# yixuan/ADMM

Hardware: AMD Instinct MI355X
Metric: ADMM iterations/sec, Lasso tall n=100000 p=10000 (100-lambda warm-started path) (higher is better)
Workload: dtype f32; 1 GPU; admm_lasso tall path (BASELINE configs[1]); n=100000, p=10000, nlambda=100, standardize=True, intercept=True, parallelism=single GPU, step=one cold-started warm-chained lambda path

## Files before the change

### admm_amd/_lib.py

```python
import ctypes
import os

import numpy as np

_HERE = os.path.dirname(os.path.abspath(__file__))
LIB_PATH = os.environ.get("ADMM_HIP_LIB") or os.path.join(_HERE, "lib", "libadmm_hip.so")

ADMM_MEM_HOST = 0
ADMM_MEM_DEVICE = 1


class AdmmOpts(ctypes.Structure):
    _fields_ = [("maxit", ctypes.c_int), ("eps_abs", ctypes.c_double),
                ("eps_rel", ctypes.c_double), ("rho", ctypes.c_double)]


class AdmmHipOptions(ctypes.Structure):
    _fields_ = [(k, ctypes.c_int) for k in (
        "struct_size", "gram_backend", "gram_split", "factor_backend", "inverse_precision", "tall_xupdate", "tall_refine",
        "consensus_two_pass", "consensus_unfused", "bp_two_pass", "lad_no_hat", "wide_no_persist", "wide_unfused", "wide_gram_sprad",
        "sharing_bp_direct", "cv_downdate", "peer_exchange", "batch_iters", "profile_stride", "pool_mb", "screen", "lad_two_pass",
        "par_devices")] + [("reserved", ctypes.c_int * 9)]


class AdmmStats(ctypes.Structure):
    _fields_ = [("t_h2d", ctypes.c_double), ("t_standardize", ctypes.c_double), ("t_gram", ctypes.c_double),
                ("t_eigs", ctypes.c_double), ("t_factor", ctypes.c_double), ("t_loop", ctypes.c_double),
                ("t_total", ctypes.c_double), ("loop_ms_events", ctypes.c_double),
                ("xupdate_ms_avg", ctypes.c_double), ("xupdate_samples", ctypes.c_longlong),
                ("total_iter", ctypes.c_longlong), ("xupdate_launches", ctypes.c_longlong),
                ("rho", ctypes.c_double), ("eig_est", ctypes.c_double),
                ("branch", ctypes.c_int), ("xupdate_variant", ctypes.c_int),
                ("exchange_variant", ctypes.c_int), ("refine", ctypes.c_int), ("persist_iter", ctypes.c_longlong),
                ("factor_flops", ctypes.c_double)]

    def as_dict(self):
        return {k: getattr(self, k) for k, _ in self._fields_}


class AdmmHipError(RuntimeError):
    def __init__(self, code, msg):
        super().__init__(f"libadmm_hip error {code}: {msg}")
        self.code = code


_lib = None

_DP = ctypes.c_void_p
_c_double_p = ctypes.POINTER(ctypes.c_double)
_c_float_p = ctypes.POINTER(ctypes.c_float)
_c_int_p = ctypes.POINTER(ctypes.c_int)

EXPORTS = ["admm_hip_lasso", "admm_hip_enet", "admm_hip_parlasso", "admm_hip_lad", "admm_hip_bp",
           "admm_hip_last_error", "admm_hip_version", "admm_hip_device_count", "admm_hip_set_device",
           "admm_hip_device_synchronize", "admm_hip_lasso_plan_create", "admm_hip_lasso_plan_run",
           "admm_hip_lasso_plan_destroy", "admm_hip_comm_unique_id", "admm_hip_comm_init", "admm_hip_comm_finalize", "admm_hip_comm_info",
           "admm_hip_parlasso_dist", "admm_hip_lasso_plan_create_dist",
           "admm_hip_lasso_plan_trace_enable", "admm_hip_lasso_plan_trace_read",
           "admm_hip_lasso_plan_state_enable", "admm_hip_lasso_plan_state_read", "admm_hip_lasso_plan_system_read",
           "admm_hip_host_lanczos", "admm_hip_test_symv",
           "admm_hip_comm_peer_prepare", "admm_hip_comm_init_peer", "admm_hip_comm_init_shm", "admm_hip_comm_test_allreduce", "admm_hip_comm_test_reduce_scatter",
           "admm_hip_lasso_dist", "admm_hip_test_gram", "admm_hip_test_spd_inverse", "admm_hip_test_cv_fold_system",
           "admm_hip_lasso_dist_cols", "admm_hip_test_gemv_t", "admm_hip_lad_traced", "admm_hip_bp_traced",
           "admm_hip_lasso_plan_create_dist_cols", "admm_hip_lasso_cv", "admm_hip_lasso_multi",
           "admm_hip_parbp", "admm_hip_parbp_traced", "admm_hip_parbp_dist", "admm_hip_dantzig", "admm_hip_dantzig_traced",
           "admm_hip_lad_state", "admm_hip_bp_state", "admm_hip_lasso_plan_data_read", "admm_hip_trim_memory", "admm_hip_test_gather",
           "admm_hip_options_default", "admm_hip_options_set", "admm_hip_option_set", "admm_hip_options_reset", "admm_hip_option_get",
           "admm_hip_last_parallel_layout", "admm_hip_parallel_assign", "admm_hip_grplasso", "admm_hip_grplasso_plan_create",
           "admm_hip_quantreg", "admm_hip_quantreg_state", "admm_hip_huber", "admm_hip_huber_state",
           "admm_hip_mtlasso", "admm_hip_mtlasso_plan_create", "admm_hip_test_symv_multi", "admm_hip_test_tall_early_exits",
           "admm_hip_sgl", "admm_hip_sgl_plan_create", "admm_hip_host_sgl_lambda0",
           "admm_hip_boxenet", "admm_hip_boxenet_plan_create", "admm_hip_host_box_lambda0",
           "admm_hip_test_gemm_nt", "admm_hip_test_cholesky_linvt", "admm_hip_test_spd_inverse_shift",
           "admm_hip_test_symv_plan", "admm_hip_test_symv_ex", "admm_hip_test_symv_multi_ex", "admm_hip_test_symv_f64acc"]

GROUP_MAX = 1024
MT_MAX = 16
MT_RHS_BUILT = (2, 4, 8, 12)

_GROUP_ARGS = [_c_int_p, _c_double_p, ctypes.c_int]
TALL_ONLY = [("admm_hip_grplasso", _GROUP_ARGS, 5), ("admm_hip_sgl", _GROUP_ARGS + [_c_double_p, ctypes.c_double], 5),
             ("admm_hip_boxenet", [_c_double_p] * 3 + [ctypes.c_double], 5), ("admm_hip_mtlasso", [ctypes.c_int, ctypes.c_int, _c_double_p], 4)]

TRACE_FIELDS = 12
TRACE_COLD, TRACE_CONVERGED, TRACE_ACCELERATE, TRACE_RESTART = -1, 0, 1, 2
TRACE_CONTINUE = 1


def load():
    global _lib
    if _lib is not None:
        return _lib
    path = os.environ.get("ADMM_HIP_LIB") or LIB_PATH
    if not os.path.exists(path):
        raise FileNotFoundError(
            f"{path} not found: build it with `python -m admm_amd.build` (hipcc --offload-arch=gfx950). "
            "admm_amd has no CPU fallback.")
    if not os.environ.get("ADMM_HIP_LIB"):
        from . import build as _build
        if os.path.isdir(_build.CSRC) and not _build._lib_is_current(path):
            raise RuntimeError(f"{path} was not built from the sources in {_build.CSRC} (source hash differs or is missing): "
                               "run `python -m admm_amd.build`")
    lib = ctypes.CDLL(path, mode=ctypes.RTLD_GLOBAL)
    lasso_args = [_DP, _DP, ctypes.c_int, ctypes.c_int, ctypes.c_int,
                  _DP, ctypes.c_int, ctypes.c_int, ctypes.c_double, ctypes.c_int, ctypes.c_int]
    tail = [ctypes.POINTER(AdmmOpts), _c_double_p, _c_float_p, _c_int_p, ctypes.POINTER(AdmmStats)]
    lib.admm_hip_lasso.argtypes = lasso_args + tail
    lib.admm_hip_enet.argtypes = lasso_args + [ctypes.c_double] + tail
    lib.admm_hip_parlasso.argtypes = lasso_args + [ctypes.c_int] + tail
    lib.admm_hip_lasso_cv.argtypes = ([_DP, _DP, ctypes.c_int, ctypes.c_int, ctypes.c_int, _c_int_p, ctypes.c_int,
                                       _DP, ctypes.c_int, ctypes.c_int, ctypes.c_double, ctypes.c_int, ctypes.c_int, ctypes.c_double,
                                       ctypes.POINTER(AdmmOpts), _c_double_p, _c_float_p, _c_int_p,
                                       _c_double_p, _c_double_p, _c_double_p, _c_int_p, _c_float_p, _c_int_p, _c_int_p,
                                       ctypes.POINTER(AdmmStats)])
    lib.admm_hip_lasso_cv.restype = ctypes.c_int
    lib.admm_hip_lasso_multi.argtypes = ([_DP, _DP, ctypes.c_int, ctypes.c_int, ctypes.c_int, ctypes.c_int,
                                          _DP, ctypes.c_int, ctypes.c_int, ctypes.c_double, ctypes.c_int, ctypes.c_int, ctypes.c_double,
                                          ctypes.POINTER(AdmmOpts), _c_double_p, _c_float_p, _c_int_p, ctypes.POINTER(AdmmStats)])
    lib.admm_hip_lasso_multi.restype = ctypes.c_int
    lib.admm_hip_lad.argtypes = [_DP, _DP, ctypes.c_int, ctypes.c_int, ctypes.c_int, ctypes.c_int,
                                 ctypes.POINTER(AdmmOpts), _c_double_p, _c_int_p, ctypes.POINTER(AdmmStats)]
    lib.admm_hip_bp.argtypes = [_DP, _DP, ctypes.c_int, ctypes.c_int, ctypes.c_int,
                                ctypes.POINTER(AdmmOpts), _c_double_p, _c_int_p, ctypes.POINTER(AdmmStats)]
    lib.admm_hip_lad_traced.argtypes = lib.admm_hip_lad.argtypes + [_c_double_p, ctypes.c_longlong, ctypes.POINTER(ctypes.c_longlong)]
    lib.admm_hip_lad_traced.restype = ctypes.c_int
    lib.admm_hip_bp_traced.argtypes = lib.admm_hip_bp.argtypes + [_c_double_p, ctypes.c_longlong, ctypes.POINTER(ctypes.c_longlong)]
    lib.admm_hip_bp_traced.restype = ctypes.c_int
    lib.admm_hip_lad_state.argtypes = lib.admm_hip_lad_traced.argtypes + [_c_double_p, ctypes.c_longlong, ctypes.POINTER(ctypes.c_longlong)]
    lib.admm_hip_lad_state.restype = ctypes.c_int
    lib.admm_hip_quantreg.argtypes = [_DP, _DP, ctypes.c_int, ctypes.c_int, ctypes.c_int, ctypes.c_int, _c_double_p, ctypes.c_int,
                                      ctypes.POINTER(AdmmOpts), _c_double_p, _c_int_p, ctypes.POINTER(AdmmStats)]
    lib.admm_hip_quantreg.restype = ctypes.c_int
    lib.admm_hip_quantreg_state.argtypes = ([_DP, _DP, ctypes.c_int, ctypes.c_int, ctypes.c_int, ctypes.c_int, ctypes.c_double,
                                             ctypes.POINTER(AdmmOpts), _c_double_p, _c_int_p, ctypes.POINTER(AdmmStats)]
                                            + [_c_double_p, ctypes.c_longlong, ctypes.POINTER(ctypes.c_longlong)] * 2)
    lib.admm_hip_quantreg_state.restype = ctypes.c_int
    lib.admm_hip_huber.argtypes = [_DP, _DP, ctypes.c_int, ctypes.c_int, ctypes.c_int, ctypes.c_int, _c_double_p, _c_double_p, ctypes.c_int,
                                   ctypes.POINTER(AdmmOpts), _c_double_p, _c_int_p, ctypes.POINTER(AdmmStats)]
    lib.admm_hip_huber.restype = ctypes.c_int
    lib.admm_hip_huber_state.argtypes = ([_DP, _DP, ctypes.c_int, ctypes.c_int, ctypes.c_int, ctypes.c_int, ctypes.c_double, ctypes.c_double,
                                          ctypes.POINTER(AdmmOpts), _c_double_p, _c_int_p, ctypes.POINTER(AdmmStats)]
                                         + [_c_double_p, ctypes.c_longlong, ctypes.POINTER(ctypes.c_longlong)] * 2)
    lib.admm_hip_huber_state.restype = ctypes.c_int
    lib.admm_hip_bp_state.argtypes = lib.admm_hip_bp_traced.argtypes + [_c_double_p, ctypes.c_longlong, ctypes.POINTER(ctypes.c_longlong)]
    lib.admm_hip_bp_state.restype = ctypes.c_int
    lib.admm_hip_dantzig.argtypes = [_DP, _DP, ctypes.c_int, ctypes.c_int, ctypes.c_int, _DP, ctypes.c_int, ctypes.c_int, ctypes.c_double,
                                     ctypes.c_int, ctypes.c_int, ctypes.POINTER(AdmmOpts), _c_double_p, _c_double_p, _c_int_p, ctypes.POINTER(AdmmStats)]
    lib.admm_hip_dantzig.restype = ctypes.c_int
    lib.admm_hip_dantzig_traced.argtypes = lib.admm_hip_dantzig.argtypes + [_c_double_p, ctypes.c_longlong, ctypes.POINTER(ctypes.c_longlong)]
    lib.admm_hip_dantzig_traced.restype = ctypes.c_int
    lib.admm_hip_parbp.argtypes = [_DP, _DP, ctypes.c_int, ctypes.c_int, ctypes.c_int, ctypes.c_int,
                                   ctypes.POINTER(AdmmOpts), _c_double_p, _c_int_p, ctypes.POINTER(AdmmStats)]
    lib.admm_hip_parbp.restype = ctypes.c_int
    lib.admm_hip_parbp_traced.argtypes = lib.admm_hip_parbp.argtypes + [_c_double_p, ctypes.c_longlong, ctypes.POINTER(ctypes.c_longlong)]
    lib.admm_hip_parbp_traced.restype = ctypes.c_int
    lib.admm_hip_parbp_dist.argtypes = [_DP, _DP, ctypes.c_int, ctypes.c_int, ctypes.c_longlong, ctypes.c_longlong, ctypes.c_int, ctypes.c_int,
                                        ctypes.POINTER(AdmmOpts), _c_double_p, _c_int_p, ctypes.POINTER(AdmmStats)]
    lib.admm_hip_parbp_dist.restype = ctypes.c_int
    for name in ("admm_hip_lasso", "admm_hip_enet", "admm_hip_parlasso", "admm_hip_lad", "admm_hip_bp",
                 "admm_hip_device_count", "admm_hip_set_device", "admm_hip_device_synchronize"):
        getattr(lib, name).restype = ctypes.c_int
    lib.admm_hip_set_device.argtypes = [ctypes.c_int]
    lib.admm_hip_last_error.restype = ctypes.c_char_p
    lib.admm_hip_version.restype = ctypes.c_char_p
    lib.admm_hip_lasso_plan_create.argtypes = lasso_args + [ctypes.c_double, ctypes.c_int, ctypes.POINTER(AdmmOpts),
                                               ctypes.POINTER(ctypes.c_void_p), _c_int_p]
    lib.admm_hip_lasso_plan_create.restype = ctypes.c_int
    for name, extra, at in TALL_ONLY:
        args = lasso_args[:at] + extra + lasso_args[5:]
        for fn, rest in ((getattr(lib, name), tail), (getattr(lib, name + "_plan_create"), [tail[0], ctypes.POINTER(ctypes.c_void_p), _c_int_p])):
            fn.argtypes, fn.restype = args + rest, ctypes.c_int
    lib.admm_hip_host_sgl_lambda0.argtypes = [_c_float_p, ctypes.c_int, _c_int_p, _c_double_p, ctypes.c_int, _c_double_p, ctypes.c_double, _c_float_p]
    lib.admm_hip_host_sgl_lambda0.restype = ctypes.c_int
    lib.admm_hip_host_box_lambda0.argtypes = [_c_float_p, ctypes.c_int, _c_float_p, _c_float_p, _c_double_p, ctypes.c_double, _c_float_p]
    lib.admm_hip_host_box_lambda0.restype = ctypes.c_int
    lib.admm_hip_lasso_plan_run.argtypes = [ctypes.c_void_p, _c_double_p, _c_float_p, _c_int_p, ctypes.POINTER(AdmmStats)]
    lib.admm_hip_lasso_plan_run.restype = ctypes.c_int
    lib.admm_hip_lasso_plan_destroy.argtypes = [ctypes.c_void_p]
    lib.admm_hip_lasso_plan_destroy.restype = ctypes.c_int
    dist_args = [_DP, _DP, ctypes.c_int, ctypes.c_longlong, ctypes.c_int, ctypes.c_int,
                 _DP, ctypes.c_int, ctypes.c_int, ctypes.c_double, ctypes.c_int, ctypes.c_int, ctypes.c_int, ctypes.POINTER(AdmmOpts)]
    lib.admm_hip_parlasso_dist.argtypes = dist_args + [_c_double_p, _c_float_p, _c_int_p, ctypes.POINTER(AdmmStats)]
    lib.admm_hip_parlasso_dist.restype = ctypes.c_int
    lib.admm_hip_lasso_plan_create_dist.argtypes = dist_args + [ctypes.POINTER(ctypes.c_void_p), _c_int_p]
    lib.admm_hip_lasso_plan_create_dist.restype = ctypes.c_int
    lib.admm_hip_lasso_dist.argtypes = [_DP, _DP, ctypes.c_int, ctypes.c_longlong, ctypes.c_int, ctypes.c_int,
                                        _DP, ctypes.c_int, ctypes.c_int, ctypes.c_double, ctypes.c_int, ctypes.c_int, ctypes.c_double,
                                        ctypes.POINTER(AdmmOpts), _c_double_p, _c_float_p, _c_int_p, ctypes.POINTER(AdmmStats)]
    lib.admm_hip_lasso_dist.restype = ctypes.c_int
    lib.admm_hip_lasso_dist_cols.argtypes = [_DP, _DP, ctypes.c_int, ctypes.c_int, ctypes.c_longlong, ctypes.c_longlong, ctypes.c_int,
                                             _DP, ctypes.c_int, ctypes.c_int, ctypes.c_double, ctypes.c_int, ctypes.c_int, ctypes.c_double,
                                             ctypes.POINTER(AdmmOpts), _c_double_p, _c_float_p, _c_int_p, ctypes.POINTER(AdmmStats)]
    lib.admm_hip_lasso_dist_cols.restype = ctypes.c_int
    lib.admm_hip_lasso_plan_create_dist_cols.argtypes = lib.admm_hip_lasso_dist_cols.argtypes[:15] + [ctypes.POINTER(ctypes.c_void_p), _c_int_p]
    lib.admm_hip_lasso_plan_create_dist_cols.restype = ctypes.c_int
    lib.admm_hip_comm_unique_id.argtypes = [ctypes.c_void_p]
    lib.admm_hip_comm_unique_id.restype = ctypes.c_int
    lib.admm_hip_comm_init.argtypes = [ctypes.c_int, ctypes.c_int, ctypes.c_void_p]
    lib.admm_hip_comm_init.restype = ctypes.c_int
    lib.admm_hip_comm_finalize.argtypes = []
    lib.admm_hip_comm_finalize.restype = ctypes.c_int
    lib.admm_hip_options_default.argtypes = [ctypes.POINTER(AdmmHipOptions)]
    lib.admm_hip_options_default.restype = ctypes.c_int
    lib.admm_hip_options_set.argtypes = [ctypes.POINTER(AdmmHipOptions)]
    lib.admm_hip_options_set.restype = ctypes.c_int
    lib.admm_hip_option_set.argtypes = [ctypes.c_char_p, ctypes.c_char_p]
    lib.admm_hip_option_set.restype = ctypes.c_int
    lib.admm_hip_options_reset.argtypes = []
    lib.admm_hip_options_reset.restype = ctypes.c_int
    lib.admm_hip_option_get.argtypes = [ctypes.c_char_p]
    lib.admm_hip_option_get.restype = ctypes.c_char_p
    lib.admm_hip_comm_info.argtypes = [ctypes.POINTER(ctypes.c_int)] * 3
    lib.admm_hip_comm_info.restype = ctypes.c_int
    lib.admm_hip_comm_peer_prepare.argtypes = [ctypes.c_int, ctypes.c_void_p]
    lib.admm_hip_comm_peer_prepare.restype = ctypes.c_int
    lib.admm_hip_comm_init_peer.argtypes = [ctypes.c_int, ctypes.c_int, ctypes.c_void_p]
    lib.admm_hip_comm_init_peer.restype = ctypes.c_int
    lib.admm_hip_comm_init_shm.argtypes = [ctypes.c_int, ctypes.c_int, ctypes.c_char_p, ctypes.c_ulonglong]
    lib.admm_hip_comm_init_shm.restype = ctypes.c_int
    lib.admm_hip_comm_test_allreduce.argtypes = [ctypes.c_void_p, ctypes.c_longlong, ctypes.c_void_p, ctypes.c_longlong, ctypes.c_int]
    lib.admm_hip_comm_test_allreduce.restype = ctypes.c_int
    lib.admm_hip_comm_test_reduce_scatter.argtypes = [ctypes.c_void_p, ctypes.c_longlong, ctypes.c_void_p]
    lib.admm_hip_comm_test_reduce_scatter.restype = ctypes.c_int
    lib.admm_hip_lasso_plan_trace_enable.argtypes = [ctypes.c_void_p, ctypes.c_longlong]
    lib.admm_hip_lasso_plan_trace_enable.restype = ctypes.c_int
    lib.admm_hip_lasso_plan_trace_read.argtypes = [ctypes.c_void_p, _c_double_p, ctypes.c_longlong, ctypes.POINTER(ctypes.c_longlong)]
    lib.admm_hip_lasso_plan_trace_read.restype = ctypes.c_int
    lib.admm_hip_lasso_plan_state_enable.argtypes = [ctypes.c_void_p, ctypes.c_longlong]
    lib.admm_hip_lasso_plan_state_enable.restype = ctypes.c_int
    lib.admm_hip_lasso_plan_state_read.argtypes = [ctypes.c_void_p, ctypes.POINTER(ctypes.c_float), ctypes.c_longlong,
                                                   ctypes.POINTER(ctypes.c_longlong), ctypes.POINTER(ctypes.c_longlong)]
    lib.admm_hip_lasso_plan_state_read.restype = ctypes.c_int
    lib.admm_hip_lasso_plan_data_read.argtypes = [ctypes.c_void_p, ctypes.POINTER(ctypes.c_float), ctypes.c_longlong, ctypes.POINTER(ctypes.c_float)]
    lib.admm_hip_lasso_plan_data_read.restype = ctypes.c_int
    lib.admm_hip_lasso_plan_system_read.argtypes = [ctypes.c_void_p, ctypes.POINTER(ctypes.c_float), ctypes.c_longlong]
    lib.admm_hip_lasso_plan_system_read.restype = ctypes.c_int
    lib.admm_hip_test_symv.argtypes = [_c_float_p, ctypes.c_int, _c_float_p, _c_float_p, _c_float_p, _c_float_p]
    lib.admm_hip_test_symv.restype = ctypes.c_int
    lib.admm_hip_test_symv_multi.argtypes = [_c_float_p, ctypes.c_int, _c_float_p, ctypes.c_int, ctypes.c_int, _c_float_p]
    lib.admm_hip_test_symv_multi.restype = ctypes.c_int
    lib.admm_hip_test_symv_plan.argtypes = [ctypes.c_int] * 4 + [_c_int_p, ctypes.POINTER(ctypes.c_longlong), _c_int_p, ctypes.c_int]
    lib.admm_hip_test_symv_plan.restype = ctypes.c_int
    lib.admm_hip_test_symv_ex.argtypes = [_c_float_p, ctypes.c_int, _c_float_p, _c_float_p, ctypes.c_int, ctypes.c_int, ctypes.c_int,
                                          _c_float_p, _c_float_p, _c_int_p]
    lib.admm_hip_test_symv_ex.restype = ctypes.c_int
    lib.admm_hip_test_symv_multi_ex.argtypes = [_c_float_p, ctypes.c_int, _c_float_p, ctypes.c_int, ctypes.c_int, ctypes.c_int, ctypes.c_int,
                                                _c_float_p, _c_int_p]
    lib.admm_hip_test_symv_multi_ex.restype = ctypes.c_int
    lib.admm_hip_test_symv_f64acc.argtypes = [_c_float_p, ctypes.c_int, _c_float_p, _c_float_p, _c_double_p, _c_double_p, _c_int_p]
    lib.admm_hip_test_symv_f64acc.restype = ctypes.c_int
    lib.admm_hip_test_tall_early_exits.argtypes = [ctypes.POINTER(ctypes.c_longlong)]
    lib.admm_hip_test_tall_early_exits.restype = ctypes.c_int
    lib.admm_hip_test_gram.argtypes = [ctypes.c_void_p, ctypes.c_int, ctypes.c_int, ctypes.c_int, ctypes.c_int, ctypes.c_void_p]
    lib.admm_hip_test_gram.restype = ctypes.c_int
    lib.admm_hip_test_gemv_t.argtypes = [ctypes.c_void_p, ctypes.c_int, ctypes.c_int, ctypes.c_int, ctypes.c_void_p, ctypes.c_void_p]
    lib.admm_hip_test_gemv_t.restype = ctypes.c_int
    lib.admm_hip_test_spd_inverse.argtypes = [ctypes.c_void_p, ctypes.c_int, ctypes.c_int, ctypes.c_void_p]
    lib.admm_hip_test_spd_inverse.restype = ctypes.c_int
    lib.admm_hip_test_spd_inverse_shift.argtypes = [ctypes.c_void_p, ctypes.c_int, ctypes.c_double, ctypes.c_void_p]
    lib.admm_hip_test_spd_inverse_shift.restype = ctypes.c_int
    lib.admm_hip_test_cholesky_linvt.argtypes = [ctypes.c_int, ctypes.c_void_p, ctypes.c_int, ctypes.c_void_p, ctypes.c_void_p]
    lib.admm_hip_test_cholesky_linvt.restype = ctypes.c_int
    lib.admm_hip_test_gemm_nt.argtypes = [ctypes.c_int] * 9 + [ctypes.c_double, ctypes.c_double, ctypes.c_void_p, ctypes.c_void_p, ctypes.c_void_p]
    lib.admm_hip_test_gemm_nt.restype = ctypes.c_int
    lib.admm_hip_test_cv_fold_system.argtypes = [ctypes.c_void_p, ctypes.c_void_p, ctypes.c_int, ctypes.c_int, ctypes.c_void_p, ctypes.c_int, ctypes.c_int,
                                                 ctypes.c_int, ctypes.c_int, ctypes.c_void_p, ctypes.c_void_p, ctypes.c_void_p, ctypes.c_void_p, ctypes.c_void_p]
    lib.admm_hip_test_cv_fold_system.restype = ctypes.c_int
    lib.admm_hip_host_lanczos.argtypes = [_c_float_p, ctypes.c_int, _c_float_p, _c_int_p]
    lib.admm_hip_host_lanczos.restype = ctypes.c_int
    lib.admm_hip_test_gather.argtypes = [ctypes.c_void_p, ctypes.c_int, ctypes.c_int, ctypes.c_int, ctypes.c_void_p, _c_double_p]
    lib.admm_hip_test_gather.restype = ctypes.c_int
    lib.admm_hip_last_parallel_layout.argtypes = [_c_int_p, _c_int_p, ctypes.c_int]
    lib.admm_hip_last_parallel_layout.restype = ctypes.c_int
    lib.admm_hip_parallel_assign.argtypes = [ctypes.c_int, ctypes.c_char_p, ctypes.c_int, _c_int_p, _c_int_p, ctypes.c_int]
    lib.admm_hip_parallel_assign.restype = ctypes.c_int
    lib.admm_hip_trim_memory.argtypes = []
    lib.admm_hip_trim_memory.restype = ctypes.c_int
    _lib = lib
    return lib


def check(code):
    if code != 0:
        raise AdmmHipError(code, load().admm_hip_last_error().decode())


class DevicePtr:

    def __init__(self, ptr):
        self.ptr = int(ptr)


def as_input(a, n=None, p=None):
    if isinstance(a, DevicePtr):
        return ctypes.c_void_p(a.ptr), ADMM_MEM_DEVICE, a
    arr = np.asfortranarray(np.asarray(a, dtype=np.float64))
    return ctypes.c_void_p(arr.ctypes.data), ADMM_MEM_HOST, arr


class options:

    def __init__(self, **kw):
        self.kw = {k.upper(): (None if v is None else str(v)) for k, v in kw.items()}
        self.old = {}

    def __enter__(self):
        lib = load()
        try:
            for k, v in self.kw.items():
                cur = lib.admm_hip_option_get(k.encode())
                self.old[k] = cur.decode() if cur is not None else None
                check(lib.admm_hip_option_set(k.encode(), None if v is None else v.encode()))
        except BaseException:
            self.__exit__(None, None, None)
            raise
        return self

    def __exit__(self, *exc):
        lib = load()
        for k, v in self.old.items():
            check(lib.admm_hip_option_set(k.encode(), None if v is None else v.encode()))
        return False

    @staticmethod
    def set(**kw):
        lib = load()
        for k, v in kw.items():
            check(lib.admm_hip_option_set(k.upper().encode(), None if v is None else str(v).encode()))

    @staticmethod
    def reset():
        check(load().admm_hip_options_reset())

    @staticmethod
    def struct(**fields):
        lib = load()
        o = AdmmHipOptions()
        check(lib.admm_hip_options_default(ctypes.byref(o)))
        for k, v in fields.items():
            setattr(o, k, int(v))
        check(lib.admm_hip_options_set(ctypes.byref(o)))
        return o


def last_parallel_layout():
    lib = load()
    nr = ctypes.c_int(0)
    devs = (ctypes.c_int * 64)()
    check(lib.admm_hip_last_parallel_layout(ctypes.byref(nr), devs, 64))
    return [int(devs[r]) for r in range(min(nr.value, 64))]


def parallel_assign(nblocks, par_devices, device_count):
    lib = load()
    nr = ctypes.c_int(0)
    devs = (ctypes.c_int * 64)()
    check(lib.admm_hip_parallel_assign(int(nblocks), None if par_devices is None else str(par_devices).encode(), int(device_count),
                                       ctypes.byref(nr), devs, 64))
    return [int(devs[r]) for r in range(nr.value)] if nr.value > 1 else []
```

### admm_amd/csrc/api.hip

```cpp
#include "calls.h"
#include "comm.h"
#include "inproc.h"
#include "test_hooks.h"

using namespace admm;

template <typename F>
static int guarded(F&& f) {
    try {
        check_option_overlay();
        f();
        return ADMM_OK;
    } catch (const Error& e) {
        set_last_error(e.what());
        return e.code;
    } catch (const std::bad_alloc&) {
        set_last_error("host allocation failed");
        return ADMM_ERR_INTERNAL;
    } catch (const std::exception& e) {
        set_last_error(e.what());
        return ADMM_ERR_INTERNAL;
    }
}

// ... 284 lines not shown
int admm_hip_mtlasso_plan_create(const double* x, const double* Y, int n, int p, int m, int mem,
                                 const double* row_weight,
                                 const double* lambda_in, int nlambda_in, int nlambda_auto, double lmin_ratio,
                                 int standardize, int intercept, const admm_opts* opts,
                                 admm_hip_plan** plan_out, int* nlambda_out) {
    return guarded([&] { plan_create(x, Y, n, p, mem, mt_spec(PATH_SPEC(-1.0), p, m, row_weight), plan_out, nlambda_out); });
}

int admm_hip_options_default(admm_hip_options* o) {
    return guarded([&] {
        ADMM_REQUIRE(o != nullptr, "options must not be NULL");
        std::memset(o, 0, sizeof(*o));
        o->struct_size = (int)sizeof(*o);
    });
}
int admm_hip_options_reset(void) { return guarded([&] { thread_options() = ThreadOptions(); }); }
int admm_hip_option_set(const char* name, const char* value) {
    return guarded([&] {
        ADMM_REQUIRE(name != nullptr && name[0] != 0, "option name must not be empty");
        Opt id;
        ADMM_REQUIRE(opt_find(name, &id), std::string("unknown option '") + name + "' (INTEGRATION.md section 5 lists the names)");
        opt_set_thread(id, value);
    });
}
const char* admm_hip_option_get(const char* name) {
    Opt id;
    return name && opt_find(name, &id) ? opt_text(id) : nullptr;
}
int admm_hip_options_set(const admm_hip_options* o) {
    return guarded([&] {
        ThreadOptions n;
        if (o == nullptr) { thread_options() = n; return; }
        ADMM_REQUIRE(o->struct_size >= (int)(2 * sizeof(int)) && o->struct_size <= (int)sizeof(admm_hip_options), "options: bad struct_size");
        admm_hip_options v;
        std::memset(&v, 0, sizeof(v));
        std::memcpy(&v, o, (size_t)o->struct_size);
        auto set = [&](Opt k, const char* val) { opt_parse(k, val, &n.v[(int)k]); n.has[(int)k] = true; };
        auto num = [&](Opt k, int val) { set(k, std::to_string(val).c_str()); };
        if (v.gram_backend == 1) set(Opt::GRAM, "rocblas");
        if (v.gram_split) { ADMM_REQUIRE(v.gram_split >= 1 && v.gram_split <= 3, "options: gram_split"); set(Opt::GRAM_SPLIT, v.gram_split == 1 ? "0" : (v.gram_split == 2 ? "f16x2" : "bf16x3")); }
        if (v.factor_backend == 1) set(Opt::FACTOR, "rocsolver");
        if (v.inverse_precision) { ADMM_REQUIRE(v.inverse_precision == 1 || v.inverse_precision == 2, "options: inverse_precision"); set(Opt::INVERSE, v.inverse_precision == 1 ? "f32" : "f64"); }
        if (v.tall_xupdate) { ADMM_REQUIRE(v.tall_xupdate == 1 || v.tall_xupdate == 2, "options: tall_xupdate"); set(Opt::XUPDATE, v.tall_xupdate == 1 ? "gemv" : "sym"); }
        if (v.tall_refine) set(Opt::REFINE, "1");
        if (v.consensus_two_pass) set(Opt::PAR_ONEPASS, "0");
        if (v.consensus_unfused >= 1) set(Opt::PAR_FUSE_PZ, "0");
        if (v.consensus_unfused >= 2) set(Opt::PAR_BATCH, "0");
        if (v.bp_two_pass) set(Opt::BP_ONEPASS, "0");
        if (v.lad_no_hat) set(Opt::LAD_HAT, "0");
        if (v.wide_no_persist == 1) set(Opt::WIDE_PERSIST, "0");
        if (v.wide_no_persist == 2) set(Opt::WIDE_PERSIST_COLS, "0");
        if (v.wide_unfused) set(Opt::WIDE_FUSE, "0");
        if (v.wide_gram_sprad) set(Opt::WIDE_SPRAD, "gram");
        if (v.sharing_bp_direct) set(Opt::SBP_GRAM, "0");
        if (v.cv_downdate) set(Opt::CV_DOWNDATE, v.cv_downdate == 1 ? "1" : "0");
        if (v.peer_exchange) set(Opt::PEER_FUSED, v.peer_exchange == 1 ? "2" : "0");
        if (v.batch_iters > 0) num(Opt::BATCH_ITERS, v.batch_iters);
        if (v.profile_stride > 0) num(Opt::PROFILE_STRIDE, v.profile_stride);
        if (v.pool_mb) num(Opt::POOL_MB, v.pool_mb < 0 ? 0 : v.pool_mb);
        if (v.lad_two_pass) set(Opt::LAD_ONEPASS, "0");
        if (v.par_devices) {
            ADMM_REQUIRE(v.par_devices >= -1 && v.par_devices <= 64, "options: par_devices");
            std::string l;
            for (int d = 0; d < v.par_devices; ++d) l += (d ? "," : "") + std::to_string(d);
            set(Opt::PAR_DEVICES, v.par_devices == -1 ? "all" : l.c_str());
        }
        if (v.screen) {
            ADMM_REQUIRE(v.screen >= 1 && v.screen <= 3, "options: screen");
            set(Opt::WIDE_SCREEN, v.screen == 1 ? "16" : (v.screen == 3 ? "8" : "0"));
            set(Opt::SBP_SCREEN, v.screen == 2 ? "0" : "1");
        }
        thread_options() = n;
    });
}
int admm_hip_comm_unique_id(void* id_out) {
    return guarded([&] { ADMM_REQUIRE(id_out != nullptr, "id_out must not be NULL"); comm_unique_id(id_out); });
}
int admm_hip_comm_init(int nranks, int rank, const void* id) {
    return guarded([&] { ADMM_REQUIRE(id != nullptr, "id must not be NULL"); require_device(); comm_init(nranks, rank, id); });
}
int admm_hip_comm_finalize(void) {
    return guarded([&] { comm_finalize(); });
}
int admm_hip_comm_info(int* nranks_out, int* rank_out, int* backend_out) {
    return guarded([&] {
        const CommInfo ci = comm_info_live();
        if (nranks_out) *nranks_out = ci.active ? ci.nranks : 1;
        if (rank_out) *rank_out = ci.active ? ci.rank : 0;
        if (backend_out) *backend_out = ci.active ? ci.backend : 0;
    });
}
int admm_hip_comm_peer_prepare(int nranks, void* handle_out) {
    return guarded([&] { ADMM_REQUIRE(handle_out != nullptr, "handle_out must not be NULL"); require_device(); comm_peer_prepare(nranks, handle_out); });
}
int admm_hip_comm_init_peer(int nranks, int rank, const void* handles) {
    return guarded([&] { ADMM_REQUIRE(handles != nullptr, "handles must not be NULL"); require_device(); comm_init_peer(nranks, rank, handles); });
}
int admm_hip_comm_init_shm(int nranks, int rank, const char* name, unsigned long long token) {
    return guarded([&] { require_device(); comm_init_shm(nranks, rank, name, token); });
}
int admm_hip_comm_test_allreduce(float* fbuf, long long nf, double* dbuf, long long nd, int mem) {
    return guarded([&] {
        ADMM_REQUIRE(nf >= 0 && nd >= 0 && (nf == 0 || fbuf) && (nd == 0 || dbuf), "bad arguments");
        ADMM_REQUIRE(comm_info().active, "no communicator");
        require_device();
        Stream st;
        DevBuf<float> df; DevBuf<double> dd;
        float* pf = fbuf; double* pd = dbuf;
        if (mem == ADMM_MEM_HOST) {
            df.alloc((size_t)nf); dd.alloc((size_t)nd);
            if (nf) ADMM_HIP_CHECK(hipMemcpyAsync(df.get(), fbuf, (size_t)nf * sizeof(float), hipMemcpyHostToDevice, st.s));
            if (nd) ADMM_HIP_CHECK(hipMemcpyAsync(dd.get(), dbuf, (size_t)nd * sizeof(double), hipMemcpyHostToDevice, st.s));
            pf = df.get(); pd = dd.get();
        }
        if (nf && nd) allreduce_sum_f32_f64(pf, (size_t)nf, pd, (size_t)nd, st.s);
        else if (nf) allreduce_sum_f32(pf, (size_t)nf, st.s);
        else if (nd) allreduce_sum_f64(pd, (size_t)nd, st.s);
        if (mem == ADMM_MEM_HOST) {
            if (nf) ADMM_HIP_CHECK(hipMemcpyAsync(fbuf, pf, (size_t)nf * sizeof(float), hipMemcpyDeviceToHost, st.s));
            if (nd) ADMM_HIP_CHECK(hipMemcpyAsync(dbuf, pd, (size_t)nd * sizeof(double), hipMemcpyDeviceToHost, st.s));
        }
        st.sync();
        comm_check();
    });
}

int admm_hip_comm_test_reduce_scatter(const float* send, long long count, float* recv) {
    return guarded([&] {
        ADMM_REQUIRE(count > 0 && count % 4 == 0 && send && recv, "bad arguments (count must be a positive multiple of 4)");
        require_device();
        const CommInfo ci = comm_info();
        const size_t nr = (size_t)(ci.active ? ci.nranks : 1);
        Stream st;
        DevBuf<float> ds(nr * (size_t)count), dr((size_t)count);
        ADMM_HIP_CHECK(hipMemcpyAsync(ds.get(), send, nr * (size_t)count * sizeof(float), hipMemcpyHostToDevice, st.s));
        reduce_scatter_sum_f32(ds.get(), dr.get(), (size_t)count, st.s);
        ADMM_HIP_CHECK(hipMemcpyAsync(recv, dr.get(), (size_t)count * sizeof(float), hipMemcpyDeviceToHost, st.s));
        st.sync();
        comm_check();
    });
}

int admm_hip_lasso_plan_run(admm_hip_plan* plan, double* lambda_out, float* beta_out, int* niter_out, admm_stats* stats) {
    return guarded([&] { run_plan(reinterpret_cast<PlanHandle*>(plan), PATH_OUT, 0.0); });
}

int admm_hip_lasso_plan_destroy(admm_hip_plan* plan) {
    return guarded([&] { delete reinterpret_cast<PlanHandle*>(plan); });
}

int admm_hip_lasso_plan_trace_enable(admm_hip_plan* plan, long long capacity_records) {
    return guarded([&] {
        ADMM_REQUIRE(capacity_records > 0 && capacity_records <= (1ll << 26), "trace capacity must be within [1, 2^26] records");
        plan_of(plan).enable_trace(capacity_records);
    });
}

int admm_hip_lasso_plan_trace_read(admm_hip_plan* plan, double* out, long long cap_records, long long* nrecords_out) {
    return guarded([&] {
        ADMM_REQUIRE(out != nullptr && nrecords_out != nullptr && cap_records >= 0, "bad trace output arguments");
        *nrecords_out = plan_of(plan).read_trace(out, cap_records);
    });
}

int admm_hip_lasso_plan_state_enable(admm_hip_plan* plan, long long capacity_records) {
    return guarded([&] {
        ADMM_REQUIRE(capacity_records > 0 && capacity_records <= (1ll << 22), "state capacity must be within [1, 2^22] records");
        plan_of(plan).enable_state(capacity_records);
    });
}

int admm_hip_lasso_plan_state_read(admm_hip_plan* plan, float* out, long long cap_records, long long* nrecords_out, long long* record_floats_out) {
    return guarded([&] {
        ADMM_REQUIRE(nrecords_out != nullptr && cap_records >= 0 && (out != nullptr || cap_records == 0), "bad state output arguments");
        *nrecords_out = plan_of(plan).read_state(out, cap_records, record_floats_out);
    });
}

int admm_hip_lasso_plan_data_read(admm_hip_plan* plan, float* x_out, long long ld, float* y_out) {
    return guarded([&] {
        plan_of(plan).read_data(x_out, ld, y_out);
    });
}

int admm_hip_lasso_plan_system_read(admm_hip_plan* plan, float* out, long long ld) {
    return guarded([&] {
        plan_of(plan).read_system(out, ld);
    });
}

int admm_hip_last_parallel_layout(int* nranks, int* devices, int cap) {
    return guarded([&] {
        ADMM_REQUIRE(nranks != nullptr && cap >= 0 && (cap == 0 || devices != nullptr), "bad layout arguments");
        *nranks = (int)last_layout().size();
        for (int r = 0; r < std::min(cap, *nranks); ++r) devices[r] = last_layout()[r];
    });
}

int admm_hip_parallel_assign(int nblocks, const char* par_devices, int device_count, int* nranks, int* devices, int cap) {
    return guarded([&] {
        ADMM_REQUIRE(nblocks >= 1 && device_count >= 0, "nblocks must be >= 1 and device_count >= 0");
        ADMM_REQUIRE(nranks != nullptr && cap >= 0 && (cap == 0 || devices != nullptr), "bad layout arguments");
        const std::vector<int> lay = par_layout(nblocks, parse_par_devices(par_devices, device_count));
        *nranks = lay.empty() ? 1 : (int)lay.size();
        for (int r = 0; r < std::min(cap, (int)lay.size()); ++r) devices[r] = lay[r];
    });
}

const char* admm_hip_last_error(void) { return last_error_ref().c_str(); }
const char* admm_hip_version(void) { return "admm_hip 0.3 (gfx950)"; }
int admm_hip_trim_memory(void) {
    admm::pool_trim();
    return ADMM_OK;
}

int admm_hip_device_count(void) {
    int cnt = 0;
    if (hipGetDeviceCount(&cnt) != hipSuccess) return 0;
    return cnt;
}
int admm_hip_set_device(int device) {
    return guarded([&] { ADMM_HIP_CHECK(hipSetDevice(device)); });
}
int admm_hip_device_synchronize(void) {
    return guarded([&] { ADMM_HIP_CHECK(hipDeviceSynchronize()); });
}

int admm_hip_host_lanczos(const float* A, int n, float* eig_out, int* nmatop_out) {
    return guarded([&] {
        ADMM_REQUIRE(A && eig_out && n >= 3, "bad arguments");
        auto op = [&](const float* v, float* w) {
            for (int i = 0; i < n; ++i) w[i] = 0.f;
            for (int j = 0; j < n; ++j) {
                const float vj = v[j];
                const float* col = A + (size_t)j * n;
                for (int i = 0; i < n; ++i) w[i] += col[i] * vj;
            }
        };
        *eig_out = lanczos_largest_f32(op, n, nmatop_out);
    });
}

int admm_hip_host_sgl_lambda0(const float* xy, int p, const int* group, const double* group_weight, int ngroups,
                              const double* l1_weight, double alpha, float* out) {
    return guarded([&] {
        ADMM_REQUIRE(xy && out && p > 0, "bad arguments");
        const PathSpec s = sgl_spec(PathSpec(), p, group, group_weight, ngroups, l1_weight, alpha);
        s.check_sgl_args(p);
        const std::vector<int> start = s.group_starts();
        std::vector<double> l1, wg;
        sgl_prepare(alpha, l1_weight, group_weight, start, l1, wg);
        *out = sgl_lambda0(xy, start, l1, wg);
    });
}

int admm_hip_host_box_lambda0(const float* xy, int p, const float* lower_std, const float* upper_std, const double* penalty_factor,
                              double alpha, float* out) {
    return guarded([&] {
        ADMM_REQUIRE(xy && out && p > 0, "bad arguments");
        PathSpec s = box_spec(PathSpec(), p, nullptr, nullptr, penalty_factor);
        s.alpha = alpha;
        s.check_box_args(p);
        for (int j = 0; j < p; ++j)
            ADMM_REQUIRE((!lower_std || lower_std[j] <= 0.f) && (!upper_std || upper_std[j] >= 0.f), "the box must hold zero");
        float l0 = box_lambda0(xy, p, lower_std, upper_std, penalty_factor);
        if (s.enet()) l0 = box_lambda0_enet(l0, alpha);
        *out = l0;
    });
}

int admm_hip_test_symv(const float* A, int p, const float* v0, const float* v1, float* y0, float* y1) {
    return guarded([&] {
        ADMM_REQUIRE(A && v0 && v1 && y0 && y1 && p > 0, "bad arguments");
        test_symv(A, p, v0, v1, y0, y1);
    });
}

int admm_hip_test_symv_multi(const float* A, int p, const float* V, int nr, int rhs_per_pass, float* Yout) {
    return guarded([&] {
        ADMM_REQUIRE(A && V && Yout && p > 0 && nr >= 1 && nr <= 64, "bad arguments");
        test_symv_multi(A, p, V, nr, rhs_per_pass, Yout);
    });
}

int admm_hip_test_symv_plan(int p, int cus, int part, int nparts, int* sched_out, long long* info_out, int* tiles_out, int tile_capacity) {
    return guarded([&] {
        ADMM_REQUIRE(sched_out && info_out && tiles_out, "symv plan hook: sched_out, info_out and tiles_out must not be NULL");
        ADMM_REQUIRE(p >= 1 && p <= kSymvHookMaxP && cus <= 65536 && nparts >= 1 && nparts <= 64 && part >= 0 && part < nparts && tile_capacity >= 1,
                     "symv plan hook: p in 1 .. 32768, cus <= 65536, nparts in 1 .. 64, part in 0 .. nparts - 1, tile_capacity >= 1");
        test_symv_plan(p, cus, part, nparts, sched_out, info_out, tiles_out, tile_capacity);
    });
}

int admm_hip_test_symv_ex(const float* A, int p, const float* v0, const float* v1, int variant, int part, int nparts, float* y0, float* y1,
                          int* sched_out) {
    return guarded([&] {
        ADMM_REQUIRE(A && v0 && v1 && y0 && y1 && sched_out, "symv_ex hook: A, v0, v1, y0, y1 and sched_out must not be NULL");
        ADMM_REQUIRE(p >= 1 && p <= kSymvHookMaxP && variant >= 0 && variant <= 2 && nparts >= 1 && nparts <= 64 && part >= 0 && part < nparts,
                     "symv_ex hook: p in 1 .. 32768, variant in 0 .. 2, nparts in 1 .. 64, part in 0 .. nparts - 1");
        test_symv_ex(A, p, v0, v1, variant, part, nparts, y0, y1, sched_out);
    });
}

int admm_hip_test_symv_multi_ex(const float* A, int p, const float* V, int nr, int rhs_per_pass, int nt, int finish, float* Yout, int* sched_out) {
    return guarded([&] {
        ADMM_REQUIRE(A && V && Yout && sched_out, "symv_multi_ex hook: A, V, Yout and sched_out must not be NULL");
        ADMM_REQUIRE(p >= 1 && p <= kSymvHookMaxP && nr >= 1 && nr <= 64 && test_symv_rhs_built(rhs_per_pass) && (nt == 0 || nt == 1) && (finish == 0 || finish == 1),
                     "symv_multi_ex hook: p in 1 .. 32768, nr in 1 .. 64, rhs_per_pass one of the built widths (2, 4, 8, 12), nt and finish 0 or 1");
        test_symv_multi_ex(A, p, V, nr, rhs_per_pass, nt, finish, Yout, sched_out);
    });
}

int admm_hip_test_symv_f64acc(const float* A, int p, const float* v0, const float* v1, double* y0, double* y1, int* sched_out) {
    return guarded([&] {
        ADMM_REQUIRE(A && v0 && v1 && y0 && y1 && sched_out, "symv_f64acc hook: A, v0, v1, y0, y1 and sched_out must not be NULL");
        ADMM_REQUIRE(p >= 1 && p <= kSymvHookMaxP, "symv_f64acc hook: p in 1 .. 32768");
        test_symv_f64acc(A, p, v0, v1, y0, y1, sched_out);
    });
}

int admm_hip_test_tall_early_exits(long long* count) {
    return guarded([&] {
        ADMM_REQUIRE(count != nullptr, "bad arguments");
        *count = tall_last_early_exits();
    });
}

int admm_hip_test_gram(const void* A, int rows, int cols, int atA, int is_double, void* G) {
    return guarded([&] {
        ADMM_REQUIRE(A && G && rows > 0 && cols > 0, "bad arguments");
        if (is_double) test_gram<double>(static_cast<const double*>(A), rows, cols, atA != 0, static_cast<double*>(G));
        else test_gram<float>(static_cast<const float*>(A), rows, cols, atA != 0, static_cast<float*>(G));
    });
}

int admm_hip_test_gemv_t(const void* A, int rows, int cols, int is_double, const void* v, void* y) {
    return guarded([&] {
        ADMM_REQUIRE(A && v && y && rows > 0 && cols > 0, "bad arguments");
        if (is_double) test_gemv_t<double>(static_cast<const double*>(A), rows, cols, static_cast<const double*>(v), static_cast<double*>(y));
        else test_gemv_t<float>(static_cast<const float*>(A), rows, cols, static_cast<const float*>(v), static_cast<float*>(y));
    });
}

int admm_hip_test_gather(const void* A, int rows, int cols, int is_double, const void* v, double* y) {
    return guarded([&] {
        ADMM_REQUIRE(A && v && y && rows > 0 && cols > 0, "bad arguments");
        if (is_double) test_gather<double>(static_cast<const double*>(A), rows, cols, static_cast<const double*>(v), y);
        else test_gather<float>(static_cast<const float*>(A), rows, cols, static_cast<const float*>(v), y);
    });
}

int admm_hip_test_spd_inverse(const void* A, int n, int precision, void* Ainv) {
    return guarded([&] {
        ADMM_REQUIRE(A && Ainv && n > 0 && precision >= 0 && precision <= 2, "bad arguments");
        if (precision == 1) test_spd_inverse<double>(static_cast<const double*>(A), n, static_cast<double*>(Ainv), false);
        else test_spd_inverse<float>(static_cast<const float*>(A), n, static_cast<float*>(Ainv), precision == 2);
    });
}

int admm_hip_test_spd_inverse_shift(const float* A, int n, double diag, float* Ainv) {
    return guarded([&] {
        ADMM_REQUIRE(A && Ainv && n > 0 && std::isfinite(diag), "bad arguments");
        test_spd_inverse_shift(A, n, diag, Ainv);
    });
}

int admm_hip_test_cholesky_linvt(int is_double, const void* A, int n, void* L, void* U) {
    return guarded([&] {
        ADMM_REQUIRE(A && L && U && n > 0, "bad arguments");
        if (is_double) test_cholesky_linvt<double>(static_cast<const double*>(A), n, static_cast<double*>(L), static_cast<double*>(U));
        else test_cholesky_linvt<float>(static_cast<const float*>(A), n, static_cast<float*>(L), static_cast<float*>(U));
    });
}

int admm_hip_test_gemm_nt(int is_double, int lower, int mirror, int kstart_row, int b_lower, int in_place, int M, int N, int K,
                          double alpha, double beta, const void* A, const void* B, void* C) {
    return guarded([&] {
        ADMM_REQUIRE(A && B && C, "gemm_nt hook: A, B and C must not be NULL");
        ADMM_REQUIRE(M > 0 && N > 0 && K > 0 && M <= 16384 && N <= 16384 && K <= (1 << 20), "gemm_nt hook: M, N in 1 .. 16384 and K in 1 .. 2^20");
        ADMM_REQUIRE(std::isfinite(alpha) && std::isfinite(beta), "gemm_nt hook: alpha and beta must be finite");
        ADMM_REQUIRE(!lower || M == N, "gemm_nt hook: lower needs a square output (M == N)");
        ADMM_REQUIRE(!mirror || lower, "gemm_nt hook: the mirrored store belongs to lower launches");
        ADMM_REQUIRE(!b_lower || (is_double && !lower), "gemm_nt hook: b_lower (the K loop ended at the tile's last column) is double only and not for lower launches");
        ADMM_REQUIRE(!in_place || (N <= 128 && K == 128 && !lower), "gemm_nt hook: in_place needs N <= 128, K == 128 and a full (not lower) launch");
        if (is_double)
            test_gemm_nt<double>(lower != 0, mirror != 0, kstart_row != 0, b_lower != 0, in_place != 0, M, N, K, alpha, beta, static_cast<const double*>(A),
                                 static_cast<const double*>(B), static_cast<double*>(C));
        else
            test_gemm_nt<float>(lower != 0, mirror != 0, kstart_row != 0, false, in_place != 0, M, N, K, alpha, beta, static_cast<const float*>(A),
                                static_cast<const float*>(B), static_cast<float*>(C));
    });
}

int admm_hip_test_cv_fold_system(const double* x, const double* y, int n, int p, const int* fold_id, int nfolds, int fold,
                                 int standardize, int intercept, float* gram, float* xy, float* mean_x, float* scale_x, float* mean_scale_y) {
    return guarded([&] { test_cv_fold_system(x, y, n, p, fold_id, nfolds, fold, standardize, intercept, gram, xy, mean_x, scale_x, mean_scale_y); });
}

}
```

### admm_amd/csrc/lasso_tall.hip

```cpp
#include "prep.h"
#include "gemv_kernels.h"
#include "symv_kernels.h"
#include "solvers.h"
#include "sgl_host.h"
#include "box_host.h"
#include "comm.h"
#include "loop_driver.h"
#include "plan_host.h"
#include "peer_device.h"
#include "probe.h"

namespace admm {

struct TallCtl {
    double rho, lam, eps_primal, eps_dual, adj_a, adj_c, tau;
    double a_next, tau_next;
    int mode;
    int restart;
    int iter;
    int lam_idx;
    int done;
    int first;
    int total;
    int fin_idx;
    int fin_niter;
    int pad;
};

struct TallParams {
    int p, nwg, nseg, maxit, nlam, enet;
    long long part_stride;
    double eps_abs, eps_rel, alpha, sqrt_p;
    const double* lambdas;
    const float* XY;
    const float* a_part; const float* b_part;
    const float* dot0; const float* dot1; const float* axp0; const float* axp1;
    long long ldo; int nrb, p32; SymvSched sched;
    float* x; float* z0; float* z1; float* y0; float* y1; float* adj_z; float* adj_y; float* u; float* w;
    TallCtl* ctl;
    double* P;
    float* beta;
    int* niter;
    int* done_host;
#ifdef ADMM_HIP_PROBE
    long long* probe;
#endif
    double* trace;
    long long trace_cap;
    const float* refine_ab;
    long long refine_ld;
    float* state;
    long long state_cap;
    unsigned long long* verdict;
    unsigned long long run_tag;
};

__host__ __device__ inline unsigned long long tall_verdict_word(unsigned long long run_tag, int total, bool discard) {
    return run_tag | ((unsigned long long)(unsigned)total << 1) | (discard ? 1ull : 0ull);
}
constexpr int kVerdictShift = 33;
constexpr int kVerdictWords = kSyVerdictReplicas * kSyVerdictStride;

constexpr int kTailThreads = 256;
constexpr int kTailLanes = kSySumLanes;
constexpr int kTailElems = kTailThreads / kTailLanes;

__device__ __forceinline__ double tall_load_partial(const double* p, bool in_launch) {
    if (!in_launch) return *p;
    return __longlong_as_double((long long)__hip_atomic_load(reinterpret_cast<const unsigned long long*>(p), __ATOMIC_RELAXED, __HIP_MEMORY_SCOPE_AGENT));
}
__device__ __forceinline__ void tall_store_wt(float* p, float v) {
    __hip_atomic_store(reinterpret_cast<unsigned int*>(p), __float_as_uint(v), __ATOMIC_RELAXED, __HIP_MEMORY_SCOPE_AGENT);
}
__device__ __forceinline__ void tall_store_wt(double* p, double v) {
    __hip_atomic_store(reinterpret_cast<unsigned long long*>(p), (unsigned long long)__double_as_longlong(v), __ATOMIC_RELAXED, __HIP_MEMORY_SCOPE_AGENT);
}

template <bool IN_LAUNCH = false>
__device__ void tall_decide(const TallParams& q, int par) {
    __shared__ double dscratch[6 * (kTailThreads / 64)];
    WIDE_PROBE_DECL
    WIDE_PROBE(0);
    const TallCtl in = q.ctl[par];
    TallCtl* outp = &q.ctl[par ^ 1];
    if (in.done) {
        if (threadIdx.x == 0) { TallCtl o = in; o.fin_idx = -1; *outp = o; }
        return;
    }
    WIDE_PROBE(1);
    double acc[6] = {0, 0, 0, 0, 0, 0};
    const double* Pin = q.P + (size_t)par * q.nwg * 8;
    for (int w = threadIdx.x; w < q.nwg; w += kTailThreads) {
#pragma unroll
        for (int k = 0; k < 6; ++k) acc[k] += tall_load_partial(Pin + (size_t)w * 8 + k, IN_LAUNCH);
    }
    block_sum<double, 6>(acc, dscratch);
    if (threadIdx.x != 0) return;
    WIDE_PROBE(2);
    const double r2 = acc[0], dz2 = acc[1], daz2 = acc[2], x2 = acc[3], z2 = acc[4], y2 = acc[5];
    double tr_rp = 0, tr_rd = 0, tr_c = 0, tr_code = ADMM_TRACE_COLD;
    TallCtl out = in;
    out.first = 0;
    out.fin_idx = -1; out.fin_niter = 0;
    if (!in.first) {
        const double rp = sqrt(r2);
        const double rd = in.rho * sqrt(dz2);
        tr_rp = rp; tr_rd = rd;
        if (rp < in.eps_primal && rd < in.eps_dual) {
            out.fin_idx = in.lam_idx; out.fin_niter = in.iter + 1;
            out.mode = 0;
            tr_code = ADMM_TRACE_CONVERGED;
        } else {
            const double old_c = in.adj_c;
            const double c = in.rho * rp * rp + in.rho * daz2;
            tr_c = c;
            if (c < 0.999 * old_c) {
                out.adj_a = in.a_next; out.adj_c = c; out.tau = in.tau_next; out.restart = 0;
                tr_code = ADMM_TRACE_ACCELERATE;
            } else {
                out.adj_a = 1.0; out.adj_c = old_c / 0.999; out.tau = -1.0; out.restart = 1;
                tr_code = ADMM_TRACE_RESTART;
            }
            out.mode = 1;
            out.iter = in.iter + 1;
            if (in.iter + 1 >= q.maxit) {
                out.fin_idx = in.lam_idx; out.fin_niter = q.maxit + 1;
            }
        }
        if (out.fin_idx >= 0) {
            out.lam_idx = in.lam_idx + 1;
            out.iter = 0;
            if (out.lam_idx >= q.nlam) out.done = 1;
            else out.lam = q.lambdas[out.lam_idx];
            q.niter[out.fin_idx] = out.fin_niter;
        }
    } else {
        out.mode = 1; out.tau = 0.0; out.restart = 0;
    }
    if (q.verdict != nullptr && (out.mode == 0 || out.done)) {
        const unsigned long long word = tall_verdict_word(q.run_tag, in.total + 1, true);
        for (int r = 0; r < kSyVerdictReplicas; ++r)
            __hip_atomic_store(q.verdict + (size_t)r * kSyVerdictStride, word, __ATOMIC_RELAXED, __HIP_MEMORY_SCOPE_AGENT);
    }
    out.eps_primal = fmax(sqrt(x2), sqrt(z2)) * q.eps_rel + q.sqrt_p * q.eps_abs;
    out.eps_dual = sqrt(y2) * q.eps_rel + q.sqrt_p * q.eps_abs;
    out.a_next = 0.5 + 0.5 * sqrt(1.0 + 4.0 * out.adj_a * out.adj_a);
    out.tau_next = (out.adj_a - 1.0) / out.a_next;
    out.total = in.total + 1;
    *outp = out;
    if (out.done) *q.done_host = 1;
    WIDE_PROBE(3);
    WIDE_PROBE_FLUSH(2, in.total);
    if (q.trace != nullptr && in.total < q.trace_cap) {
        double* t = q.trace + (size_t)in.total * ADMM_TRACE_FIELDS;
        t[0] = in.lam_idx; t[1] = in.iter; t[2] = in.eps_primal; t[3] = in.eps_dual; t[4] = tr_rp; t[5] = tr_rd;
        t[6] = tr_c; t[7] = in.adj_c; t[8] = tr_code; t[9] = in.rho; t[10] = in.rho; t[11] = in.lam;
    }
}

struct TallDecideExtra {
    static constexpr bool kHas = true;
    TallParams q; int par;
    __device__ void operator()() const { tall_decide<false>(q, par); }
};

__device__ __forceinline__ float tall_extrapolate(float t1, float t, float cur, float old) {
#pragma clang fp contract(off)
    const float a = t1 * cur;
    const float b = t * old;
    return a - b;
}

struct TallElem { float zc, yc, zo, yo, adjz, adjy, x, xy; };

__device__ __forceinline__ TallElem tall_load_elem(const TallParams& q, int par, int i) {
    const float* zc_ = par ? q.z1 : q.z0; const float* yc_ = par ? q.y1 : q.y0;
    const float* zo_ = par ? q.z0 : q.z1; const float* yo_ = par ? q.y0 : q.y1;
    TallElem e;
    e.zc = zc_[i]; e.yc = yc_[i]; e.zo = zo_[i]; e.yo = yo_[i]; e.adjz = q.adj_z[i]; e.adjy = q.adj_y[i]; e.x = q.x[i]; e.xy = q.XY[i];
    return e;
}

__device__ __forceinline__ float tall_soft(float vec, double pen) {
    const double v = (double)vec;
    return v > pen ? (float)(v - pen) : (v < -pen ? (float)(v + pen) : 0.f);
}

__device__ __forceinline__ double tall_block_shrink(double nrm2, double pen) {
    const double nrm = sqrt(nrm2);
    return nrm > pen ? 1.0 - pen / nrm : 0.0;
}

template <bool WT = false>
__device__ __forceinline__ void tall_update_elem(const TallParams& q, const TallCtl& c, int par, int i, const TallElem& e, float a, float b, double (&acc)[6]) {
#pragma clang fp contract(off)
    float* zo_ = par ? q.z0 : q.z1; float* yo_ = par ? q.y0 : q.y1;
    const float zc = e.zc, yc = e.yc, zo = e.zo, yo = e.yo;
    if (c.fin_idx >= 0) q.beta[(size_t)c.fin_idx * q.p + i] = zc;
    if (c.done) return;
    float adjz, adjy, x;
    if (c.mode) {
        if (c.restart) { adjz = zo; adjy = yo; x = b; }
        else {
            const float t = (float)c.tau, t1 = (float)(1.0 + c.tau);
            adjz = tall_extrapolate(t1, t, zc, zo);
            adjy = tall_extrapolate(t1, t, yc, yo);
            x = a;
        }
    } else { adjz = e.adjz; adjy = e.adjy; x = e.x; }
    const float rho_f = (float)c.rho;
    const float vec = x + adjy / rho_f;
    const double pen = c.lam / c.rho;
    float zn;
    if (!q.enet) zn = tall_soft(vec, pen);
    else {
        const float thresh = (float)(q.alpha * pen);
        const float denom = (float)(1.0 + pen * (1.0 - q.alpha));
        zn = vec > thresh ? (vec - thresh) / denom : (vec < -thresh ? (vec + thresh) / denom : 0.f);
    }
    const float r = x - zn;
    const float yn = adjy + rho_f * r;
    const float dz = zn - zc, daz = zn - adjz;
    acc[0] = (double)r * r; acc[1] = (double)dz * dz; acc[2] = (double)daz * daz;
    acc[3] = (double)x * x; acc[4] = (double)zn * zn; acc[5] = (double)yn * yn;
    q.x[i] = x; zo_[i] = zn; yo_[i] = yn; q.adj_z[i] = adjz; q.adj_y[i] = adjy;
    if (q.state != nullptr && c.total < q.state_cap) {
        float* s = q.state + (size_t)c.total * 5 * q.p;
        s[i] = x; s[q.p + i] = zn; s[2 * (size_t)q.p + i] = yn; s[3 * (size_t)q.p + i] = adjz; s[4 * (size_t)q.p + i] = adjy;
    }
    const float tn = (float)c.tau_next, tn1 = (float)(1.0 + c.tau_next);
    const float adjz_a = tall_extrapolate(tn1, tn, zn, zc), adjy_a = tall_extrapolate(tn1, tn, yn, yc);
    const float un = (float)((double)(e.xy - adjy_a) + c.rho * (double)adjz_a);
    const float wn = (float)((double)(e.xy - yc) + c.rho * (double)zc);
    if (WT) { tall_store_wt(q.u + i, un); tall_store_wt(q.w + i, wn); }
    else { q.u[i] = un; q.w[i] = wn; }
}

__device__ __forceinline__ void tall_publish_norms(const TallParams& q, int par, const double (&acc)[6], double* scratch) {
    static_assert(kTailLanes == 8, "owner lanes are the multiples of 8");
    const int lane = threadIdx.x & 63, wid = threadIdx.x >> 6;
    const double v8[8] = {acc[0], acc[1], acc[2], acc[3], acc[4], acc[5], 0.0, 0.0};
    const double tot = halving_sum8_top(v8, lane);
    if ((lane & 7) == 0 && lane < 48) scratch[(lane >> 3) * (kTailThreads / 64) + wid] = tot;
    __syncthreads();
    if (threadIdx.x < 6) {
        double sum = 0;
        for (int ww = 0; ww < kTailThreads / 64; ++ww) sum += scratch[threadIdx.x * (kTailThreads / 64) + ww];
        q.P[((size_t)(par ^ 1) * q.nwg + blockIdx.x) * 8 + threadIdx.x] = sum;
    }
}

enum { TAIL_GEMV = 0, TAIL_SYMV = 1, TAIL_PEER = 2, TAIL_PEER1 = 3 };

__device__ __forceinline__ void tall_lane_sum(float& a, float& b) {
#pragma unroll
    for (int m = 1; m < kTailLanes; m <<= 1) { a += __shfl_xor(a, m, 64); b += __shfl_xor(b, m, 64); }
}

template <int MODE>
__device__ __forceinline__ void tall_gather_ab(const TallParams& q, int i, int sub, bool valid, float& a, float& b) {
    if (MODE == TAIL_SYMV) {
        symv_sum_partials<kTailLanes>(q.dot0, q.dot1, q.axp0, q.axp1, q.ldo, q.nrb, q.sched, q.p32, i, sub, valid, a, b);
        return;
    }
    a = 0.f; b = 0.f;
    if (valid) {
        for (int k = sub; k < q.nseg; k += kTailLanes) {
            const size_t o = (size_t)k * q.part_stride + i;
            a += q.a_part[o]; b += q.b_part[o];
        }
    }
    tall_lane_sum(a, b);
}

template <int MODE>
__global__ void __launch_bounds__(kTailThreads)
tall_tail_kernel(TallParams q, int par, PeerExchange ex) {
    __shared__ double scratch[6 * (kTailThreads / 64)];
    WIDE_PROBE_DECL
    WIDE_PROBE(0);
    const TallCtl c = q.ctl[par ^ 1];
    const int sub = threadIdx.x & (kTailLanes - 1);
    const int i = blockIdx.x * kTailElems + threadIdx.x / kTailLanes;
    const bool valid = i < q.p;
    const bool owner = valid && sub == 0;
    TallElem e = {0.f, 0.f, 0.f, 0.f, 0.f, 0.f, 0.f, 0.f};
    if (owner) e = tall_load_elem(q, par, i);
    float a = 0.f, b = 0.f;
    if (MODE == TAIL_PEER || MODE == TAIL_PEER1) {
        const bool live = !q.ctl[par].done;
        if (MODE == TAIL_PEER1 && live) {
            float sa, sb;
            symv_sum_partials<kTailLanes>(q.dot0, q.dot1, q.axp0, q.axp1, q.ldo, q.nrb, q.sched, q.p32, i, sub, valid, sa, sb);
            if (valid) {
                for (int dst = sub; dst < ex.nranks; dst += kTailLanes)
                    peer_store_f32x2(reinterpret_cast<float*>(peer_dst_slot(ex, dst)) + 2 * (size_t)i, sa, sb);
            }
            peer_publish(ex, gridDim.x);
        }
        const bool ok = live ? peer_wait_relaxed(ex) : false;
        if (ok && valid) {
            for (int r = sub; r < ex.nranks; r += kTailLanes) {
                const float2 v = peer_load_f32x2(reinterpret_cast<const float*>(peer_src_slot(ex, r)) + 2 * (size_t)i);
                a += v.x; b += v.y;
            }
        }
        tall_lane_sum(a, b);
    } else {
        tall_gather_ab<MODE>(q, i, sub, valid, a, b);
        if (MODE == TAIL_SYMV && q.refine_ab != nullptr && valid) {
            a = q.refine_ab[i] + a;
            b = q.refine_ab[q.refine_ld + i] + b;
        }
    }
    if (c.done && c.fin_idx < 0) return;
    WIDE_PROBE(1);

    double acc[6] = {0, 0, 0, 0, 0, 0};
    if (owner) tall_update_elem(q, c, par, i, e, a, b, acc);
    if (c.done) return;
    WIDE_PROBE(2);
    tall_publish_norms(q, par, acc, scratch);
    WIDE_PROBE(3);
    WIDE_PROBE_FLUSH(blockIdx.x == 0 ? 0 : (blockIdx.x == gridDim.x - 1 ? 1 : -1), c.total - 1);
}

struct GroupCoord { int gs, gn; double w; };
struct GroupTailParams {
    const int2* tiles;
    const GroupCoord* coord;
    const double* l1;
};
constexpr int kGroupMax = ADMM_HIP_GROUP_MAX;

template <int MODE, bool SPARSE = false>
__global__ void __launch_bounds__(kTailThreads)
tall_group_tail_kernel(TallParams q, int par, GroupTailParams gp) {
#pragma clang fp contract(off)
    static_assert(MODE == TAIL_GEMV || MODE == TAIL_SYMV, "single device");
    __shared__ double scratch[6 * (kTailThreads / 64)];
    __shared__ double snrm[kTailElems];
    __shared__ float sx[kGroupMax], sadjz[kGroupMax], sadjy[kGroupMax], sv[kGroupMax], szc[kGroupMax], syc[kGroupMax], sxy[kGroupMax];
    const TallCtl c = q.ctl[par ^ 1];
    const int2 tile = gp.tiles[blockIdx.x];
    const int i0 = tile.x, cnt = tile.y;
    const int sub = threadIdx.x & (kTailLanes - 1), e = threadIdx.x / kTailLanes;
    const int npass = (cnt + kTailElems - 1) / kTailElems;
    const bool big = cnt > kTailElems;
    const GroupCoord gc = gp.coord[i0 + min(e, cnt - 1)];
    float* zo_ = par ? q.z0 : q.z1; float* yo_ = par ? q.y0 : q.y1;
    const float rho_f = (float)c.rho;

    for (int k = 0; k < npass; ++k) {
        const int s = k * kTailElems + e, i = i0 + s;
        const bool valid = s < cnt, owner = valid && sub == 0;
        TallElem el = {0.f, 0.f, 0.f, 0.f, 0.f, 0.f, 0.f, 0.f};
        if (owner) el = tall_load_elem(q, par, i);
        double l1 = 0.0;
        if (SPARSE && owner) l1 = gp.l1[i];
        float a, b;
        tall_gather_ab<MODE>(q, i, sub, valid, a, b);
        if (c.done && c.fin_idx < 0) return;
        if (owner) {
            if (c.fin_idx >= 0) q.beta[(size_t)c.fin_idx * q.p + i] = el.zc;
            if (!c.done) {
                float adjz, adjy, x;
                if (c.mode) {
                    if (c.restart) { adjz = el.zo; adjy = el.yo; x = b; }
                    else {
                        const float t = (float)c.tau, t1 = (float)(1.0 + c.tau);
                        adjz = tall_extrapolate(t1, t, el.zc, el.zo);
                        adjy = tall_extrapolate(t1, t, el.yc, el.yo);
                        x = a;
                    }
                } else { adjz = el.adjz; adjy = el.adjy; x = el.x; }
                float vec = x + adjy / rho_f;
                if (SPARSE && gc.gn > 1) vec = tall_soft(vec, c.lam * l1 / c.rho);
                sx[s] = x; sadjz[s] = adjz; sadjy[s] = adjy; sv[s] = vec;
                szc[s] = el.zc; syc[s] = el.yc; sxy[s] = el.xy;
            }
        }
    }
    if (c.done) return;
    __syncthreads();

    double nrm2 = 0.0;
    if (big) {
        if (sub == 0) {
            double part = 0.0;
            for (int s = e; s < cnt; s += kTailElems) { const double v = (double)sv[s]; part += v * v; }
            snrm[e] = part;
        }
        __syncthreads();
        for (int m = 0; m < kTailElems; ++m) nrm2 += snrm[m];
    } else if (sub == 0 && e < cnt && gc.gn > 1) {
        const int s0 = gc.gs - i0;
        for (int m = 0; m < gc.gn; ++m) { const double v = (double)sv[s0 + m]; nrm2 += v * v; }
    }
    const double pen = c.lam * gc.w / c.rho;
    double shrink = 0.0;
    if (gc.gn > 1) shrink = tall_block_shrink(nrm2, pen);

    double acc[6] = {0, 0, 0, 0, 0, 0};
    const float tn = (float)c.tau_next, tn1 = (float)(1.0 + c.tau_next);
    for (int k = 0; k < npass; ++k) {
        const int s = k * kTailElems + e, i = i0 + s;
        if (!(s < cnt && sub == 0)) continue;
        const float x = sx[s], adjz = sadjz[s], adjy = sadjy[s], vec = sv[s], zc = szc[s], yc = syc[s], xy = sxy[s];
        const double v = (double)vec;
        float zn;
        if (gc.gn == 1) zn = tall_soft(vec, pen);
        else zn = (float)(v * shrink);
        const float r = x - zn;
        const float yn = adjy + rho_f * r;
        const float dz = zn - zc, daz = zn - adjz;
        acc[0] += (double)r * r; acc[1] += (double)dz * dz; acc[2] += (double)daz * daz;
        acc[3] += (double)x * x; acc[4] += (double)zn * zn; acc[5] += (double)yn * yn;
        q.x[i] = x; zo_[i] = zn; yo_[i] = yn; q.adj_z[i] = adjz; q.adj_y[i] = adjy;
        if (q.state != nullptr && c.total < q.state_cap) {
            float* st = q.state + (size_t)c.total * 5 * q.p;
            st[i] = x; st[q.p + i] = zn; st[2 * (size_t)q.p + i] = yn; st[3 * (size_t)q.p + i] = adjz; st[4 * (size_t)q.p + i] = adjy;
        }
        const float adjz_a = tall_extrapolate(tn1, tn, zn, zc), adjy_a = tall_extrapolate(tn1, tn, yn, yc);
        q.u[i] = (float)((double)(xy - adjy_a) + c.rho * (double)adjz_a);
        q.w[i] = (float)((double)(xy - yc) + c.rho * (double)zc);
    }
    tall_publish_norms(q, par, acc, scratch);
}

struct BoxTailParams {
    const double* pf;
    const float* lo; const float* hi;
};

template <int MODE>
__global__ void __launch_bounds__(kTailThreads)
tall_box_tail_kernel(TallParams q, int par, BoxTailParams bp) {
#pragma clang fp contract(off)
    static_assert(MODE == TAIL_GEMV || MODE == TAIL_SYMV, "single device");
    __shared__ double scratch[6 * (kTailThreads / 64)];
    const TallCtl c = q.ctl[par ^ 1];
    const int sub = threadIdx.x & (kTailLanes - 1);
    const int i = blockIdx.x * kTailElems + threadIdx.x / kTailLanes;
    const bool valid = i < q.p;
    const bool owner = valid && sub == 0;
    TallElem e = {0.f, 0.f, 0.f, 0.f, 0.f, 0.f, 0.f, 0.f};
    double pf = 0.0;
    float lo = 0.f, hi = 0.f;
    if (owner) { e = tall_load_elem(q, par, i); pf = bp.pf[i]; lo = bp.lo[i]; hi = bp.hi[i]; }
    float a, b;
    tall_gather_ab<MODE>(q, i, sub, valid, a, b);
    if (c.done && c.fin_idx < 0) return;

    double acc[6] = {0, 0, 0, 0, 0, 0};
    if (owner) {
        float* zo_ = par ? q.z0 : q.z1; float* yo_ = par ? q.y0 : q.y1;
        const float zc = e.zc, yc = e.yc, zo = e.zo, yo = e.yo;
        if (c.fin_idx >= 0) q.beta[(size_t)c.fin_idx * q.p + i] = zc;
        if (!c.done) {
            float adjz, adjy, x;
            if (c.mode) {
                if (c.restart) { adjz = zo; adjy = yo; x = b; }
                else {
                    const float t = (float)c.tau, t1 = (float)(1.0 + c.tau);
                    adjz = tall_extrapolate(t1, t, zc, zo);
                    adjy = tall_extrapolate(t1, t, yc, yo);
                    x = a;
                }
            } else { adjz = e.adjz; adjy = e.adjy; x = e.x; }
            const float rho_f = (float)c.rho;
            const float vec = x + adjy / rho_f;
            const double pen = c.lam * pf / c.rho;
            float zn;
            if (!q.enet) zn = tall_soft(vec, pen);
            else {
                const float thresh = (float)(q.alpha * pen);
                const float denom = (float)(1.0 + pen * (1.0 - q.alpha));
                zn = vec > thresh ? (vec - thresh) / denom : (vec < -thresh ? (vec + thresh) / denom : 0.f);
            }
            zn = fminf(fmaxf(zn, lo), hi);
            const float r = x - zn;
            const float yn = adjy + rho_f * r;
            const float dz = zn - zc, daz = zn - adjz;
            acc[0] = (double)r * r; acc[1] = (double)dz * dz; acc[2] = (double)daz * daz;
            acc[3] = (double)x * x; acc[4] = (double)zn * zn; acc[5] = (double)yn * yn;
            q.x[i] = x; zo_[i] = zn; yo_[i] = yn; q.adj_z[i] = adjz; q.adj_y[i] = adjy;
            if (q.state != nullptr && c.total < q.state_cap) {
                float* s = q.state + (size_t)c.total * 5 * q.p;
                s[i] = x; s[q.p + i] = zn; s[2 * (size_t)q.p + i] = yn; s[3 * (size_t)q.p + i] = adjz; s[4 * (size_t)q.p + i] = adjy;
            }
            const float tn = (float)c.tau_next, tn1 = (float)(1.0 + c.tau_next);
            const float adjz_a = tall_extrapolate(tn1, tn, zn, zc), adjy_a = tall_extrapolate(tn1, tn, yn, yc);
            q.u[i] = (float)((double)(e.xy - adjy_a) + c.rho * (double)adjz_a);
            q.w[i] = (float)((double)(e.xy - yc) + c.rho * (double)zc);
        }
    }
    if (c.done) return;
    tall_publish_norms(q, par, acc, scratch);
}

struct MtTailParams {
    int m;
    long long ldv, ldxy;
    float* uw;
    const float* dot; const float* axp;
    long long dot_stride, axp_stride;
    const double* row_w;
};
constexpr int kMtMax = ADMM_HIP_MT_MAX;
static_assert(kMtMax % kMtChunk == 0, "whole chunks");

__global__ void __launch_bounds__(kTailThreads)
tall_mt_tail_kernel(TallParams q, int par, MtTailParams mp) {
#pragma clang fp contract(off)
    __shared__ double scratch[6 * (kTailThreads / 64)];
    const TallCtl c = q.ctl[par ^ 1];
    const int sub = threadIdx.x & (kTailLanes - 1);
    const int i = blockIdx.x * kTailElems + threadIdx.x / kTailLanes;
    const bool valid = i < q.p;
    const bool owner = valid && sub == 0;
    const int m = mp.m;
    const float* zc_ = par ? q.z1 : q.z0; const float* yc_ = par ? q.y1 : q.y0;
    float* zo_ = par ? q.z0 : q.z1; float* yo_ = par ? q.y0 : q.y1;
    const double wj = owner ? mp.row_w[i] : 0.0;
    const float rho_f = (float)c.rho;
    float sx[kMtMax], sadjz[kMtMax], sadjy[kMtMax], sv[kMtMax], szc[kMtMax], syc[kMtMax], sxy[kMtMax];
    double nrm2 = 0.0;

#pragma unroll
    for (int ch = 0; ch < kMtMax / kMtChunk; ++ch) {
        const int k0 = ch * kMtChunk;
        if (k0 < m) {
            const int nk = min(kMtChunk, m - k0);
            TallElem e[kMtChunk];
#pragma unroll
            for (int kk = 0; kk < kMtChunk; ++kk) {
                const int kc = min(k0 + kk, m - 1);
                const size_t o = (size_t)kc * mp.ldv + i;
                e[kk] = TallElem{0.f, 0.f, 0.f, 0.f, 0.f, 0.f, 0.f, 0.f};
                if (owner) {
                    e[kk].zc = zc_[o]; e[kk].yc = yc_[o]; e[kk].zo = zo_[o]; e[kk].yo = yo_[o];
                    e[kk].adjz = q.adj_z[o]; e[kk].adjy = q.adj_y[o]; e[kk].x = q.x[o]; e[kk].xy = q.XY[(size_t)kc * mp.ldxy + i];
                }
            }
            float a[kMtChunk], b[kMtChunk];
            symv_sum_partials_n<kTailLanes, kMtChunk>(mp.dot + (size_t)(2 * k0) * mp.dot_stride, mp.dot_stride, mp.axp + (size_t)(2 * k0) * mp.axp_stride, mp.axp_stride,
                                                      nk, q.ldo, q.nrb, q.sched, q.p32, i, sub, valid, a, b);
            if (c.done && c.fin_idx < 0) return;
#pragma unroll
            for (int kk = 0; kk < kMtChunk; ++kk) {
                const int k = k0 + kk;
                if (kk < nk && owner) {
                    const TallElem el = e[kk];
                    if (c.fin_idx >= 0) q.beta[((size_t)c.fin_idx * m + k) * q.p + i] = el.zc;
                    if (!c.done) {
                        float adjz, adjy, x;
                        if (c.mode) {
                            if (c.restart) { adjz = el.zo; adjy = el.yo; x = b[kk]; }
                            else {
                                const float t = (float)c.tau, t1 = (float)(1.0 + c.tau);
                                adjz = tall_extrapolate(t1, t, el.zc, el.zo);
                                adjy = tall_extrapolate(t1, t, el.yc, el.yo);
                                x = a[kk];
                            }
                        } else { adjz = el.adjz; adjy = el.adjy; x = el.x; }
                        const float vec = x + adjy / rho_f;
                        sx[k] = x; sadjz[k] = adjz; sadjy[k] = adjy; sv[k] = vec; szc[k] = el.zc; syc[k] = el.yc; sxy[k] = el.xy;
                        const double v = (double)vec;
                        nrm2 += v * v;
                    }
                }
            }
        }
    }
    if (c.done) return;

    const double pen = c.lam * wj / c.rho;
    double shrink = 0.0;
    if (m > 1) shrink = tall_block_shrink(nrm2, pen);

    double acc[6] = {0, 0, 0, 0, 0, 0};
    const float tn = (float)c.tau_next, tn1 = (float)(1.0 + c.tau_next);
    const size_t pm = (size_t)q.p * m;
#pragma unroll
    for (int k = 0; k < kMtMax; ++k) {
        if (k < m && owner) {
            const float x = sx[k], adjz = sadjz[k], adjy = sadjy[k], vec = sv[k], zc = szc[k], yc = syc[k], xy = sxy[k];
            const double v = (double)vec;
            float zn;
            if (m == 1) zn = tall_soft(vec, pen);
            else zn = (float)(v * shrink);
            const float r = x - zn;
            const float yn = adjy + rho_f * r;
            const float dz = zn - zc, daz = zn - adjz;
            acc[0] += (double)r * r; acc[1] += (double)dz * dz; acc[2] += (double)daz * daz;
            acc[3] += (double)x * x; acc[4] += (double)zn * zn; acc[5] += (double)yn * yn;
            const size_t o = (size_t)k * mp.ldv + i;
            q.x[o] = x; zo_[o] = zn; yo_[o] = yn; q.adj_z[o] = adjz; q.adj_y[o] = adjy;
            if (q.state != nullptr && c.total < q.state_cap) {
                float* st = q.state + (size_t)c.total * 5 * pm + (size_t)k * q.p + i;
                st[0] = x; st[pm] = zn; st[2 * pm] = yn; st[3 * pm] = adjz; st[4 * pm] = adjy;
            }
            const float adjz_a = tall_extrapolate(tn1, tn, zn, zc), adjy_a = tall_extrapolate(tn1, tn, yn, yc);
            mp.uw[(size_t)(2 * k) * mp.ldv + i] = (float)((double)(xy - adjy_a) + c.rho * (double)adjz_a);
            mp.uw[(size_t)(2 * k + 1) * mp.ldv + i] = (float)((double)(xy - yc) + c.rho * (double)zc);
        }
    }
    tall_publish_norms(q, par, acc, scratch);
}


__global__ void __launch_bounds__(kTailThreads)
tall_shard_reduce_kernel(TallParams q, float* ab, long long ld, const int* skip) {
    if (*skip) return;
    const int sub = threadIdx.x & (kTailLanes - 1);
    const int i = blockIdx.x * kTailElems + threadIdx.x / kTailLanes;
    float a, b;
    symv_sum_partials<kTailLanes>(q.dot0, q.dot1, q.axp0, q.axp1, q.ldo, q.nrb, q.sched, q.p32, i, sub, i < q.p, a, b);
    if (i < q.p && sub == 0) { ab[i] = a; ab[ld + i] = b; }
}

__global__ void __launch_bounds__(kTailThreads)
tall_refine_resid_kernel(TallParams q, const double* d0, const double* d1, const double* x0, const double* x1, float* ru, float* rw, const int* skip) {
    if (*skip) return;
    const int sub = threadIdx.x & (kTailLanes - 1);
    const int i = blockIdx.x * kTailElems + threadIdx.x / kTailLanes;
    double ma, mb;
    symv_sum_partials<kTailLanes, double>(d0, d1, x0, x1, q.ldo, q.nrb, q.sched, q.p32, i, sub, i < q.p, ma, mb);
    if (i < q.p && sub == 0) { ru[i] = (float)((double)q.u[i] - ma); rw[i] = (float)((double)q.w[i] - mb); }
}

__global__ void __launch_bounds__(kTailThreads)
tall_shard_push_kernel(TallParams q, PeerExchange ex, long long ld, const int* skip) {
    if (*skip) return;
    const int sub = threadIdx.x & (kTailLanes - 1);
    const int i = blockIdx.x * kTailElems + threadIdx.x / kTailLanes;
    float a, b;
    symv_sum_partials<kTailLanes>(q.dot0, q.dot1, q.axp0, q.axp1, q.ldo, q.nrb, q.sched, q.p32, i, sub, i < q.p, a, b);
    if (i < q.p) {
        for (int dst = sub; dst < ex.nranks; dst += kTailLanes)
            peer_store_f32x2(reinterpret_cast<float*>(peer_dst_slot(ex, dst)) + 2 * (size_t)i, a, b);
    }
    peer_publish(ex, gridDim.x);
}

__global__ void tall_init_kernel(TallParams q, double rho, double lam0) {
    const int i = blockIdx.x * blockDim.x + threadIdx.x;
    if (i < q.p) {
        q.x[i] = 0.f; q.z0[i] = 0.f; q.z1[i] = 0.f; q.y0[i] = 0.f; q.y1[i] = 0.f;
        q.adj_z[i] = 0.f; q.adj_y[i] = 0.f; q.u[i] = q.XY[i]; q.w[i] = 0.f;
    }
    if (i < 2 * q.nwg * 8) q.P[i] = 0.0;
    if (i == 0) {
        TallCtl c;
        c.rho = rho; c.lam = lam0; c.eps_primal = 0.0; c.eps_dual = 0.0;
        c.adj_a = 1.0; c.adj_c = 9999.0; c.tau = 0.0;
        c.a_next = 0.5 + 0.5 * sqrt(5.0); c.tau_next = 0.0;
        c.mode = 1; c.restart = 0; c.iter = 0; c.lam_idx = 0; c.done = 0; c.first = 1; c.total = 0; c.fin_idx = -1; c.fin_niter = 0; c.pad = 0;
        q.ctl[0] = c; q.ctl[1] = c;
        if (q.verdict != nullptr) q.verdict[kVerdictWords] = 0;
    }
}

static thread_local long long t_early_exits = 0;
long long tall_last_early_exits() { return t_early_exits; }

struct TallPlan final : LassoPlan {
    DeviceData<float> d;
    LassoProblem pb;
    hipStream_t st;
    admm_stats setup_stats{};
    int p = 0, nlam = 0, nwg = 0;
    long long ldp = 0;
    double rho = 0;
    std::vector<double> lam_user, lam_int;
    GemvTPlan pl;
    SymvPlan sy;
    bool use_sym = false;
    bool shard = false;
    bool peer_fused = false;
    bool peer_one = false;
    int exchange_code = 0;
    CommInfo ci;
    DevBuf<float> ab;
    double dist_flops = 0;
    long long ldv = 0;
    DevBuf<float> XY, M, a_part, b_part, x, z0, z1, y0, y1, adj_z, adj_y, u, w, beta;
    DevBuf<int> niter;
    DevBuf<double> P, dlam;
    DevBuf<TallCtl> ctl;
    DevBuf<unsigned long long> verdict;
    bool verdict_on = false, verdict_mid = false;
    unsigned long long run_no = 0;
    TallParams q{};
    bool refine = false;
    DevBuf<float> Mg, rab, ruw;
    DevBuf<double> dD0, dD1, xD0, xD1;
    bool grouped = false, sgl = false;
    DevBuf<int2> gtiles;
    DevBuf<GroupCoord> gcoord;
    DevBuf<double> gl1;
    GroupTailParams gq{};
    int mt = 0;
    int mt_rhs = 2;
    DevBuf<float> uw, mdot, maxp;
    DevBuf<double> roww;
    MtTailParams mq{};
    bool box = false;
    DevBuf<double> bpf;
    DevBuf<float> blo, bhi;
    BoxTailParams bq{};
    BoxClamp clamp;
    PinnedFlag hflag;
#ifdef ADMM_HIP_PROBE
    DevBuf<long long> probe;
#endif
    float* hbeta = nullptr;

    std::vector<hipEvent_t> ev_pool;

    ~TallPlan() override {
        if (hbeta) (void)hipHostFree(hbeta);
        for (auto e : ev_pool) (void)hipEventDestroy(e);
    }

    TallPlan(DeviceData<float>&& data, const LassoProblem& prob, hipStream_t stream) : d(std::move(data)), pb(prob), st(stream) {
        const int n = d.n;
        p = d.p;
        admm_stats& S = setup_stats;
        S.branch = 0;
        S.t_h2d = d.t_h2d; S.t_standardize = d.t_std;
        ldp = round_up(p, 128);

        shard = pb.dist;
        ci = shard ? comm_info() : CommInfo();
        const long long nt = d.n_total > 0 ? d.n_total : n;
        if (d.xy.get()) {
            ADMM_REQUIRE(!shard && d.gram.get() && d.ldgram == ldp, "Gram-form data needs X'X next to X'y");
            XY = std::move(d.xy);
        } else if (pb.penalty == Penalty::MULTITASK) {
            mt = pb.nresp;
            ADMM_REQUIRE(mt >= 1 && mt <= kMtMax && d.nresp == mt && d.Ymt.get() && (int)pb.row_weight.size() == p, "internal: multi-task sizes");
            XY.alloc((size_t)mt * ldp); XY.zero(st);
            for (int k = 0; k < mt; ++k) gemv_t_simple<float>(d.X.get(), d.ldx, n, p, d.Ymt.get() + (size_t)k * d.ldx, XY.get() + (size_t)k * ldp, st);
        } else {
            XY.alloc(ldp); XY.zero(st);
            gemv_t_simple<float>(d.X.get(), d.ldx, n, p, d.Y.get(), XY.get(), st);
            if (shard) allreduce_sum_f32(XY.get(), (size_t)p, st);
        }
        sgl = pb.penalty == Penalty::SGL; grouped = sgl || pb.penalty == Penalty::GROUP; box = pb.penalty == Penalty::BOX;
        ADMM_REQUIRE(pb.penalty == Penalty::PLAIN || (!shard && !opt_on(Opt::REFINE) && (box || !pb.enet) && (mt > 0) == (pb.penalty == Penalty::MULTITASK)),
                     "internal: a penalty other than the Lasso's is the plain single-device tall solver on column data");
        ADMM_REQUIRE(!grouped || ((int)pb.group_start.size() == (int)pb.group_weight.size() + 1 && pb.group_start.back() == p), "internal: group sizes");
        ADMM_REQUIRE((int)pb.l1_weight.size() == (sgl ? p : 0), "internal: l1 weights belong to the sparse-group lasso");
        ADMM_REQUIRE(!box || ((int)pb.box_lower.size() == p && (int)pb.box_upper.size() == p && (int)pb.penalty_factor.size() == p), "internal: box sizes");
        float lambda0 = 0.f;
        switch (pb.penalty) {
        case Penalty::PLAIN: lambda0 = device_absmax<float>(XY.get(), p, st); break;
        case Penalty::GROUP: lambda0 = group_lambda0(); break;
        case Penalty::SGL: lambda0 = sgl_plan_lambda0(); break;
        case Penalty::MULTITASK: lambda0 = mt_lambda0(); break;
        case Penalty::BOX: lambda0 = box_plan_lambda0(); break;
        }
        if (pb.enet) lambda0 = (float)(lambda0 / ((double)(float)pb.alpha + 0.0001));

        nlam = make_path_grid<float>(pb, lambda0, nt, (double)d.scaleY, lam_user, lam_int);

        {
            size_t free_b = 0, total_b = 0;
            ADMM_HIP_CHECK(hipMemGetInfo(&free_b, &total_b));
            free_b += pool_cached_bytes();
            if (opt_set(Opt::TEST_FREE_BYTES)) free_b = (size_t)opt_int(Opt::TEST_FREE_BYTES, 0);
            const bool have_gram = d.gram.get() && d.ldgram == ldp;
            const bool inv64_wanted = p < 4096 || opt_is(Opt::INVERSE, "f64");
            const double mat = (double)ldp * (double)ldp * 4.0;
            const double need = (have_gram ? 0.0 : mat) + (inv64_wanted ? 2.0 * mat : 0.5 * mat) + (opt_on(Opt::REFINE) ? mat : 0.0) +
                                (shard && ci.nranks > 1 ? mat + mat / ci.nranks : 0.0) +
                                (mt ? mt_partial_floats() * 4.0 : 0.0);
            if (need > 0.97 * (double)free_b) {
                char msg[320];
                std::snprintf(msg, sizeof msg, "tall solver: the cached %d x %d inverse and its workspace need %.1f GB, the device has %.1f GB free; "
                              "use $parallel() (row blocks, admm_hip_parlasso) or fewer columns", p, p, need / 1e9, (double)free_b / 1e9);
                throw Error(ADMM_ERR_MEMORY, msg);
            }
        }
        double t0 = now_s();
        const bool gram_given = d.gram.get() && d.ldgram == ldp;
        if (gram_given) {
            M = std::move(d.gram);
            S.t_gram = d.t_gram_tail;
        } else {
            M.alloc((size_t)ldp * ldp); M.zero(st);
            gram_full<float>(d.X.get(), d.ldx, n, p, true, M.get(), ldp, st);
            comm_stream_sync(st);
            S.t_gram = now_s() - t0;
        }
        bool inv64 = p < 4096;
        if (opt_set(Opt::INVERSE)) inv64 = opt_is(Opt::INVERSE, "f64");
        bool dist_factor = shard && ci.nranks > 1 && !inv64 && (p + 127) / 128 >= 2 * ci.nranks && p >= 256;
        if (opt_off(Opt::DIST_FACTOR)) dist_factor = false;

        rho = pb.opts.rho;
        t0 = now_s();
        if (rho <= 0) {
            SymMatVec<float> op(M.get(), ldp, p, st);
            int nmatop = 0;
            DevBuf<float> wsum;
            if (shard && ci.nranks > 1) wsum.alloc(ldp);
            const float ev = lanczos_largest_f32([&](const float* v, float* w_) {
                op(v, w_);
                if (shard && ci.nranks > 1) {
                    ADMM_HIP_CHECK(hipMemcpyAsync(wsum.get(), w_, (size_t)p * sizeof(float), hipMemcpyHostToDevice, st));
                    allreduce_sum_f32(wsum.get(), (size_t)p, st);
                    ADMM_HIP_CHECK(hipMemcpyAsync(w_, wsum.get(), (size_t)p * sizeof(float), hipMemcpyDeviceToHost, st));
                    comm_stream_sync(st);
                    comm_check();
                }
            }, p, &nmatop);
            S.eig_est = ev;
            rho = std::pow((double)ev, 1.0 / 3) * std::pow(lam_int[0], 2.0 / 3);
        }
        S.rho = rho;
        S.t_eigs = now_s() - t0;

        if (shard && ci.nranks > 1 && !gram_given) {
            const double tr0 = now_s();
            if (dist_factor) {
                const int nb128 = (p + 127) / 128, N = ci.nranks;
                const int nown = (nb128 + N - 1) / N;
                const size_t blk = (size_t)128 * ldp, cnt = (size_t)nown * blk;
                DevBuf<float> send((size_t)N * cnt), recv(cnt);
                send.zero(st);
                for (int k = 0; k < nb128; ++k) {
                    const size_t cols = (size_t)std::min(128, (int)ldp - k * 128);
                    ADMM_HIP_CHECK(hipMemcpyAsync(send.get() + ((size_t)(k % N) * nown + k / N) * blk, M.get() + (size_t)k * blk, cols * ldp * sizeof(float),
                                                  hipMemcpyDeviceToDevice, st));
                }
                reduce_scatter_sum_f32(send.get(), recv.get(), cnt, st);
                for (int k = ci.rank; k < nb128; k += N) {
                    const size_t cols = (size_t)std::min(128, (int)ldp - k * 128);
                    ADMM_HIP_CHECK(hipMemcpyAsync(M.get() + (size_t)k * blk, recv.get() + (size_t)(k / N) * blk, cols * ldp * sizeof(float), hipMemcpyDeviceToDevice, st));
                }
            } else {
                allreduce_sum_f32(M.get(), (size_t)ldp * ldp, st);
            }
            comm_stream_sync(st);
            comm_check();
            S.t_gram += now_s() - tr0;
        }

        refine = opt_on(Opt::REFINE) && !shard;
        if (refine) {
            Mg.alloc((size_t)ldp * ldp);
            ADMM_HIP_CHECK(hipMemcpyAsync(Mg.get(), M.get(), (size_t)ldp * ldp * sizeof(float), hipMemcpyDeviceToDevice, st));
            add_diag<float>(Mg.get(), ldp, p, (float)rho, st);
        }
        t0 = now_s();
        if (inv64) {
            spd_inverse_f32_via_f64(M.get(), ldp, p, (double)(float)rho, st);
        } else if (dist_factor) {
            add_diag<float>(M.get(), ldp, p, (float)rho, st);
            sy.init(p, st, ci.rank, ci.nranks);
            std::vector<int> need;
            {
                const int nb128 = (p + 127) / 128;
                std::vector<char> mark((size_t)nb128 * nb128, 0);
                for (const int4& t : sy.htiles)
                    for (int bi = 2 * t.x; bi <= 2 * t.x + 1 && bi < nb128; ++bi)
                        for (int bj = t.y / 128; bj <= (t.y + t.z - 1) / 128 && bj < nb128; ++bj)
                            if (bj <= bi && !mark[(size_t)bi * nb128 + bj]) { mark[(size_t)bi * nb128 + bj] = 1; need.push_back(bi << 16 | bj); }
            }
            double fl = 0;
            spd_inverse_mfma_f32_dist(M.get(), ldp, p, need, &fl, st);
            dist_flops = fl;
        } else {
            add_diag<float>(M.get(), ldp, p, (float)rho, st);
            spd_inverse_f32(M.get(), ldp, p, st);
        }
        comm_stream_sync(st);
        S.t_factor = now_s() - t0;
        d.X.release();

        use_sym = p >= 2048;
        if (opt_set(Opt::XUPDATE)) use_sym = opt_is(Opt::XUPDATE, "sym");
        if (refine) use_sym = true;
        if (shard) use_sym = true;
        if (mt) use_sym = true;
        pl = plan_gemv_t<float>(p, p, 2, 4);
        nwg = (p + kTailElems - 1) / kTailElems;
        if (grouped) nwg = pack_group_tiles();
        ldv = round_up(p, 256);
        if (use_sym) sy.init(p, st, shard ? ci.rank : 0, shard ? ci.nranks : 1);
        if (refine) {
            rab.alloc((size_t)2 * ldv); rab.zero(st);
            ruw.alloc((size_t)2 * ldv); ruw.zero(st);
            dD0.alloc((size_t)sy.nrb * sy.ldo); dD1.alloc((size_t)sy.nrb * sy.ldo);
            xD0.alloc((size_t)sy.nax_rows * sy.ldo); xD1.alloc((size_t)sy.nax_rows * sy.ldo);
            dD0.zero(st); dD1.zero(st); xD0.zero(st); xD1.zero(st);
        }
        if (shard) { ab.alloc((size_t)2 * ldp); ab.zero(st); }
        else if (!use_sym) { a_part.alloc((size_t)pl.nseg * ldp); b_part.alloc((size_t)pl.nseg * ldp); a_part.zero(st); b_part.zero(st); }
        const ExchangeForm xf = peer_exchange_form(shard, ci, reinterpret_cast<const void*>(tall_tail_kernel<TAIL_PEER1>), kTailThreads, nwg);
        peer_fused = xf.fused; peer_one = xf.one; exchange_code = xf.variant;
        const size_t npl = (size_t)std::max(mt, 1);
        x.alloc(npl * ldv); z0.alloc(npl * ldv); z1.alloc(npl * ldv); y0.alloc(npl * ldv); y1.alloc(npl * ldv);
        adj_z.alloc(npl * ldv); adj_y.alloc(npl * ldv); u.alloc(ldv); w.alloc(ldv);
        beta.alloc((size_t)nlam * p * npl); niter.alloc(nlam);
        P.alloc((size_t)2 * nwg * 8); dlam.alloc(nlam); ctl.alloc(2);
        u.zero(st); w.zero(st);
        ADMM_HIP_CHECK(hipMemcpyAsync(dlam.get(), lam_int.data(), nlam * sizeof(double), hipMemcpyHostToDevice, st));

        q.p = p; q.nwg = nwg; q.nseg = pl.nseg; q.maxit = pb.opts.maxit; q.nlam = nlam; q.enet = pb.enet ? 1 : 0;
        q.part_stride = ldp;
        q.eps_abs = pb.opts.eps_abs; q.eps_rel = pb.opts.eps_rel; q.alpha = (double)(float)pb.alpha; q.sqrt_p = std::sqrt((double)p * (double)npl);
        q.lambdas = dlam.get(); q.XY = XY.get(); q.a_part = a_part.get(); q.b_part = b_part.get();
        if (shard) { q.a_part = ab.get(); q.b_part = ab.get() + ldp; q.nseg = 1; }
        q.dot0 = sy.dot0.get(); q.dot1 = sy.dot1.get(); q.axp0 = sy.axp0.get(); q.axp1 = sy.axp1.get();
        q.ldo = sy.ldo; q.nrb = sy.nrb; q.p32 = sy.p32; q.sched = sy.sched;
        q.refine_ab = refine ? rab.get() : nullptr; q.refine_ld = ldv;
        q.x = x.get(); q.z0 = z0.get(); q.z1 = z1.get(); q.y0 = y0.get(); q.y1 = y1.get();
        q.adj_z = adj_z.get(); q.adj_y = adj_y.get(); q.u = u.get(); q.w = w.get();
        q.ctl = ctl.get(); q.P = P.get(); q.beta = beta.get(); q.niter = niter.get();
        q.done_host = hflag.p;
        verdict_on = use_sym && !shard && !refine && !mt && !opt_off(Opt::SYMV_VERDICT);
        verdict_mid = opt_int(Opt::SYMV_VERDICT, 2) == 2;
        if (verdict_on) {
            verdict.alloc(kVerdictWords + kSyVerdictStride); verdict.zero(st);
            q.verdict = verdict.get();
        }
#ifdef ADMM_HIP_PROBE
        probe.alloc((size_t)4096 * 4 * 8); probe.zero(st);
        q.probe = probe.get();
        sy.probe = probe.get();
#endif

        if (mt) {
            static const int kAutoRhs[kMtMax] = {2, 4, 8, 8, 12, 12, 8, 8, 4, 4, 12, 12, 4, 4, 8, 8};
            mt_rhs = kAutoRhs[mt - 1];
            if (const OptValue* v = opt(Opt::MT_RHS)) { if (v->i > 0) mt_rhs = kSyNR[v->i - 1]; }
            uw.alloc((size_t)2 * mt * ldv); uw.zero(st);
            const size_t ds = (size_t)sy.nrb * sy.ldo, as = (size_t)sy.nax_rows * sy.ldo;
            mdot.alloc((size_t)2 * mt * ds); maxp.alloc((size_t)2 * mt * as);
            mdot.zero(st); maxp.zero(st);
            x.zero(st); z0.zero(st); z1.zero(st); y0.zero(st); y1.zero(st); adj_z.zero(st); adj_y.zero(st);
            roww.alloc(p);
            ADMM_HIP_CHECK(hipMemcpyAsync(roww.get(), pb.row_weight.data(), (size_t)p * sizeof(double), hipMemcpyHostToDevice, st));
            mq.m = mt; mq.ldv = ldv; mq.ldxy = ldp; mq.uw = uw.get();
            mq.dot = mdot.get(); mq.axp = maxp.get(); mq.dot_stride = (long long)ds; mq.axp_stride = (long long)as;
            mq.row_w = roww.get();
        }
        ADMM_HIP_CHECK(hipHostMalloc(reinterpret_cast<void**>(&hbeta), (size_t)nlam * p * npl * sizeof(float), hipHostMallocDefault));
        comm_stream_sync(st);
    }

    float box_plan_lambda0() {
        std::vector<float> lo(p), hi(p), h(p);
        for (int j = 0; j < p; ++j) {
            lo[j] = box_round_lower(box_to_std(pb.box_lower[j], (double)d.scaleX[j], (double)d.scaleY));
            hi[j] = box_round_upper(box_to_std(pb.box_upper[j], (double)d.scaleX[j], (double)d.scaleY));
        }
        clamp.set(pb.box_lower, pb.box_upper);
        bpf.alloc((size_t)p); blo.alloc((size_t)p); bhi.alloc((size_t)p);
        ADMM_HIP_CHECK(hipMemcpyAsync(bpf.get(), pb.penalty_factor.data(), (size_t)p * sizeof(double), hipMemcpyHostToDevice, st));
        ADMM_HIP_CHECK(hipMemcpyAsync(blo.get(), lo.data(), (size_t)p * sizeof(float), hipMemcpyHostToDevice, st));
        ADMM_HIP_CHECK(hipMemcpyAsync(bhi.get(), hi.data(), (size_t)p * sizeof(float), hipMemcpyHostToDevice, st));
        read_back(h.data(), XY.get(), (size_t)p * sizeof(float), st);
        bq.pf = bpf.get(); bq.lo = blo.get(); bq.hi = bhi.get();
        return box_lambda0(h.data(), p, lo.data(), hi.data(), pb.penalty_factor.data());
    }

    float mt_lambda0() {
        std::vector<float> h((size_t)mt * ldp);
        read_back(h.data(), XY.get(), h.size() * sizeof(float), st);
        double best = 0.0;
        for (int j = 0; j < p; ++j) {
            if (!(pb.row_weight[j] > 0)) continue;
            double s2 = 0.0;
            for (int k = 0; k < mt; ++k) { const double v = (double)h[(size_t)k * ldp + j]; s2 += v * v; }
            best = std::max(best, std::sqrt(s2) / pb.row_weight[j]);
        }
        return (float)best;
    }
    double mt_partial_floats() const {
        const double nrb = (double)((p + kSyRB - 1) / kSyRB), ldo = nrb * kSyRB;
        return 2.0 * mt * (nrb + (double)((p + 31) / 32)) * ldo;
    }

    float group_lambda0() {
        std::vector<float> h(p);
        read_back(h.data(), XY.get(), (size_t)p * sizeof(float), st);
        double best = 0.0;
        for (size_t g = 0; g + 1 < pb.group_start.size(); ++g) {
            if (!(pb.group_weight[g] > 0)) continue;
            double s2 = 0.0;
            for (int j = pb.group_start[g]; j < pb.group_start[g + 1]; ++j) s2 += (double)h[j] * (double)h[j];
            best = std::max(best, std::sqrt(s2) / pb.group_weight[g]);
        }
        return (float)best;
    }

    float sgl_plan_lambda0() {
        std::vector<float> h(p);
        read_back(h.data(), XY.get(), (size_t)p * sizeof(float), st);
        return sgl_lambda0(h.data(), pb.group_start, pb.l1_weight, pb.group_weight);
    }

    int pack_group_tiles() {
        std::vector<int2> tiles;
        std::vector<GroupCoord> coord(p);
        const bool flat = sgl && std::none_of(pb.group_weight.begin(), pb.group_weight.end(), [](double w) { return w > 0; });
        std::vector<int> each;
        if (flat) for (int j = 0; j <= p; ++j) each.push_back(j);
        const std::vector<int>& start = flat ? each : pb.group_start;
        int first = 0, count = 0;
        const auto flush = [&] { if (count > 0) tiles.push_back(make_int2(first, count)); first += count; count = 0; };
        for (size_t g = 0; g + 1 < start.size(); ++g) {
            const int gs = start[g], gn = start[g + 1] - gs;
            const double wg = flat ? 0.0 : pb.group_weight[g];
            ADMM_REQUIRE(gn >= 1 && gn <= kGroupMax && gs == first + count, "internal: bad group partition");
            for (int j = gs; j < gs + gn; ++j)
                coord[j] = GroupCoord{gs, gn, sgl && gn == 1 ? sgl_single_weight(pb.l1_weight[j], wg) : wg};
            if (count + gn > kTailElems) flush();
            count += gn;
            if (gn > kTailElems) flush();
        }
        flush();
        gtiles.alloc(tiles.size()); gcoord.alloc(coord.size());
        ADMM_HIP_CHECK(hipMemcpyAsync(gtiles.get(), tiles.data(), tiles.size() * sizeof(int2), hipMemcpyHostToDevice, st));
        ADMM_HIP_CHECK(hipMemcpyAsync(gcoord.get(), coord.data(), coord.size() * sizeof(GroupCoord), hipMemcpyHostToDevice, st));
        if (sgl) {
            gl1.alloc((size_t)p);
            ADMM_HIP_CHECK(hipMemcpyAsync(gl1.get(), pb.l1_weight.data(), (size_t)p * sizeof(double), hipMemcpyHostToDevice, st));
        }
        comm_stream_sync(st);
        gq.tiles = gtiles.get(); gq.coord = gcoord.get(); gq.l1 = sgl ? gl1.get() : nullptr;
        return (int)tiles.size();
    }

    Records records() override { return {st, 5ll * p * std::max(mt, 1), &q.trace, &q.trace_cap, &q.state, &q.state_cap}; }

    void read_system(float* out, long long ld) override {
        if (!refine) throw Error(ADMM_ERR_INVALID_ARG, "the system matrix is only kept with ADMM_HIP_REFINE=1");
        ADMM_REQUIRE(out != nullptr && ld >= p, "bad output for the system matrix");
        ADMM_HIP_CHECK(hipMemcpy2D(out, (size_t)ld * sizeof(float), Mg.get(), (size_t)ldp * sizeof(float), (size_t)p * sizeof(float), (size_t)p, hipMemcpyDeviceToHost));
    }

    void run(LassoResult& res) override {
        admm_stats S = setup_stats;
        S.xupdate_variant = shard ? 2 : (use_sym ? 1 : 0);
        S.exchange_variant = exchange_code;
        S.refine = refine ? 1 : 0;
        S.factor_flops = dist_flops;
        res.lambda = lam_user;
        beta.zero(st); niter.zero(st);
        q.run_tag = ++run_no << kVerdictShift;
        const int init_n = std::max(p, 2 * nwg * 8);
        for (int k = 0; k < std::max(mt, 1); ++k) {
            TallParams qk = q;
            if (mt) {
                const size_t o = (size_t)k * ldv;
                qk.x += o; qk.z0 += o; qk.z1 += o; qk.y0 += o; qk.y1 += o; qk.adj_z += o; qk.adj_y += o;
                qk.XY += (size_t)k * ldp; qk.u = uw.get() + (size_t)(2 * k) * ldv; qk.w = uw.get() + (size_t)(2 * k + 1) * ldv;
            }
            hipLaunchKernelGGL(tall_init_kernel, dim3((init_n + 255) / 256), dim3(256), 0, st, qk, rho, lam_int[0]);
        }
        if (q.state != nullptr && mt)
            ADMM_HIP_CHECK(hipMemcpy2DAsync(q.state, (size_t)p * sizeof(float), XY.get(), (size_t)ldp * sizeof(float), (size_t)p * sizeof(float),
                                            (size_t)mt, hipMemcpyDeviceToDevice, st));
        else if (q.state != nullptr)
            ADMM_HIP_CHECK(hipMemcpyAsync(q.state, XY.get(), (size_t)p * sizeof(float), hipMemcpyDeviceToDevice, st));
        *hflag.p = 0;
#ifdef ADMM_HIP_PROBE
        sy.probe_idx = 0;
#endif

        const int batch = batch_iters(pb.batch_iters, 32);
        const int stride = pb.profile_stride;
        size_t nev = 0;
        const auto done_at = [&](long long g) -> const int* { return &ctl.get()[(int)(g & 1)].done; };
        const LoopTimes lt = run_until_done(st, done_at, batch, (long long)nlam * ((long long)pb.opts.maxit + 2) + 4, [&](long long g) {
            const int par = (int)(g & 1);
            const bool sample = stride > 0 && (g % stride) == stride / 2 && nev < 8192;
            hipEvent_t e0 = nullptr, e1 = nullptr;
            if (sample) {
                while (ev_pool.size() < nev + 2) {
                    hipEvent_t e; ADMM_HIP_CHECK(hipEventCreate(&e));
                    ev_pool.push_back(e);
                }
                e0 = ev_pool[nev]; e1 = ev_pool[nev + 1];
                nev += 2;
            }
            const TallDecideExtra dec{q, par};
            SymvVerdict vd;
            if (verdict_on) { vd.words = verdict.get(); vd.discard = tall_verdict_word(q.run_tag, (int)(g + 1), true); vd.early = verdict.get() + kVerdictWords; vd.mid = verdict_mid; }
            const int* skip = &ctl.get()[par].done;
            const auto xupdate = [&] {
                if (use_sym) sy.launch(M.get(), ldp, u.get(), w.get(), skip, st, dec, e0, e1, vd);
                else launch_gemv_t<float, 2, 4, TallDecideExtra>(pl, M.get(), ldp, p, p, u.get(), w.get(), a_part.get(), b_part.get(), ldp, skip, st, dec, e0, e1);
            };
            const auto group_tail = [&] {
                void (*tail)(TallParams, int, GroupTailParams) =
                    use_sym ? (sgl ? tall_group_tail_kernel<TAIL_SYMV, true> : tall_group_tail_kernel<TAIL_SYMV>)
                            : (sgl ? tall_group_tail_kernel<TAIL_GEMV, true> : tall_group_tail_kernel<TAIL_GEMV>);
                hipLaunchKernelGGL(tail, dim3(nwg), dim3(kTailThreads), 0, st, q, par, gq);
            };
            if (mt) {
                const int nvec = 2 * mt;
                for (int r0 = 0; r0 < nvec; r0 += mt_rhs) {
                    SymvNArgs a;
                    a.A = M.get(); a.lda = ldp; a.p = p;
                    a.v = uw.get() + (size_t)r0 * ldv; a.vstride = ldv;
                    a.dot = mdot.get() + (size_t)r0 * mq.dot_stride; a.dot_stride = mq.dot_stride;
                    a.axp = maxp.get() + (size_t)r0 * mq.axp_stride; a.axp_stride = mq.axp_stride;
                    a.nvec = std::min(mt_rhs, nvec - r0); a.ldo = sy.ldo; a.tiles = sy.tiles.get(); a.skip = skip;
                    hipEvent_t es = r0 == 0 ? e0 : nullptr, ee = r0 + mt_rhs >= nvec ? e1 : nullptr;
                    if (r0 == 0) symvn_launch(sy, mt_rhs, a, st, dec, es, ee);
                    else symvn_launch(sy, mt_rhs, a, st, SymvNoExtra(), es, ee);
                }
                hipLaunchKernelGGL(tall_mt_tail_kernel, dim3(nwg), dim3(kTailThreads), 0, st, q, par, mq);
            } else if (grouped) {
                xupdate();
                group_tail();
            } else if (shard && peer_fused) {
                sy.launch(M.get(), ldp, u.get(), w.get(), skip, st, dec, e0, e1);
                const PeerExchange ex = comm_peer_begin((size_t)2 * ldp * sizeof(float));
                if (peer_one) {
                    hipLaunchKernelGGL(tall_tail_kernel<TAIL_PEER1>, dim3(nwg), dim3(kTailThreads), 0, st, q, par, ex);
                } else {
                    hipLaunchKernelGGL(tall_shard_push_kernel, dim3(nwg), dim3(kTailThreads), 0, st, q, ex, ldp, skip);
                    hipLaunchKernelGGL(tall_tail_kernel<TAIL_PEER>, dim3(nwg), dim3(kTailThreads), 0, st, q, par, ex);
                }
            } else if (shard) {
                sy.launch(M.get(), ldp, u.get(), w.get(), skip, st, dec, e0, e1);
                hipLaunchKernelGGL(tall_shard_reduce_kernel, dim3(nwg), dim3(kTailThreads), 0, st, q, ab.get(), ldp, skip);
                allreduce_sum_f32(ab.get(), (size_t)2 * ldp, st);
                hipLaunchKernelGGL(tall_tail_kernel<TAIL_GEMV>, dim3(nwg), dim3(kTailThreads), 0, st, q, par, PeerExchange{});
            } else if (use_sym && refine) {
                sy.launch(M.get(), ldp, u.get(), w.get(), skip, st, dec, e0, e1);
                hipLaunchKernelGGL(tall_shard_reduce_kernel, dim3(nwg), dim3(kTailThreads), 0, st, q, rab.get(), ldv, skip);
                SymvArgsD ad;
                ad.A = Mg.get(); ad.lda = ldp; ad.p = p; ad.v0 = rab.get(); ad.v1 = rab.get() + ldv;
                ad.dot0 = dD0.get(); ad.dot1 = dD1.get(); ad.axp0 = xD0.get(); ad.axp1 = xD1.get(); ad.ldo = sy.ldo; ad.tiles = sy.tiles.get(); ad.skip = skip;
                hipLaunchKernelGGL(symv2_lower_f64acc_kernel, dim3(sy.ntiles), dim3(kSyThreads), 0, st, ad);
                hipLaunchKernelGGL(tall_refine_resid_kernel, dim3(nwg), dim3(kTailThreads), 0, st, q, dD0.get(), dD1.get(), xD0.get(), xD1.get(),
                                   ruw.get(), ruw.get() + ldv, skip);
                sy.launch(M.get(), ldp, ruw.get(), ruw.get() + ldv, skip, st, SymvNoExtra());
                hipLaunchKernelGGL(tall_tail_kernel<TAIL_SYMV>, dim3(nwg), dim3(kTailThreads), 0, st, q, par, PeerExchange{});
            } else if (box) {
                xupdate();
                if (use_sym) hipLaunchKernelGGL(tall_box_tail_kernel<TAIL_SYMV>, dim3(nwg), dim3(kTailThreads), 0, st, q, par, bq);
                else hipLaunchKernelGGL(tall_box_tail_kernel<TAIL_GEMV>, dim3(nwg), dim3(kTailThreads), 0, st, q, par, bq);
            } else {
                xupdate();
                if (use_sym) hipLaunchKernelGGL(tall_tail_kernel<TAIL_SYMV>, dim3(nwg), dim3(kTailThreads), 0, st, q, par, PeerExchange{});
                else hipLaunchKernelGGL(tall_tail_kernel<TAIL_GEMV>, dim3(nwg), dim3(kTailThreads), 0, st, q, par, PeerExchange{});
            }
        }, LoopOpts{shard ? nullptr : hflag.p, 0, false});
        S.t_loop = lt.wall_s; S.loop_ms_events = lt.events_ms; S.xupdate_launches = lt.launched;
        const CtlPair<TallCtl> hctl = read_ctl(ctl.get());
        unsigned long long early = 0;
        if (verdict_on) ADMM_HIP_CHECK(hipMemcpy(&early, verdict.get() + kVerdictWords, sizeof early, hipMemcpyDeviceToHost));
        t_early_exits = (long long)early;
        WIDE_PROBE_DUMP(probe);
        if (nev > 0) {
            double tot = 0;
            for (size_t k = 0; k + 1 < nev; k += 2) {
                float m1 = 0.f;
                ADMM_HIP_CHECK(hipEventElapsedTime(&m1, ev_pool[k], ev_pool[k + 1]));
                tot += m1;
            }
            S.xupdate_samples = (long long)(nev / 2);
            S.xupdate_ms_avg = tot / (double)(nev / 2);
        }

        ADMM_HIP_CHECK(hipMemcpyAsync(hbeta, beta.get(), (size_t)nlam * p * std::max(mt, 1) * sizeof(float), hipMemcpyDeviceToHost, st));
        comm_stream_sync(st);
        if (mt) {
            const size_t col = (size_t)p + 1;
            std::vector<float> bk;
            res.beta.assign(col * mt * nlam, 0.f);
            for (int k = 0; k < mt; ++k) {
                S.total_iter = read_out_path<float>(d, hbeta + (size_t)k * p, nlam, niter.get(), col, 0, res.niter, bk, INT_MAX, (size_t)mt * p, &d.meanYs[k]);
                for (int l = 0; l < nlam; ++l) std::memcpy(res.beta.data() + ((size_t)l * mt + k) * col, bk.data() + (size_t)l * col, col * sizeof(float));
            }
        } else {
            S.total_iter = read_out_path<float>(d, hbeta, nlam, niter.get(), (size_t)p + 1, 0, res.niter, res.beta, INT_MAX, 0, nullptr, &clamp);
        }
        decisions = hctl.c[0].done ? hctl.total() : 0;
        res.stats = S;
    }
};

std::unique_ptr<LassoPlan> make_tall_plan(DeviceData<float>&& d, const LassoProblem& pb, hipStream_t st) {
    return std::unique_ptr<LassoPlan>(new TallPlan(std::move(d), pb, st));
}

}
```

### admm_amd/csrc/options.h

```cpp
#pragma once
#include <limits>
#include <string>
#include <vector>

namespace admm {

enum class OptKind { Flag, Int, Real, Choice, Text, Sched, Devices };
struct OptAccepts {
    OptKind kind;
    double lo = 0, hi = 0;
    const char* choices = nullptr;
};
constexpr OptAccepts Flag() { return {OptKind::Flag, 0, 1}; }
constexpr OptAccepts Int(double lo, double hi) { return {OptKind::Int, lo, hi}; }
constexpr OptAccepts Real(double lo, double hi) { return {OptKind::Real, lo, hi}; }
constexpr OptAccepts Choice(const char* c) { return {OptKind::Choice, 0, 0, c}; }
constexpr OptAccepts Text() { return {OptKind::Text}; }
constexpr OptAccepts Sched() { return {OptKind::Sched}; }
constexpr OptAccepts Devices() { return {OptKind::Devices}; }
constexpr double kPositive = std::numeric_limits<double>::min();

#define ADMM_OPTIONS(X)                                                                                                                  \
    X(BATCH_ITERS, Int(1, 1 << 20), "iterations enqueued between two host polls (rounded up to even; default per solver)")             \
    X(PROFILE_STRIDE, Int(0, 1 << 30), "time every k-th tall x-update launch with HIP events (0: off)")                                 \
    X(GRAM, Choice("rocblas|oneshot"), "tall Gram through rocBLAS / host input transferred before the Gram is built")                    \
    X(GRAM_SPLIT, Choice("0|f16x2|bf16x3"), "tall Gram of order >= ~4000: exact fp32 kernel / fp16 x 2 (default) / bf16 x 3")          \
    X(GRAM_B3_KTILES, Int(0, 1 << 20), "K tiles per launch of the 16-bit split Gram (0: one launch)")                                   \
    X(FACTOR, Choice("rocsolver"), "Cholesky + inverse through rocSOLVER / rocBLAS instead of the hand-written kernels")                \
    X(INVERSE, Choice("f32|f64"), "precision the cached inverse is built in")                                                           \
    X(XUPDATE, Choice("sym|gemv|full"), "tall x-update: symmetric lower-triangle kernel / full-matrix mat-vec (gemv and full alike)")   \
    X(SYMV_SCHED, Sched(), "tall x-update: column-segment widths of the long / short row strips and the split between them")           \
    X(SYMV_VERDICT, Choice("0|1|2"), "tall x-update: tiles of a discarded launch leave never / when they start / also mid-tile (default)") \
    X(REFINE, Flag(), "tall path: refine every x-update with a double-precision residual")                                               \
    X(DIST_FACTOR, Flag(), "row-sharded tall solver: 0 = every rank factorises the whole all-reduced Gram")                            \
    X(CV_DOWNDATE, Flag(), "cross-validation folds' Grams as down-dates of the full-data Gram: 1 always, 0 never")                      \
    X(PREP_FUSED, Flag(), "0: convert, column statistics and standardisation as separate sweeps over X")                                \
    X(H2D, Choice("pageable"), "host inputs through plain hipMemcpy instead of the pinned staging ring")                                 \
    X(POOL_MB, Int(0, 1 << 30), "cache of released device blocks, megabytes (0: off)")                                                  \
    X(WIDE_FUSE, Flag(), "wide path: 0 = three launches per iteration")                                                                  \
    X(WIDE_TGLOBAL, Flag(), "wide path: 1 = t through global memory instead of LDS")                                                     \
    X(WIDE_SPRAD, Choice("gram"), "wide path: spectral radius from the explicit n x n Gram")                                            \
    X(WIDE_SCREEN, Choice("0|8|16|auto"), "wide path: screen the regular steps never / 8-bit code / fp16 copy / chosen at any size")    \
    X(WIDE_SCREEN_STATS, Flag(), "wide path: print the screen's counts")                                                                 \
    X(WIDE_PERSIST, Flag(), "wide path: 0 = no persistent active-set stretches")                                                         \
    X(WIDE_PERSIST_COLS, Flag(), "column-sharded wide solver: 0 = no persistent active-set stretches")                                  \
    X(WIDE_ROWS_C, Int(1, 32), "wide path: column groups of the 2-D stretch (kept only when it fits with the problem's row groups)")    \
    X(WIDE_PERSIST_STATS, Flag(), "wide path: print the stretch statistics")                                                             \
    X(PAR_ONEPASS, Flag(), "consensus solver: 0 = the reference's two products per Woodbury worker")                                    \
    X(PAR_ONEPASS_TAU, Real(0, 1e300), "one-pass Woodbury workers: threshold of the cancellation guard (0: never fall back)")           \
    X(PAR_ONEPASS_STATS, Flag(), "one-pass Woodbury workers: print how many worker-iterations took the dense pass")                     \
    X(PAR_FUSE_PZ, Flag(), "consensus solver: 0 = pack and z as two launches")                                                           \
    X(PAR_BATCH, Flag(), "consensus solver: 0 = one launch per worker and product")                                                      \
    X(PAR_DEVICES, Devices(), "admm_hip_parlasso / admm_hip_parbp over several devices in one process")                                \
    X(TEST_PAR_FAIL_RANK, Int(0, 63), "test hook: this rank of an in-process call fails before its first exchange")                    \
    X(PEER_FUSED, Choice("0|1|2"), "PEER back-end: 0 = the generic all-reduce, 2 = producer and consumer as two launches")             \
    X(PEER_MEM, Choice("uncached"), "PEER exchange buffers as uncached device memory")                                                   \
    X(COMM_SLOT_BYTES, Int(4096, 1ll << 40), "payload capacity of one PEER / SHM exchange (rounded down to 16 bytes)")                 \
    X(COMM_TIMEOUT_S, Real(kPositive, 1e300), "wait bound of the per-iteration exchanges, seconds")                                    \
    X(COMM_PATIENT_TIMEOUT_S, Real(kPositive, 1e300), "wait bound of setup reductions and replica joins, seconds")                     \
    X(LAD_HAT, Flag(), "LAD: 0 = the general projection also for n <= 2000")                                                            \
    X(LAD_ONEPASS, Flag(), "LAD: 0 = the reference's two products per iteration")                                                      \
    X(QUANT_SLOTS, Int(0, 8), "admm_hip_quantreg, admm_hip_huber: fits per pass over X on the one-pass branch: 0 = automatic, 1 = serial, else at most that many") \
    X(MT_RHS, Choice("0|2|4|8|12"), "admm_hip_mtlasso: right-hand sides per pass over the cached inverse (0: automatic)")               \
    X(BP_ONEPASS, Flag(), "basis pursuit: 0 = the reference's two products per iteration")                                             \
    X(SBP_GRAM, Flag(), "admm_hip_parbp: 0 = the direct launches on every active-set iteration")                                       \
    X(SBP_GRAM_CAP, Int(1, 1024), "admm_hip_parbp: most columns of the Gram-space matrix (rounded to multiples of 8)")                 \
    X(SBP_GRAM_CARRY, Flag(), "admm_hip_parbp: 0 = every Gram-space stretch starts from the direct launches' n-vectors")              \
    X(SBP_SCREEN, Flag(), "admm_hip_parbp: screen the regular iterations always / never")                                             \
    X(SBP_SCREEN_STATS, Flag(), "admm_hip_parbp: print the screen's counts")                                                           \
    X(SBP_WGS, Int(1, 1 << 20), "admm_hip_parbp: workgroups of the x-update launches")                                                 \
    X(SBP_SHARE, Int(1, 1 << 20), "admm_hip_parbp: smallest share of a block's non-zero list a workgroup takes")                      \
    X(SBP_TEST_DELAY_US, Int(0, 1000000), "test hook: every even workgroup of a Gram-space launch starts that many us late")           \
    X(TEST_RESIDENT_WGS, Int(0, 1ll << 40), "test hook: pretend the device holds that many resident workgroups")                      \
    X(TEST_FREE_BYTES, Int(0, 1ll << 52), "test hook: pretend the device has that many bytes free")                                    \
    X(PROBE_OUT, Text(), "dev build with in-kernel timestamps (-DADMM_HIP_PROBE): file the probe records go to")

enum class Opt : int {
#define ADMM_OPT_ID(id, accepts, summary) id,
    ADMM_OPTIONS(ADMM_OPT_ID)
#undef ADMM_OPT_ID
};
constexpr int kNumOptions = 0
#define ADMM_OPT_COUNT(id, accepts, summary) +1
    ADMM_OPTIONS(ADMM_OPT_COUNT)
#undef ADMM_OPT_COUNT
    ;

struct OptValue {
    std::string text;
    long long i = 0;
    double r = 0;
    int sched[3] = {0, 0, 0};
};
struct ThreadOptions {
    bool has[kNumOptions] = {};
    OptValue v[kNumOptions];
};

const OptValue* opt(Opt id);
inline bool opt_set(Opt id) { return opt(id) != nullptr; }
inline long long opt_int(Opt id, long long dflt) { const OptValue* v = opt(id); return v ? v->i : dflt; }
inline double opt_real(Opt id, double dflt) { const OptValue* v = opt(id); return v ? v->r : dflt; }
inline const char* opt_text(Opt id) { const OptValue* v = opt(id); return v ? v->text.c_str() : nullptr; }
inline bool opt_on(Opt id) { return opt_int(id, -1) == 1; }
inline bool opt_off(Opt id) { return opt_int(id, -1) == 0; }
bool opt_is(Opt id, const char* choice);

inline int batch_iters(int set, int dflt) { return set > 0 ? (set + 1) / 2 * 2 : dflt; }

bool opt_find(const char* name, Opt* id);
void opt_parse(Opt id, const char* text, OptValue* out);
ThreadOptions& thread_options();
void opt_set_thread(Opt id, const char* value);
void check_option_overlay();
std::vector<int> parse_par_devices(const char* v, int device_count);

}
```

### admm_amd/csrc/symv_kernels.h

```cpp
#pragma once
#include "admm_internal.h"
#include "device_utils.h"
#include <hip/hip_ext.h>
#include <climits>

namespace admm {

constexpr int kSyRB = 256;
constexpr int kSyCB = 128;
constexpr int kSyCBMax = 256;
static_assert(kSyCBMax == 256, "SYMV_SCHED's widths are checked against 256 where the option is parsed (options.hip)");
constexpr int kSyThreads = 256;

struct SymvSched {
    int width_big = kSyCB, width_small = kSyCB;
    int rb_split = 0;
    __host__ __device__ int width(int rb) const { return rb >= rb_split ? width_big : width_small; }
    __host__ __device__ int nseg(int rb, int p32) const {
        const int cols = min((rb + 1) * kSyRB, p32), w = width(rb);
        return (cols + w - 1) / w;
    }
};
constexpr int kSySumLanes = 8;

struct SymvArgs {
    const float* A; long long lda; int p;
    const float* v0; const float* v1;
    float* dot0; float* dot1;
    float* axp0; float* axp1;
    long long ldo;
    const int4* tiles;
    const int* skip;
    const unsigned long long* verdict;
    unsigned long long discard;
    unsigned long long* early;
#ifdef ADMM_HIP_PROBE
    long long* probe; int probe_idx;
#endif
};

constexpr int kSyVerdictReplicas = 64;
constexpr int kSyVerdictStride = 16;
struct SymvVerdict {
    const unsigned long long* words = nullptr;
    unsigned long long discard = 0;
    unsigned long long* early = nullptr;
    bool mid = false;
};

template <typename T>
__device__ __forceinline__ T butterfly8(const T (&v)[8], int lane) {
    T a4[4], a2[2];
    {
        const int b = (lane >> 5) & 1;
#pragma unroll
        for (int k = 0; k < 4; ++k) {
            const T keep = b ? v[k + 4] : v[k], send = b ? v[k] : v[k + 4];
            a4[k] = keep + __shfl_xor(send, 32, 64);
        }
    }
    {
        const int b = (lane >> 4) & 1;
#pragma unroll
        for (int k = 0; k < 2; ++k) {
            const T keep = b ? a4[k + 2] : a4[k], send = b ? a4[k] : a4[k + 2];
            a2[k] = keep + __shfl_xor(send, 16, 64);
        }
    }
    const int b = (lane >> 3) & 1;
    const T keep = b ? a2[1] : a2[0], send = b ? a2[0] : a2[1];
    T r = keep + __shfl_xor(send, 8, 64);
    r += __shfl_xor(r, 4, 64);
    r += __shfl_xor(r, 2, 64);
    r += __shfl_xor(r, 1, 64);
    return r;
}

struct SymvPlainVec {
    __device__ __forceinline__ float4 load4(const float* p) const { return *reinterpret_cast<const float4*>(p); }
    __device__ __forceinline__ float load1(const float* p) const { return *p; }
};
struct SymvBypassVec {
    __device__ __forceinline__ float4 load4(const float* p) const {
        const unsigned long long lo = __hip_atomic_load(reinterpret_cast<const unsigned long long*>(p), __ATOMIC_RELAXED, __HIP_MEMORY_SCOPE_AGENT);
        const unsigned long long hi = __hip_atomic_load(reinterpret_cast<const unsigned long long*>(p) + 1, __ATOMIC_RELAXED, __HIP_MEMORY_SCOPE_AGENT);
        return make_float4(__uint_as_float((unsigned)lo), __uint_as_float((unsigned)(lo >> 32)), __uint_as_float((unsigned)hi), __uint_as_float((unsigned)(hi >> 32)));
    }
    __device__ __forceinline__ float load1(const float* p) const {
        return __uint_as_float(__hip_atomic_load(reinterpret_cast<const unsigned int*>(p), __ATOMIC_RELAXED, __HIP_MEMORY_SCOPE_AGENT));
    }
};
struct SymvNoWait { __device__ __forceinline__ void operator()() const {} };

template <bool PRE, typename Wait, typename VecLoad, bool NT = false, bool MID = false>
__device__ __forceinline__ void symv2_tile(const SymvArgs& a, const int4 t, Wait wait, VecLoad vl,
                                           float4 (*red)[kSyThreads], float (*sdot)[kSyCBMax]) {
    const int rb = t.x, seg = t.w;
    const int cw = t.z >> 2;
    const int lane = threadIdx.x & 63, wid = threadIdx.x >> 6;
    const int row = rb * kSyRB + lane * 4;
    const int col0 = t.y + wid * cw;
    const int p4 = (a.p + 3) & ~3;
    const bool active = row < p4;
    const bool has = col0 < a.p;
    const float* base = a.A + (size_t)col0 * a.lda + row;
    float4 av[8];
    if (PRE) {
#pragma unroll
        for (int k = 0; k < 8; ++k) {
            av[k] = make_float4(0.f, 0.f, 0.f, 0.f);
            if (has && active && col0 + k < a.p) av[k] = *reinterpret_cast<const float4*>(base + (size_t)k * a.lda);
        }
        wait();
    }
    float4 aU = make_float4(0.f, 0.f, 0.f, 0.f), aW = aU;

    if (has) {
        const float4 uI = active ? vl.load4(a.v0 + row) : make_float4(0.f, 0.f, 0.f, 0.f);
        const float4 wI = active ? vl.load4(a.v1 + row) : make_float4(0.f, 0.f, 0.f, 0.f);
        const int cj = col0 + lane;
        const float uj = (lane < cw && cj < a.p) ? vl.load1(a.v0 + cj) : 0.f;
        const float wj = (lane < cw && cj < a.p) ? vl.load1(a.v1 + cj) : 0.f;
        const bool diag = col0 + (cw - 1) >= rb * kSyRB;
        const int nq = cw >> 3;
        const int last = active ? min(a.p - 1, diag ? row + 3 : INT_MAX) : -1;
        const unsigned long long* vword = a.verdict + (size_t)(blockIdx.x & (kSyVerdictReplicas - 1)) * kSyVerdictStride;
#pragma unroll 1
        for (int q = 0; q < nq; ++q) {
            unsigned long long vq = 0;
            if constexpr (MID) vq = __hip_atomic_load(vword, __ATOMIC_RELAXED, __HIP_MEMORY_SCOPE_AGENT);
            if (!PRE || q > 0) {
#pragma unroll
                for (int k = 0; k < 8; ++k) {
                    const int col = col0 + q * 8 + k;
                    av[k] = make_float4(0.f, 0.f, 0.f, 0.f);
                    if constexpr (NT) { if (col <= last) av[k] = load16_nt<float4>(base + (size_t)(q * 8 + k) * a.lda); }
                    else { if (col <= last) av[k] = *reinterpret_cast<const float4*>(base + (size_t)(q * 8 + k) * a.lda); }
                }
            }
            if constexpr (MID) {
                const unsigned lo = __builtin_amdgcn_readfirstlane((unsigned)vq), hi = __builtin_amdgcn_readfirstlane((unsigned)(vq >> 32));
                if ((((unsigned long long)hi << 32) | lo) == a.discard) break;
            }
            float dU[8], dW[8];
#pragma unroll
            for (int k = 0; k < 8; ++k) {
                const int col = col0 + q * 8 + k;
                float4 v = av[k];
                float4 ax = v;
                if (diag) {
                    if (row + 0 < col) v.x = 0.f;
                    if (row + 1 < col) v.y = 0.f;
                    if (row + 2 < col) v.z = 0.f;
                    if (row + 3 < col) v.w = 0.f;
                    ax = v;
                    if (row + 0 == col) ax.x = 0.f;
                    if (row + 1 == col) ax.y = 0.f;
                    if (row + 2 == col) ax.z = 0.f;
                    if (row + 3 == col) ax.w = 0.f;
                }
                dU[k] = fmaf(v.x, uI.x, fmaf(v.y, uI.y, fmaf(v.z, uI.z, v.w * uI.w)));
                dW[k] = fmaf(v.x, wI.x, fmaf(v.y, wI.y, fmaf(v.z, wI.z, v.w * wI.w)));
                const float ujc = __int_as_float(__builtin_amdgcn_readlane(__float_as_int(uj), (q * 8 + k) & 63));
                const float wjc = __int_as_float(__builtin_amdgcn_readlane(__float_as_int(wj), (q * 8 + k) & 63));
                aU.x = fmaf(ax.x, ujc, aU.x); aU.y = fmaf(ax.y, ujc, aU.y); aU.z = fmaf(ax.z, ujc, aU.z); aU.w = fmaf(ax.w, ujc, aU.w);
                aW.x = fmaf(ax.x, wjc, aW.x); aW.y = fmaf(ax.y, wjc, aW.y); aW.z = fmaf(ax.z, wjc, aW.z); aW.w = fmaf(ax.w, wjc, aW.w);
            }
            const float du = butterfly8(dU, lane);
            const float dw = butterfly8(dW, lane);
            if ((lane & 7) == 0) {
                sdot[0][wid * cw + q * 8 + (lane >> 3)] = du;
                sdot[1][wid * cw + q * 8 + (lane >> 3)] = dw;
            }
        }
    } else {
        for (int c = lane; c < cw; c += 64) { sdot[0][wid * cw + c] = 0.f; sdot[1][wid * cw + c] = 0.f; }
    }
    red[0][threadIdx.x] = aU;
    red[1][threadIdx.x] = aW;
    __syncthreads();
    if (wid < 2) {
        float4 s = red[wid][lane];
#pragma unroll
        for (int ww = 1; ww < 4; ++ww) {
            const float4 o = red[wid][ww * 64 + lane];
            s.x += o.x; s.y += o.y; s.z += o.z; s.w += o.w;
        }
        float* dst = (wid == 0 ? a.axp0 : a.axp1) + (size_t)seg * a.ldo + row;
        *reinterpret_cast<float4*>(dst) = s;
    } else {
        float* dst = (wid == 2 ? a.dot0 : a.dot1) + (size_t)rb * a.ldo + t.y;
        for (int c = lane * 4; c < t.z; c += 256) *reinterpret_cast<float4*>(dst + c) = *reinterpret_cast<const float4*>(&sdot[wid - 2][c]);
    }
}

struct SymvNoExtra { __device__ void operator()() const {} };

template <typename Extra, bool NT = false, bool MID = false>
__global__ void __launch_bounds__(kSyThreads, 4)
symv2_lower_kernel(SymvArgs a, Extra extra) {
    if (blockIdx.x == 0) { extra(); return; }
    const int4 t = a.tiles[blockIdx.x - 1];
    const unsigned long long vw = __hip_atomic_load(a.verdict + (size_t)(blockIdx.x & (kSyVerdictReplicas - 1)) * kSyVerdictStride,
                                                    __ATOMIC_RELAXED, __HIP_MEMORY_SCOPE_AGENT);
    const int done = *a.skip;
    if (done != 0) return;
    if (vw == a.discard) {
        if (threadIdx.x == 0) atomicAdd(a.early, 1ull);
        return;
    }
    __shared__ float4 red[2][kSyThreads];
    __shared__ __attribute__((aligned(16))) float sdot[2][kSyCBMax];
#ifdef ADMM_HIP_PROBE
    const long long pt0 = wall_clock64();
#endif
    symv2_tile<false, SymvNoWait, SymvPlainVec, NT, MID>(a, t, SymvNoWait(), SymvPlainVec(), red, sdot);
#ifdef ADMM_HIP_PROBE
    if (a.probe != nullptr && threadIdx.x == 0) {
        const int nt = (int)gridDim.x - 1, t = (int)blockIdx.x - 1;
        const int which = t == 0 ? 0 : (t == nt / 2 ? 1 : (t == nt - 1 ? 2 : (t == (3 * nt) / 4 ? 3 : -1)));
        if (which >= 0) {
            long long* d = a.probe + ((size_t)(a.probe_idx & 4095) * 4 + 3) * 8 + which * 2;
            d[0] = pt0; d[1] = wall_clock64();
        }
    }
#endif
}

struct SymvNArgs {
    const float* A; long long lda; int p;
    const float* v; long long vstride;
    float* dot; long long dot_stride;
    float* axp; long long axp_stride;
    int nvec;
    long long ldo;
    const int4* tiles;
    const int* skip;
};
constexpr int kSyNR[] = {2, 4, 8, 12};
constexpr int kSyNRCount = (int)(sizeof(kSyNR) / sizeof(kSyNR[0]));

template <int NR, bool DIAG>
__device__ __forceinline__ void symvn_chunk(float4 (&av)[8], const float4 (&vI)[NR], const float (&vj)[NR], float4 (&acc)[NR],
                                            int row, int colq, int q, int lane, float (*sdot)[kSyCBMax], int sbase) {
    float4 ax[DIAG ? 8 : 1];
    if (DIAG) {
#pragma unroll
        for (int k = 0; k < 8; ++k) {
            const int col = colq + k;
            float4 v = av[k];
            if (row + 0 < col) v.x = 0.f;
            if (row + 1 < col) v.y = 0.f;
            if (row + 2 < col) v.z = 0.f;
            if (row + 3 < col) v.w = 0.f;
            av[k] = v;
            if (row + 0 == col) v.x = 0.f;
            if (row + 1 == col) v.y = 0.f;
            if (row + 2 == col) v.z = 0.f;
            if (row + 3 == col) v.w = 0.f;
            ax[DIAG ? k : 0] = v;
        }
    }
#pragma unroll
    for (int r = 0; r < NR; ++r) {
        float d[8];
        const float4 xi = vI[r];
        float4 s = acc[r];
#pragma unroll
        for (int k = 0; k < 8; ++k) {
            const float4 v = av[k];
            const float4 x = DIAG ? ax[DIAG ? k : 0] : av[k];
            d[k] = fmaf(v.x, xi.x, fmaf(v.y, xi.y, fmaf(v.z, xi.z, v.w * xi.w)));
            const float c = __int_as_float(__builtin_amdgcn_readlane(__float_as_int(vj[r]), (q * 8 + k) & 63));
            s.x = fmaf(x.x, c, s.x); s.y = fmaf(x.y, c, s.y); s.z = fmaf(x.z, c, s.z); s.w = fmaf(x.w, c, s.w);
        }
        acc[r] = s;
        const float dr = butterfly8(d, lane);
        if ((lane & 7) == 0) sdot[r][sbase + (lane >> 3)] = dr;
    }
}

template <int NR, typename Extra, bool NT = false>
__global__ void __launch_bounds__(kSyThreads, 2)
symvn_lower_kernel(SymvNArgs a, Extra extra) {
    static_assert(NR >= 2 && NR % 2 == 0, "right-hand sides come in pairs (u_k, w_k)");
    if (blockIdx.x == 0) { extra(); return; }
    if (a.skip != nullptr && *a.skip != 0) return;
    __shared__ float4 red[2][kSyThreads];
    __shared__ __attribute__((aligned(16))) float sdot[NR][kSyCBMax];
    const int4 t = a.tiles[blockIdx.x - 1];
    const int rb = t.x, seg = t.w;
    const int cw = t.z >> 2;
    const int lane = threadIdx.x & 63, wid = threadIdx.x >> 6;
    const int row = rb * kSyRB + lane * 4;
    const int col0 = t.y + wid * cw;
    const int p4 = (a.p + 3) & ~3;
    const bool active = row < p4;
    const bool has = col0 < a.p;
    const float* base = a.A + (size_t)col0 * a.lda + row;
    float4 acc[NR];
#pragma unroll
    for (int r = 0; r < NR; ++r) acc[r] = make_float4(0.f, 0.f, 0.f, 0.f);

    if (has) {
        float4 vI[NR];
        float vj[NR];
        const int cj = col0 + lane;
#pragma unroll
        for (int r = 0; r < NR; ++r) {
            const float* vr = a.v + (size_t)min(r, a.nvec - 1) * a.vstride;
            vI[r] = active ? *reinterpret_cast<const float4*>(vr + row) : make_float4(0.f, 0.f, 0.f, 0.f);
            vj[r] = (lane < cw && cj < a.p) ? vr[cj] : 0.f;
        }
        const bool diag = col0 + (cw - 1) >= rb * kSyRB;
        const int nq = cw >> 3;
#pragma unroll 1
        for (int q = 0; q < nq; ++q) {
            float4 av[8];
#pragma unroll
            for (int k = 0; k < 8; ++k) {
                const int col = col0 + q * 8 + k;
                av[k] = make_float4(0.f, 0.f, 0.f, 0.f);
                if constexpr (NT) { if (active && col < a.p) av[k] = load16_nt<float4>(base + (size_t)(q * 8 + k) * a.lda); }
                else { if (active && col < a.p) av[k] = *reinterpret_cast<const float4*>(base + (size_t)(q * 8 + k) * a.lda); }
            }
            if (diag) symvn_chunk<NR, true>(av, vI, vj, acc, row, col0 + q * 8, q, lane, sdot, wid * cw + q * 8);
            else symvn_chunk<NR, false>(av, vI, vj, acc, row, col0 + q * 8, q, lane, sdot, wid * cw + q * 8);
        }
    } else {
#pragma unroll
        for (int r = 0; r < NR; ++r)
            for (int c = lane; c < cw; c += 64) sdot[r][wid * cw + c] = 0.f;
    }
#pragma unroll
    for (int pr = 0; pr < NR / 2; ++pr) {
        if (pr > 0) __syncthreads();
        red[0][threadIdx.x] = acc[2 * pr];
        red[1][threadIdx.x] = acc[2 * pr + 1];
        __syncthreads();
        const int r = 2 * pr + (wid & 1);
        if (r >= a.nvec) continue;
        if (wid < 2) {
            float4 s = red[wid][lane];
#pragma unroll
            for (int ww = 1; ww < 4; ++ww) {
                const float4 o = red[wid][ww * 64 + lane];
                s.x += o.x; s.y += o.y; s.z += o.z; s.w += o.w;
            }
            float* dst = a.axp + (size_t)r * a.axp_stride + (size_t)seg * a.ldo + row;
            *reinterpret_cast<float4*>(dst) = s;
        } else {
            float* dst = a.dot + (size_t)r * a.dot_stride + (size_t)rb * a.ldo + t.y;
            for (int c = lane * 4; c < t.z; c += 256) *reinterpret_cast<float4*>(dst + c) = *reinterpret_cast<const float4*>(&sdot[r][c]);
        }
    }
}

struct SymvArgsD {
    const float* A; long long lda; int p;
    const float* v0; const float* v1;
    double* dot0; double* dot1; double* axp0; double* axp1;
    long long ldo;
    const int4* tiles;
    const int* skip;
};
static __global__ void __launch_bounds__(kSyThreads, 2)
symv2_lower_f64acc_kernel(SymvArgsD a) {
    if (a.skip != nullptr && *a.skip != 0) return;
    __shared__ double4 red[2][kSyThreads];
    __shared__ __attribute__((aligned(16))) double sdot[2][kSyCBMax];
    const int4 t = a.tiles[blockIdx.x];
    const int rb = t.x, seg = t.w, cw = t.z >> 2;
    const int lane = threadIdx.x & 63, wid = threadIdx.x >> 6;
    const int row = rb * kSyRB + lane * 4;
    const int col0 = t.y + wid * cw;
    const int p4 = (a.p + 3) & ~3;
    const bool active = row < p4, has = col0 < a.p;
    const float* base = a.A + (size_t)col0 * a.lda + row;
    double4 aU = make_double4(0, 0, 0, 0), aW = aU;
    if (has) {
        const float4 uI = active ? *reinterpret_cast<const float4*>(a.v0 + row) : make_float4(0.f, 0.f, 0.f, 0.f);
        const float4 wI = active ? *reinterpret_cast<const float4*>(a.v1 + row) : make_float4(0.f, 0.f, 0.f, 0.f);
        const int cj = col0 + lane;
        const float uj = (lane < cw && cj < a.p) ? a.v0[cj] : 0.f;
        const float wj = (lane < cw && cj < a.p) ? a.v1[cj] : 0.f;
        const bool diag = col0 + (cw - 1) >= rb * kSyRB;
        for (int q = 0; q < (cw >> 3); ++q) {
            double dU[8], dW[8];
#pragma unroll
            for (int k = 0; k < 8; ++k) {
                const int col = col0 + q * 8 + k;
                float4 v = make_float4(0.f, 0.f, 0.f, 0.f);
                if (active && col < a.p) v = *reinterpret_cast<const float4*>(base + (size_t)(q * 8 + k) * a.lda);
                float4 ax = v;
                if (diag) {
                    if (row + 0 < col) v.x = 0.f;
                    if (row + 1 < col) v.y = 0.f;
                    if (row + 2 < col) v.z = 0.f;
                    if (row + 3 < col) v.w = 0.f;
                    ax = v;
                    if (row + 0 == col) ax.x = 0.f;
                    if (row + 1 == col) ax.y = 0.f;
                    if (row + 2 == col) ax.z = 0.f;
                    if (row + 3 == col) ax.w = 0.f;
                }
                dU[k] = (double)v.x * uI.x + (double)v.y * uI.y + (double)v.z * uI.z + (double)v.w * uI.w;
                dW[k] = (double)v.x * wI.x + (double)v.y * wI.y + (double)v.z * wI.z + (double)v.w * wI.w;
                const double ujc = (double)__int_as_float(__builtin_amdgcn_readlane(__float_as_int(uj), (q * 8 + k) & 63));
                const double wjc = (double)__int_as_float(__builtin_amdgcn_readlane(__float_as_int(wj), (q * 8 + k) & 63));
                aU.x += ax.x * ujc; aU.y += ax.y * ujc; aU.z += ax.z * ujc; aU.w += ax.w * ujc;
                aW.x += ax.x * wjc; aW.y += ax.y * wjc; aW.z += ax.z * wjc; aW.w += ax.w * wjc;
            }
            const double du = butterfly8(dU, lane), dw = butterfly8(dW, lane);
            if ((lane & 7) == 0) { sdot[0][wid * cw + q * 8 + (lane >> 3)] = du; sdot[1][wid * cw + q * 8 + (lane >> 3)] = dw; }
        }
    } else {
        for (int c = lane; c < cw; c += 64) { sdot[0][wid * cw + c] = 0.0; sdot[1][wid * cw + c] = 0.0; }
    }
    red[0][threadIdx.x] = aU;
    red[1][threadIdx.x] = aW;
    __syncthreads();
    if (wid < 2) {
        double4 s = red[wid][lane];
#pragma unroll
        for (int ww = 1; ww < 4; ++ww) { const double4 o = red[wid][ww * 64 + lane]; s.x += o.x; s.y += o.y; s.z += o.z; s.w += o.w; }
        double* dst = (wid == 0 ? a.axp0 : a.axp1) + (size_t)seg * a.ldo + row;
        dst[0] = s.x; dst[1] = s.y; dst[2] = s.z; dst[3] = s.w;
    } else {
        double* dst = (wid == 2 ? a.dot0 : a.dot1) + (size_t)rb * a.ldo + t.y;
        for (int c = lane; c < t.z; c += 64) dst[c] = sdot[wid - 2][c];
    }
}

struct SymvLayout {
    int p = 0, nrb = 0, ncb = 0, p32 = 0;
    int nax_rows = 0;
    SymvSched sched;
    long long ldo = 0;
    bool nt = false;
    std::vector<int4> tiles;
};

inline SymvLayout symv_plan_layout(int p, int cus, int part, int nparts) {
    SymvLayout L;
    const int p32 = (p + 31) / 32 * 32;
    const int nrb = (p + kSyRB - 1) / kSyRB;
    L.p = p; L.p32 = p32; L.nrb = nrb;
    L.ncb = (p + kSyCB - 1) / kSyCB;
    L.ldo = (long long)nrb * kSyRB;
    SymvSched sched;
    auto count = [&](const SymvSched& sc) { long long t = 0; for (int rb = 0; rb < nrb; ++rb) t += sc.nseg(rb, p32); return t; };
    const long long slots = 4ll * cus * std::max(1, nparts);
    auto uniform = [](int w) { SymvSched sc; sc.width_big = sc.width_small = w; sc.rb_split = 0; return sc; };
    auto two = [&](int wb, int ws) { SymvSched sc; sc.width_big = wb; sc.width_small = ws; sc.rb_split = nrb / 2; return sc; };
    if (4 * count(uniform(32)) <= 3 * slots) sched = uniform(32);
    else if (count(uniform(64)) <= slots) sched = uniform(64);
    else if (10 * count(two(128, 64)) <= 14 * slots) sched = two(128, 64);
    else sched = two(192, 64);
    if (const OptValue* v = opt(Opt::SYMV_SCHED)) {
        sched.width_big = v->sched[0]; sched.width_small = v->sched[1]; sched.rb_split = (int)((long long)v->sched[2] * nrb / 1000);
    }
    std::vector<int4> h;
    int nax_rows = 1;
    for (int rb = nrb - 1; rb >= 0; --rb) {
        const int w = sched.width(rb), ns = sched.nseg(rb, p32);
        nax_rows = std::max(nax_rows, ns);
        for (int sg = 0; sg < ns; ++sg) {
            const int c0 = sg * w;
            const int cols = std::min((rb + 1) * kSyRB, p32);
            h.push_back(make_int4(rb, c0, std::min(w, cols - c0), sg));
        }
    }
    if (nparts > 1) {
        auto gcd = [](int a, int b) { while (b) { const int t = a % b; a = b; b = t; } return a; };
        std::vector<int4> mine;
        int group = -1, last_rb = -1, last_cg = -1;
        for (const int4& t : h) {
            const int w = sched.width(t.x);
            const int gw = w / gcd(w, 128) * 128;
            const int cg = t.y / gw;
            if (t.x != last_rb || cg != last_cg) { ++group; last_rb = t.x; last_cg = cg; }
            if (group % nparts == part) mine.push_back(t);
        }
        h.swap(mine);
    }
    L.nt = (size_t)2 * (size_t)p * (size_t)p / (size_t)std::max(1, nparts) > (size_t)310000000;
    L.sched = sched; L.nax_rows = nax_rows;
    L.tiles.swap(h);
    return L;
}

struct SymvPlan {
    int p = 0, nrb = 0, ncb = 0, ntiles = 0, p32 = 0;
    int nax_rows = 0;
    SymvSched sched;
    long long ldo = 0;
    DevBuf<int4> tiles;
    std::vector<int4> htiles;
    bool nt = false;
    DevBuf<float> dot0, dot1, axp0, axp1;
    DevBuf<unsigned long long> zero;
#ifdef ADMM_HIP_PROBE
    long long* probe = nullptr; mutable int probe_idx = 0;
#endif
    void init(int p_, hipStream_t st, int part = 0, int nparts = 1) {
        int cus = 256;
        { int dev = 0; hipDeviceProp_t prop; if (hipGetDevice(&dev) == hipSuccess && hipGetDeviceProperties(&prop, dev) == hipSuccess) cus = prop.multiProcessorCount; }
        SymvLayout L = symv_plan_layout(p_, cus, part, nparts);
        p = L.p; nrb = L.nrb; ncb = L.ncb; p32 = L.p32; nax_rows = L.nax_rows; sched = L.sched; ldo = L.ldo; nt = L.nt;
        htiles.swap(L.tiles);
        const std::vector<int4>& h = htiles;
        ntiles = (int)h.size();
        tiles.alloc(std::max<size_t>(h.size(), 1));
        if (!h.empty()) ADMM_HIP_CHECK(hipMemcpyAsync(tiles.get(), h.data(), h.size() * sizeof(int4), hipMemcpyHostToDevice, st));
        dot0.alloc((size_t)nrb * ldo); dot1.alloc((size_t)nrb * ldo);
        axp0.alloc((size_t)nax_rows * ldo); axp1.alloc((size_t)nax_rows * ldo);
        dot0.zero(st); dot1.zero(st); axp0.zero(st); axp1.zero(st);
        zero.alloc((size_t)kSyVerdictReplicas * kSyVerdictStride); zero.zero(st);
        ADMM_HIP_CHECK(hipStreamSynchronize(st));
    }
    SymvArgs args(const float* A, long long lda, const float* v0, const float* v1, const int* skip, const SymvVerdict& vd = SymvVerdict()) const {
        SymvArgs a;
        a.A = A; a.lda = lda; a.p = p; a.v0 = v0; a.v1 = v1;
        a.dot0 = dot0.get(); a.dot1 = dot1.get(); a.axp0 = axp0.get(); a.axp1 = axp1.get();
        a.ldo = ldo; a.tiles = tiles.get();
        a.skip = skip != nullptr ? skip : reinterpret_cast<const int*>(zero.get());
        a.verdict = vd.words != nullptr ? vd.words : zero.get();
        a.discard = vd.words != nullptr ? vd.discard : ~0ull;
        a.early = vd.early;
#ifdef ADMM_HIP_PROBE
        a.probe = probe; a.probe_idx = probe_idx++;
#endif
        return a;
    }
    template <typename Extra = SymvNoExtra>
    void launch(const float* A, long long lda, const float* v0, const float* v1, const int* skip, hipStream_t st, Extra extra = Extra(),
                hipEvent_t ev_start = nullptr, hipEvent_t ev_stop = nullptr, const SymvVerdict& vd = SymvVerdict()) {
        const SymvArgs a = args(A, lda, v0, v1, skip, vd);
        if (nt) {
            if (ev_start == nullptr && ev_stop == nullptr) hipLaunchKernelGGL((symv2_lower_kernel<Extra, true>), dim3(ntiles + 1), dim3(kSyThreads), 0, st, a, extra);
            else hipExtLaunchKernelGGL((symv2_lower_kernel<Extra, true>), dim3(ntiles + 1), dim3(kSyThreads), 0, st, ev_start, ev_stop, 0, a, extra);
            return;
        }
        if (vd.words != nullptr && vd.mid) {
            if (ev_start == nullptr && ev_stop == nullptr) hipLaunchKernelGGL((symv2_lower_kernel<Extra, false, true>), dim3(ntiles + 1), dim3(kSyThreads), 0, st, a, extra);
            else hipExtLaunchKernelGGL((symv2_lower_kernel<Extra, false, true>), dim3(ntiles + 1), dim3(kSyThreads), 0, st, ev_start, ev_stop, 0, a, extra);
            return;
        }
        if (ev_start == nullptr && ev_stop == nullptr) hipLaunchKernelGGL((symv2_lower_kernel<Extra>), dim3(ntiles + 1), dim3(kSyThreads), 0, st, a, extra);
        else hipExtLaunchKernelGGL((symv2_lower_kernel<Extra>), dim3(ntiles + 1), dim3(kSyThreads), 0, st, ev_start, ev_stop, 0, a, extra);
    }
};

template <int NL, typename T = float>
__device__ __forceinline__ void symv_sum_partials(const T* __restrict__ dot0, const T* __restrict__ dot1,
                                                  const T* __restrict__ axp0, const T* __restrict__ axp1,
                                                  long long ldo, int nrb, const SymvSched sched, int p32, int i, int sub, bool valid, T& a, T& b) {
    const int ic = valid ? i : 0;
    const int rbi = ic / kSyRB;
    const int rb0 = rbi;
    const int ndot = nrb - rb0;
    const int nax = sched.nseg(rbi, p32);
    const int ntot = valid ? ndot + nax : 0;
    const unsigned ld = (unsigned)ldo;
    a = T(0); b = T(0);
    for (int k0 = 0; k0 < ntot; k0 += 16 * NL) {
        T va[16], vb[16];
#pragma unroll
        for (int j = 0; j < 16; ++j) {
            const int k = k0 + j * NL + sub;
            const bool isdot = k < ndot;
            const int row = isdot ? rb0 + k : min(k, ntot - 1) - ndot;
            const unsigned o = (unsigned)row * ld + (unsigned)ic;
            va[j] = (isdot ? dot0 : axp0)[o];
            vb[j] = (isdot ? dot1 : axp1)[o];
        }
        __builtin_amdgcn_sched_barrier(0);
#pragma unroll
        for (int j = 0; j < 16; ++j) {
            const bool in = k0 + j * NL + sub < ntot;
            a += in ? va[j] : T(0); b += in ? vb[j] : T(0);
        }
    }
#pragma unroll
    for (int m = 1; m < NL; m <<= 1) { a += __shfl_xor(a, m, 64); b += __shfl_xor(b, m, 64); }
}

template <typename Extra>
void symvn_launch(const SymvPlan& sy, int nr, const SymvNArgs& a, hipStream_t st, Extra extra, hipEvent_t ev_start = nullptr, hipEvent_t ev_stop = nullptr) {
    const dim3 grid(sy.ntiles + 1), block(kSyThreads);
    const bool timed = ev_start != nullptr || ev_stop != nullptr;
#define ADMM_SYMVN_LAUNCH(NR, NT)                                                                                                        \
    if (timed) hipExtLaunchKernelGGL((symvn_lower_kernel<NR, Extra, NT>), grid, block, 0, st, ev_start, ev_stop, 0, a, extra);           \
    else hipLaunchKernelGGL((symvn_lower_kernel<NR, Extra, NT>), grid, block, 0, st, a, extra)
#define ADMM_SYMVN_CASE(NR)                                                                                                              \
    case NR:                                                                                                                             \
        if (sy.nt) { ADMM_SYMVN_LAUNCH(NR, true); } else { ADMM_SYMVN_LAUNCH(NR, false); }                                               \
        break;
    switch (nr) {
        ADMM_SYMVN_CASE(2) ADMM_SYMVN_CASE(4) ADMM_SYMVN_CASE(8) ADMM_SYMVN_CASE(12)
        default: throw Error(ADMM_ERR_INTERNAL, "symvn_lower_kernel is not built for that many right-hand sides per pass");
    }
#undef ADMM_SYMVN_CASE
#undef ADMM_SYMVN_LAUNCH
}

constexpr int kMtChunk = 4;
template <int NL, int KB>
__device__ __forceinline__ void symv_sum_partials_n(const float* __restrict__ dot, long long dot_stride, const float* __restrict__ axp, long long axp_stride,
                                                    int npair, long long ldo, int nrb, const SymvSched sched, int p32, int i, int sub, bool valid,
                                                    float (&a)[KB], float (&b)[KB]) {
    const int ic = valid ? i : 0;
    const int rbi = ic / kSyRB;
    const int ndot = nrb - rbi;
    const int nax = sched.nseg(rbi, p32);
    const int ntot = valid ? ndot + nax : 0;
    const unsigned ld = (unsigned)ldo;
#pragma unroll
    for (int k = 0; k < KB; ++k) { a[k] = 0.f; b[k] = 0.f; }
    for (int k0 = 0; k0 < ntot; k0 += 8 * NL) {
        float va[KB][8], vb[KB][8];
#pragma unroll
        for (int k = 0; k < KB; ++k) {
            const int kc = min(k, npair - 1);
            const float* d0 = dot + (size_t)(2 * kc) * dot_stride; const float* d1 = d0 + dot_stride;
            const float* x0 = axp + (size_t)(2 * kc) * axp_stride; const float* x1 = x0 + axp_stride;
#pragma unroll
            for (int j = 0; j < 8; ++j) {
                const int s = k0 + j * NL + sub;
                const bool isdot = s < ndot;
                const int row = isdot ? rbi + s : min(s, ntot - 1) - ndot;
                const unsigned o = (unsigned)row * ld + (unsigned)ic;
                va[k][j] = (isdot ? d0 : x0)[o];
                vb[k][j] = (isdot ? d1 : x1)[o];
            }
        }
        __builtin_amdgcn_sched_barrier(0);
#pragma unroll
        for (int k = 0; k < KB; ++k) {
#pragma unroll
            for (int j = 0; j < 8; ++j) {
                const bool in = k0 + j * NL + sub < ntot && k < npair;
                a[k] += in ? va[k][j] : 0.f; b[k] += in ? vb[k][j] : 0.f;
            }
        }
    }
#pragma unroll
    for (int k = 0; k < KB; ++k) {
#pragma unroll
        for (int m = 1; m < NL; m <<= 1) { a[k] += __shfl_xor(a[k], m, 64); b[k] += __shfl_xor(b[k], m, 64); }
    }
}

}
```

### include/admm_hip.h

```cpp
#ifndef ADMM_HIP_H
#define ADMM_HIP_H

#ifdef __cplusplus
extern "C" {
#endif

#if defined(__GNUC__)
#define ADMM_HIP_API __attribute__((visibility("default")))
#else
#define ADMM_HIP_API
#endif

#define ADMM_OK 0
#define ADMM_ERR_INVALID_ARG 1
#define ADMM_ERR_NO_DEVICE 2
#define ADMM_ERR_HIP 3
#define ADMM_ERR_BLAS 4
#define ADMM_ERR_NOT_SPD 5
#define ADMM_ERR_EIGS 6
#define ADMM_ERR_COMM 7
#define ADMM_ERR_INTERNAL 8
#define ADMM_ERR_MEMORY 9

#define ADMM_MEM_HOST 0
#define ADMM_MEM_DEVICE 1

typedef struct admm_opts {
    int maxit;
    double eps_abs;
    double eps_rel;
    double rho;
} admm_opts;

typedef struct admm_stats {
    double t_h2d;
    double t_standardize;
    double t_gram;
    double t_eigs;
    double t_factor;
    double t_loop;
    double t_total;
    double loop_ms_events;
    double xupdate_ms_avg;
    long long xupdate_samples;
    long long total_iter;
    long long xupdate_launches;
    double rho;
    double eig_est;
    int branch;
    int xupdate_variant;
    int exchange_variant;
    int refine;
    long long persist_iter;
    double factor_flops;
} admm_stats;

ADMM_HIP_API int admm_hip_lasso(const double* x, const double* y, int n, int p, int mem,
                   const double* lambda_in, int nlambda_in, int nlambda_auto, double lmin_ratio,
                   int standardize, int intercept, const admm_opts* opts,
                   double* lambda_out, float* beta_out, int* niter_out, admm_stats* stats);

ADMM_HIP_API int admm_hip_enet(const double* x, const double* y, int n, int p, int mem,
                  const double* lambda_in, int nlambda_in, int nlambda_auto, double lmin_ratio,
                  int standardize, int intercept, double alpha, const admm_opts* opts,
                  double* lambda_out, float* beta_out, int* niter_out, admm_stats* stats);

ADMM_HIP_API int admm_hip_lasso_cv(const double* x, const double* y, int n, int p, int mem, const int* fold_id, int nfolds,
                      const double* lambda_in, int nlambda_in, int nlambda_auto, double lmin_ratio,
                      int standardize, int intercept, double alpha, const admm_opts* opts,
                      double* lambda_out, float* beta_out, int* niter_out,
                      double* cv_mean, double* cv_se, double* fold_mse, int* fold_niter, float* fold_beta,
                      int* idx_min, int* idx_1se, admm_stats* stats);

ADMM_HIP_API int admm_hip_lasso_multi(const double* x, const double* Y, int n, int p, int m, int mem,
                         const double* lambda_in, int nlambda_in, int nlambda_auto, double lmin_ratio,
                         int standardize, int intercept, double alpha, const admm_opts* opts,
                         double* lambda_out, float* beta_out, int* niter_out, admm_stats* stats);

ADMM_HIP_API int admm_hip_parlasso(const double* x, const double* y, int n, int p, int mem,
                      const double* lambda_in, int nlambda_in, int nlambda_auto, double lmin_ratio,
                      int standardize, int intercept, int nthread, const admm_opts* opts,
                      double* lambda_out, float* beta_out, int* niter_out, admm_stats* stats);

ADMM_HIP_API int admm_hip_lad(const double* x, const double* y, int n, int p, int mem, int intercept,
                 const admm_opts* opts, double* beta_out, int* niter_out, admm_stats* stats);

ADMM_HIP_API int admm_hip_bp(const double* x, const double* y, int n, int p, int mem,
                const admm_opts* opts, double* beta_out, int* niter_out, admm_stats* stats);

ADMM_HIP_API int admm_hip_dantzig(const double* x, const double* y, int n, int p, int mem,
                                  const double* lambda_in, int nlambda_in, int nlambda_auto, double lmin_ratio,
                                  int standardize, int intercept, const admm_opts* opts,
                                  double* lambda_out, double* beta_out, int* niter_out, admm_stats* stats);
ADMM_HIP_API int admm_hip_dantzig_traced(const double* x, const double* y, int n, int p, int mem,
                                         const double* lambda_in, int nlambda_in, int nlambda_auto, double lmin_ratio,
                                         int standardize, int intercept, const admm_opts* opts,
                                         double* lambda_out, double* beta_out, int* niter_out, admm_stats* stats,
                                         double* trace_out, long long trace_cap, long long* ntrace_out);

ADMM_HIP_API int admm_hip_parbp(const double* x, const double* y, int n, int p, int mem, int nthread, const admm_opts* opts,
                                double* beta_out, int* niter_out, admm_stats* stats);
ADMM_HIP_API int admm_hip_parbp_traced(const double* x, const double* y, int n, int p, int mem, int nthread, const admm_opts* opts,
                                       double* beta_out, int* niter_out, admm_stats* stats,
                                       double* trace_out, long long trace_cap, long long* ntrace_out);
ADMM_HIP_API int admm_hip_parbp_dist(const double* x_cols, const double* y, int n, int p_local, long long p_total, long long col_offset,
                                     int mem, int nthread, const admm_opts* opts, double* beta_local_out, int* niter_out,
                                     admm_stats* stats);

ADMM_HIP_API int admm_hip_lad_traced(const double* x, const double* y, int n, int p, int mem, int intercept, const admm_opts* opts,
                        double* beta_out, int* niter_out, admm_stats* stats, double* trace_out, long long trace_cap, long long* ntrace_out);
ADMM_HIP_API int admm_hip_bp_traced(const double* x, const double* y, int n, int p, int mem, const admm_opts* opts,
                       double* beta_out, int* niter_out, admm_stats* stats, double* trace_out, long long trace_cap, long long* ntrace_out);

ADMM_HIP_API int admm_hip_lad_state(const double* x, const double* y, int n, int p, int mem, int intercept, const admm_opts* opts,
                       double* beta_out, int* niter_out, admm_stats* stats, double* trace_out, long long trace_cap, long long* ntrace_out,
                       double* state_out, long long state_cap, long long* nstate_out);
ADMM_HIP_API int admm_hip_bp_state(const double* x, const double* y, int n, int p, int mem, const admm_opts* opts,
                      double* beta_out, int* niter_out, admm_stats* stats, double* trace_out, long long trace_cap, long long* ntrace_out,
                      double* state_out, long long state_cap, long long* nstate_out);

ADMM_HIP_API int admm_hip_quantreg(const double* x, const double* y, int n, int p, int mem, int intercept, const double* tau, int ntau,
                      const admm_opts* opts, double* beta_out, int* niter_out, admm_stats* stats);
ADMM_HIP_API int admm_hip_quantreg_state(const double* x, const double* y, int n, int p, int mem, int intercept, double tau, const admm_opts* opts,
                            double* beta_out, int* niter_out, admm_stats* stats, double* trace_out, long long trace_cap, long long* ntrace_out,
                            double* state_out, long long state_cap, long long* nstate_out);

ADMM_HIP_API int admm_hip_huber(const double* x, const double* y, int n, int p, int mem, int intercept, const double* delta, const double* tau, int nfit,
                   const admm_opts* opts, double* beta_out, int* niter_out, admm_stats* stats);
ADMM_HIP_API int admm_hip_huber_state(const double* x, const double* y, int n, int p, int mem, int intercept, double delta, double tau, const admm_opts* opts,
                         double* beta_out, int* niter_out, admm_stats* stats, double* trace_out, long long trace_cap, long long* ntrace_out,
                         double* state_out, long long state_cap, long long* nstate_out);

typedef struct admm_hip_plan admm_hip_plan;
ADMM_HIP_API int admm_hip_lasso_plan_create(const double* x, const double* y, int n, int p, int mem,
                               const double* lambda_in, int nlambda_in, int nlambda_auto, double lmin_ratio,
                               int standardize, int intercept, double alpha, int nthread, const admm_opts* opts,
                               admm_hip_plan** plan_out, int* nlambda_out);
ADMM_HIP_API int admm_hip_lasso_plan_run(admm_hip_plan* plan, double* lambda_out, float* beta_out, int* niter_out, admm_stats* stats);
ADMM_HIP_API int admm_hip_lasso_plan_destroy(admm_hip_plan* plan);

#define ADMM_HIP_GROUP_MAX 1024
ADMM_HIP_API int admm_hip_grplasso(const double* x, const double* y, int n, int p, int mem,
                                   const int* group, const double* group_weight, int ngroups,
                                   const double* lambda_in, int nlambda_in, int nlambda_auto, double lmin_ratio,
                                   int standardize, int intercept, const admm_opts* opts,
                                   double* lambda_out, float* beta_out, int* niter_out, admm_stats* stats);
ADMM_HIP_API int admm_hip_grplasso_plan_create(const double* x, const double* y, int n, int p, int mem,
                                               const int* group, const double* group_weight, int ngroups,
                                               const double* lambda_in, int nlambda_in, int nlambda_auto, double lmin_ratio,
                                               int standardize, int intercept, const admm_opts* opts,
                                               admm_hip_plan** plan_out, int* nlambda_out);

ADMM_HIP_API int admm_hip_sgl(const double* x, const double* y, int n, int p, int mem,
                              const int* group, const double* group_weight, int ngroups, const double* l1_weight, double alpha,
                              const double* lambda_in, int nlambda_in, int nlambda_auto, double lmin_ratio,
                              int standardize, int intercept, const admm_opts* opts,
                              double* lambda_out, float* beta_out, int* niter_out, admm_stats* stats);
ADMM_HIP_API int admm_hip_sgl_plan_create(const double* x, const double* y, int n, int p, int mem,
                                          const int* group, const double* group_weight, int ngroups, const double* l1_weight, double alpha,
                                          const double* lambda_in, int nlambda_in, int nlambda_auto, double lmin_ratio,
                                          int standardize, int intercept, const admm_opts* opts,
                                          admm_hip_plan** plan_out, int* nlambda_out);

ADMM_HIP_API int admm_hip_boxenet(const double* x, const double* y, int n, int p, int mem,
                                  const double* lower, const double* upper, const double* penalty_factor, double alpha,
                                  const double* lambda_in, int nlambda_in, int nlambda_auto, double lmin_ratio,
                                  int standardize, int intercept, const admm_opts* opts,
                                  double* lambda_out, float* beta_out, int* niter_out, admm_stats* stats);
ADMM_HIP_API int admm_hip_boxenet_plan_create(const double* x, const double* y, int n, int p, int mem,
                                              const double* lower, const double* upper, const double* penalty_factor, double alpha,
                                              const double* lambda_in, int nlambda_in, int nlambda_auto, double lmin_ratio,
                                              int standardize, int intercept, const admm_opts* opts,
                                              admm_hip_plan** plan_out, int* nlambda_out);

#define ADMM_HIP_MT_MAX 16
ADMM_HIP_API int admm_hip_mtlasso(const double* x, const double* Y, int n, int p, int m, int mem,
                                  const double* row_weight,
                                  const double* lambda_in, int nlambda_in, int nlambda_auto, double lmin_ratio,
                                  int standardize, int intercept, const admm_opts* opts,
                                  double* lambda_out, float* beta_out, int* niter_out, admm_stats* stats);
ADMM_HIP_API int admm_hip_mtlasso_plan_create(const double* x, const double* Y, int n, int p, int m, int mem,
                                              const double* row_weight,
                                              const double* lambda_in, int nlambda_in, int nlambda_auto, double lmin_ratio,
                                              int standardize, int intercept, const admm_opts* opts,
                                              admm_hip_plan** plan_out, int* nlambda_out);

#define ADMM_TRACE_FIELDS 12
#define ADMM_TRACE_COLD (-1)
#define ADMM_TRACE_CONVERGED 0
#define ADMM_TRACE_ACCELERATE 1
#define ADMM_TRACE_RESTART 2
#define ADMM_TRACE_CONTINUE 1
ADMM_HIP_API int admm_hip_lasso_plan_trace_enable(admm_hip_plan* plan, long long capacity_records);
ADMM_HIP_API int admm_hip_lasso_plan_trace_read(admm_hip_plan* plan, double* out, long long cap_records, long long* nrecords_out);
ADMM_HIP_API int admm_hip_lasso_plan_system_read(admm_hip_plan* plan, float* out, long long ld);
ADMM_HIP_API int admm_hip_lasso_plan_data_read(admm_hip_plan* plan, float* x_out, long long ld, float* y_out);
ADMM_HIP_API int admm_hip_lasso_plan_state_enable(admm_hip_plan* plan, long long capacity_records);
ADMM_HIP_API int admm_hip_lasso_plan_state_read(admm_hip_plan* plan, float* out, long long cap_records, long long* nrecords_out,
                                                long long* record_floats_out);

typedef struct admm_hip_options {
    int struct_size;
    int gram_backend;
    int gram_split;
    int factor_backend;
    int inverse_precision;
    int tall_xupdate;
    int tall_refine;
    int consensus_two_pass;
    int consensus_unfused;
    int bp_two_pass;
    int lad_no_hat;
    int wide_no_persist;
    int wide_unfused;
    int wide_gram_sprad;
    int sharing_bp_direct;
    int cv_downdate;
    int peer_exchange;
    int batch_iters;
    int profile_stride;
    int pool_mb;
    int screen;
    int lad_two_pass;
    int par_devices;
    int reserved[9];
} admm_hip_options;
ADMM_HIP_API int admm_hip_options_default(admm_hip_options* o);
ADMM_HIP_API int admm_hip_options_set(const admm_hip_options* o);
ADMM_HIP_API int admm_hip_option_set(const char* name, const char* value);
ADMM_HIP_API int admm_hip_options_reset(void);
ADMM_HIP_API const char* admm_hip_option_get(const char* name);

#define ADMM_HIP_UNIQUE_ID_BYTES 128
ADMM_HIP_API int admm_hip_comm_unique_id(void* id_out);
ADMM_HIP_API int admm_hip_comm_init(int nranks, int rank, const void* id);
ADMM_HIP_API int admm_hip_comm_finalize(void);
ADMM_HIP_API int admm_hip_comm_info(int* nranks_out, int* rank_out, int* backend_out);
#define ADMM_HIP_PEER_HANDLE_BYTES 64
ADMM_HIP_API int admm_hip_comm_peer_prepare(int nranks, void* handle_out);
ADMM_HIP_API int admm_hip_comm_init_peer(int nranks, int rank, const void* handles_all_ranks);
ADMM_HIP_API int admm_hip_comm_init_shm(int nranks, int rank, const char* name, unsigned long long token);
ADMM_HIP_API int admm_hip_comm_test_allreduce(float* fbuf, long long nf, double* dbuf, long long nd, int mem);
ADMM_HIP_API int admm_hip_comm_test_reduce_scatter(const float* send, long long count, float* recv);
ADMM_HIP_API int admm_hip_parlasso_dist(const double* x_local, const double* y_local, int n_local, long long n_total, int p, int mem,
                           const double* lambda_in, int nlambda_in, int nlambda_auto, double lmin_ratio,
                           int standardize, int intercept, int nthread, const admm_opts* opts,
                           double* lambda_out, float* beta_out, int* niter_out, admm_stats* stats);
ADMM_HIP_API int admm_hip_lasso_plan_create_dist(const double* x_local, const double* y_local, int n_local, long long n_total, int p, int mem,
                                    const double* lambda_in, int nlambda_in, int nlambda_auto, double lmin_ratio,
                                    int standardize, int intercept, int nthread, const admm_opts* opts,
                                    admm_hip_plan** plan_out, int* nlambda_out);
ADMM_HIP_API int admm_hip_lasso_dist(const double* x_local, const double* y_local, int n_local, long long n_total, int p, int mem,
                        const double* lambda_in, int nlambda_in, int nlambda_auto, double lmin_ratio,
                        int standardize, int intercept, double alpha, const admm_opts* opts,
                        double* lambda_out, float* beta_out, int* niter_out, admm_stats* stats);

ADMM_HIP_API int admm_hip_lasso_dist_cols(const double* x_cols, const double* y, int n, int p_local, long long p_total, long long col_offset, int mem,
                             const double* lambda_in, int nlambda_in, int nlambda_auto, double lmin_ratio,
                             int standardize, int intercept, double alpha, const admm_opts* opts,
                             double* lambda_out, float* beta_out, int* niter_out, admm_stats* stats);

ADMM_HIP_API int admm_hip_lasso_plan_create_dist_cols(const double* x_cols, const double* y, int n, int p_local, long long p_total, long long col_offset, int mem,
                                         const double* lambda_in, int nlambda_in, int nlambda_auto, double lmin_ratio,
                                         int standardize, int intercept, double alpha, const admm_opts* opts,
                                         admm_hip_plan** plan_out, int* nlambda_out);

ADMM_HIP_API int admm_hip_last_parallel_layout(int* nranks, int* devices, int cap);
ADMM_HIP_API int admm_hip_parallel_assign(int nblocks, const char* par_devices, int device_count, int* nranks, int* devices, int cap);

ADMM_HIP_API const char* admm_hip_last_error(void);
ADMM_HIP_API const char* admm_hip_version(void);
ADMM_HIP_API int admm_hip_trim_memory(void);
ADMM_HIP_API int admm_hip_device_count(void);
ADMM_HIP_API int admm_hip_set_device(int device);
ADMM_HIP_API int admm_hip_device_synchronize(void);



ADMM_HIP_API int admm_hip_host_lanczos(const float* A, int n, float* eig_out, int* nmatop_out);

ADMM_HIP_API int admm_hip_host_sgl_lambda0(const float* xy, int p, const int* group, const double* group_weight, int ngroups,
                                           const double* l1_weight, double alpha, float* out);

ADMM_HIP_API int admm_hip_host_box_lambda0(const float* xy, int p, const float* lower_std, const float* upper_std,
                                           const double* penalty_factor, double alpha, float* out);

ADMM_HIP_API int admm_hip_test_symv(const float* A, int p, const float* v0, const float* v1, float* y0, float* y1);
ADMM_HIP_API int admm_hip_test_symv_multi(const float* A, int p, const float* V, int nr, int rhs_per_pass, float* Yout);
ADMM_HIP_API int admm_hip_test_symv_plan(int p, int cus, int part, int nparts, int* sched_out, long long* info_out, int* tiles_out,
                                         int tile_capacity);
ADMM_HIP_API int admm_hip_test_symv_ex(const float* A, int p, const float* v0, const float* v1, int variant, int part, int nparts,
                                       float* y0, float* y1, int* sched_out);
ADMM_HIP_API int admm_hip_test_symv_multi_ex(const float* A, int p, const float* V, int nr, int rhs_per_pass, int nt, int finish,
                                             float* Yout, int* sched_out);
ADMM_HIP_API int admm_hip_test_symv_f64acc(const float* A, int p, const float* v0, const float* v1, double* y0, double* y1, int* sched_out);
ADMM_HIP_API int admm_hip_test_tall_early_exits(long long* count);

ADMM_HIP_API int admm_hip_test_gram(const void* A, int rows, int cols, int atA, int is_double, void* G);
ADMM_HIP_API int admm_hip_test_gemv_t(const void* A, int rows, int cols, int is_double, const void* v, void* y);
ADMM_HIP_API int admm_hip_test_gather(const void* A, int rows, int cols, int is_double, const void* v, double* y);
ADMM_HIP_API int admm_hip_test_spd_inverse(const void* A, int n, int precision, void* Ainv);
ADMM_HIP_API int admm_hip_test_spd_inverse_shift(const float* A, int n, double diag, float* Ainv);
ADMM_HIP_API int admm_hip_test_cholesky_linvt(int is_double, const void* A, int n, void* L, void* U);
ADMM_HIP_API int admm_hip_test_gemm_nt(int is_double, int lower, int mirror, int kstart_row, int b_lower, int in_place, int M, int N, int K,
                                       double alpha, double beta, const void* A, const void* B, void* C);
ADMM_HIP_API int admm_hip_test_cv_fold_system(const double* x, const double* y, int n, int p, const int* fold_id, int nfolds, int fold,
                                              int standardize, int intercept, float* gram, float* xy, float* mean_x, float* scale_x,
                                              float* mean_scale_y);

#ifdef __cplusplus
}
#endif
#endif
```

Before: 25680 iterations/s.

## Decide restart/converge inside symv tiles and compute only one matrix-vector product

Adds a single-RHS symmetric matvec kernel in which every tile first re-derives the ADMM decision (converged, accelerate or restart) from compact norm partials. It then multiplies only the one vector that will be used, instead of computing both the accelerated and restart products and picking one afterward. Tiles leave early when the solve has converged. This roughly halves FLOPs on the dominant Gram-matrix matvec and shrinks the gather of partials, at the cost of redundant per-tile norm reductions and extra partial storage. The new path becomes the default verdict level.

```diff
diff --git a/admm_amd/_lib.py b/admm_amd/_lib.py
--- a/admm_amd/_lib.py
+++ b/admm_amd/_lib.py
@@ -72,7 +72,8 @@
            "admm_hip_sgl", "admm_hip_sgl_plan_create", "admm_hip_host_sgl_lambda0",
            "admm_hip_boxenet", "admm_hip_boxenet_plan_create", "admm_hip_host_box_lambda0",
            "admm_hip_test_gemm_nt", "admm_hip_test_cholesky_linvt", "admm_hip_test_spd_inverse_shift",
-           "admm_hip_test_symv_plan", "admm_hip_test_symv_ex", "admm_hip_test_symv_multi_ex", "admm_hip_test_symv_f64acc"]
+           "admm_hip_test_symv_plan", "admm_hip_test_symv_ex", "admm_hip_test_symv_multi_ex", "admm_hip_test_symv_f64acc",
+           "admm_hip_test_symv_one"]
 
 GROUP_MAX = 1024
 MT_MAX = 16
@@ -244,6 +245,9 @@
     lib.admm_hip_test_symv_ex.argtypes = [_c_float_p, ctypes.c_int, _c_float_p, _c_float_p, ctypes.c_int, ctypes.c_int, ctypes.c_int,
                                           _c_float_p, _c_float_p, _c_int_p]
     lib.admm_hip_test_symv_ex.restype = ctypes.c_int
+    lib.admm_hip_test_symv_one.argtypes = [_c_float_p, ctypes.c_int, _c_float_p, _c_float_p, ctypes.c_int, ctypes.c_int, ctypes.c_uint,
+                                           _c_float_p, _c_float_p, _c_float_p, ctypes.c_longlong, ctypes.POINTER(ctypes.c_longlong), _c_int_p]
+    lib.admm_hip_test_symv_one.restype = ctypes.c_int
     lib.admm_hip_test_symv_multi_ex.argtypes = [_c_float_p, ctypes.c_int, _c_float_p, ctypes.c_int, ctypes.c_int, ctypes.c_int, ctypes.c_int,
                                                 _c_float_p, _c_int_p]
     lib.admm_hip_test_symv_multi_ex.restype = ctypes.c_int
diff --git a/admm_amd/csrc/api.hip b/admm_amd/csrc/api.hip
--- a/admm_amd/csrc/api.hip
+++ b/admm_amd/csrc/api.hip
@@ -610,6 +610,17 @@
     });
 }
 
+int admm_hip_test_symv_one(const float* A, int p, const float* v0, const float* v1, int gate, int nt, unsigned int fill, float* y,
+                           float* dot_out, float* axp_out, long long plane_capacity, long long* info_out, int* sched_out) {
+    return guarded([&] {
+        ADMM_REQUIRE(A && v0 && v1 && y && info_out && sched_out, "symv_one hook: A, v0, v1, y, info_out and sched_out must not be NULL");
+        ADMM_REQUIRE((dot_out == nullptr) == (axp_out == nullptr), "symv_one hook: dot_out and axp_out are given together or not at all");
+        ADMM_REQUIRE(p >= 1 && p <= kSymvHookMaxP && gate >= 0 && gate <= 3 && (nt == 0 || nt == 1) && plane_capacity >= 0,
+                     "symv_one hook: p in 1 .. 32768, gate in 0 .. 3, nt 0 or 1, plane_capacity >= 0");
+        test_symv_one(A, p, v0, v1, gate, nt, fill, y, dot_out, axp_out, plane_capacity, info_out, sched_out);
+    });
+}
+
 int admm_hip_test_symv_multi_ex(const float* A, int p, const float* V, int nr, int rhs_per_pass, int nt, int finish, float* Yout, int* sched_out) {
     return guarded([&] {
         ADMM_REQUIRE(A && V && Yout && sched_out, "symv_multi_ex hook: A, V, Yout and sched_out must not be NULL");
diff --git a/admm_amd/csrc/lasso_tall.hip b/admm_amd/csrc/lasso_tall.hip
--- a/admm_amd/csrc/lasso_tall.hip
+++ b/admm_amd/csrc/lasso_tall.hip
@@ -52,6 +52,7 @@
     float* state;
     long long state_cap;
     unsigned long long* verdict;
+    unsigned long long* early;
     unsigned long long run_tag;
 };
 
@@ -62,6 +63,9 @@
 constexpr int kVerdictWords = kSyVerdictReplicas * kSyVerdictStride;
 
 constexpr int kTailThreads = 256;
+constexpr int kGateCols = 3;
+__host__ __device__ inline const double* tall_norm_rows(const double* P, int nwg, int par) { return P + (size_t)par * nwg * 8; }
+__host__ __device__ inline size_t tall_norm_compact(int nwg, int par) { return (size_t)2 * nwg * 8 + (size_t)par * kGateCols * nwg; }
 constexpr int kTailLanes = kSySumLanes;
 constexpr int kTailElems = kTailThreads / kTailLanes;
 
@@ -75,6 +79,88 @@
 __device__ __forceinline__ void tall_store_wt(double* p, double v) {
     __hip_atomic_store(reinterpret_cast<unsigned long long*>(p), (unsigned long long)__double_as_longlong(v), __ATOMIC_RELAXED, __HIP_MEMORY_SCOPE_AGENT);
 }
+
+enum { TALL_COLD = 0, TALL_CONVERGED = 1, TALL_ACCELERATE = 2, TALL_RESTART = 3 };
+struct TallOutcome {
+    int code;
+    int fin;
+    int done;
+    double rp, rd, c;
+    __device__ __forceinline__ bool discard() const { return code == TALL_CONVERGED || done != 0; }
+    __device__ __forceinline__ int pick() const { return code == TALL_RESTART ? 1 : 0; }
+};
+
+template <int NK> struct TallNormReq { double v[2][NK]; };
+template <int NK, bool IN_LAUNCH>
+__device__ __forceinline__ TallNormReq<NK> tall_norms_request(const double* Pin, int nwg, int rs, int cs) {
+    TallNormReq<NK> r;
+#pragma unroll
+    for (int j = 0; j < 2; ++j) {
+        const int w = threadIdx.x + j * kTailThreads;
+#pragma unroll
+        for (int k = 0; k < NK; ++k) r.v[j][k] = w < nwg ? tall_load_partial(Pin + (size_t)w * rs + (size_t)k * cs, IN_LAUNCH) : 0.0;
+    }
+    return r;
+}
+template <int NK, bool IN_LAUNCH>
+__device__ __forceinline__ void tall_norms_sum(const TallNormReq<NK>& r, const double* Pin, int nwg, int rs, int cs, double (&acc)[NK], double* scratch) {
+#pragma unroll
+    for (int k = 0; k < NK; ++k) acc[k] = 0;
+#pragma unroll
+    for (int j = 0; j < 2; ++j) {
+        if ((int)threadIdx.x + j * kTailThreads < nwg) {
+#pragma unroll
+            for (int k = 0; k < NK; ++k) acc[k] += r.v[j][k];
+        }
+    }
+    for (int w = threadIdx.x + 2 * kTailThreads; w < nwg; w += kTailThreads) {
+#pragma unroll
+        for (int k = 0; k < NK; ++k) acc[k] += tall_load_partial(Pin + (size_t)w * rs + (size_t)k * cs, IN_LAUNCH);
+    }
+    block_sum<double, NK>(acc, scratch);
+}
+
+__device__ __forceinline__ TallOutcome tall_outcome(const TallCtl& in, double r2, double dz2, double daz2, int maxit, int nlam) {
+#pragma clang fp contract(off)
+    TallOutcome o;
+    o.code = TALL_COLD; o.fin = 0; o.done = 0; o.rp = 0; o.rd = 0; o.c = 0;
+    if (in.first) return o;
+    const double rp = sqrt(r2);
+    const double rd = in.rho * sqrt(dz2);
+    o.rp = rp; o.rd = rd;
+    if (rp < in.eps_primal && rd < in.eps_dual) {
+        o.code = TALL_CONVERGED; o.fin = 1;
+    } else {
+        const double c = fma(in.rho * rp, rp, in.rho * daz2);
+        o.c = c;
+        o.code = c < 0.999 * in.adj_c ? TALL_ACCELERATE : TALL_RESTART;
+        if (in.iter + 1 >= maxit) o.fin = 1;
+    }
+    if (o.fin && in.lam_idx + 1 >= nlam) o.done = 1;
+    return o;
+}
+
+struct TallGate {
+    const TallCtl* ctl;
+    const double* Pin;
+    int nwg, maxit, nlam;
+    struct Req { TallCtl in; TallNormReq<kGateCols> n; };
+    __device__ __forceinline__ Req request() const {
+        Req r;
+        r.in = *ctl;
+        r.n = tall_norms_request<kGateCols, false>(Pin, nwg, 1, nwg);
+        return r;
+    }
+    __device__ __forceinline__ int decide(const Req& r, double* lds) const {
+        if (r.in.done) return kSyGateLeave;
+        double acc[kGateCols];
+        tall_norms_sum<kGateCols, false>(r.n, Pin, nwg, 1, nwg, acc, lds);
+        const TallOutcome o = tall_outcome(r.in, acc[0], acc[1], acc[2], maxit, nlam);
+        return o.discard() ? kSyGateLeave : o.pick();
+    }
+};
+static_assert(kSyThreads == kTailThreads, "the tiles and the deciding workgroup share the decision rule: one thread <-> partial mapping");
+static_assert(kSyGateScratch >= 6 * (kTailThreads / 64), "block_sum's scratch");
 
 template <bool IN_LAUNCH = false>
 __device__ void tall_decide(const TallParams& q, int par) {
@@ -88,34 +174,29 @@
         return;
     }
     WIDE_PROBE(1);
-    double acc[6] = {0, 0, 0, 0, 0, 0};
-    const double* Pin = q.P + (size_t)par * q.nwg * 8;
-    for (int w = threadIdx.x; w < q.nwg; w += kTailThreads) {
-#pragma unroll
-        for (int k = 0; k < 6; ++k) acc[k] += tall_load_partial(Pin + (size_t)w * 8 + k, IN_LAUNCH);
-    }
-    block_sum<double, 6>(acc, dscratch);
+    double acc[6];
+    const double* Pin = tall_norm_rows(q.P, q.nwg, par);
+    tall_norms_sum<6, IN_LAUNCH>(tall_norms_request<6, IN_LAUNCH>(Pin, q.nwg, 8, 1), Pin, q.nwg, 8, 1, acc, dscratch);
     if (threadIdx.x != 0) return;
     WIDE_PROBE(2);
-    const double r2 = acc[0], dz2 = acc[1], daz2 = acc[2], x2 = acc[3], z2 = acc[4], y2 = acc[5];
-    double tr_rp = 0, tr_rd = 0, tr_c = 0, tr_code = ADMM_TRACE_COLD;
+    const double x2 = acc[3], z2 = acc[4], y2 = acc[5];
+    const TallOutcome oc = tall_outcome(in, acc[0], acc[1], acc[2], q.maxit, q.nlam);
+    const double tr_rp = oc.rp, tr_rd = oc.rd, tr_c = oc.c;
+    double tr_code = ADMM_TRACE_COLD;
     TallCtl out = in;
     out.first = 0;
     out.fin_idx = -1; out.fin_niter = 0;
-    if (!in.first) {
-        const double rp = sqrt(r2);
-        const double rd = in.rho * sqrt(dz2);
-        tr_rp = rp; tr_rd = rd;
-        if (rp < in.eps_primal && rd < in.eps_dual) {
+    if (oc.code == TALL_COLD) {
+        out.mode = 1; out.tau = 0.0; out.restart = 0;
+    } else {
+        if (oc.code == TALL_CONVERGED) {
             out.fin_idx = in.lam_idx; out.fin_niter = in.iter + 1;
             out.mode = 0;
             tr_code = ADMM_TRACE_CONVERGED;
         } else {
             const double old_c = in.adj_c;
-            const double c = in.rho * rp * rp + in.rho * daz2;
-            tr_c = c;
-            if (c < 0.999 * old_c) {
-                out.adj_a = in.a_next; out.adj_c = c; out.tau = in.tau_next; out.restart = 0;
+            if (oc.code == TALL_ACCELERATE) {
+                out.adj_a = in.a_next; out.adj_c = oc.c; out.tau = in.tau_next; out.restart = 0;
                 tr_code = ADMM_TRACE_ACCELERATE;
             } else {
                 out.adj_a = 1.0; out.adj_c = old_c / 0.999; out.tau = -1.0; out.restart = 1;
@@ -123,21 +204,19 @@
             }
             out.mode = 1;
             out.iter = in.iter + 1;
-            if (in.iter + 1 >= q.maxit) {
+            if (oc.fin) {
                 out.fin_idx = in.lam_idx; out.fin_niter = q.maxit + 1;
             }
         }
         if (out.fin_idx >= 0) {
             out.lam_idx = in.lam_idx + 1;
             out.iter = 0;
-            if (out.lam_idx >= q.nlam) out.done = 1;
+            if (oc.done) out.done = 1;
             else out.lam = q.lambdas[out.lam_idx];
             q.niter[out.fin_idx] = out.fin_niter;
         }
-    } else {
-        out.mode = 1; out.tau = 0.0; out.restart = 0;
-    }
-    if (q.verdict != nullptr && (out.mode == 0 || out.done)) {
+    }
+    if (q.verdict != nullptr && oc.discard()) {
         const unsigned long long word = tall_verdict_word(q.run_tag, in.total + 1, true);
         for (int r = 0; r < kSyVerdictReplicas; ++r)
             __hip_atomic_store(q.verdict + (size_t)r * kSyVerdictStride, word, __ATOMIC_RELAXED, __HIP_MEMORY_SCOPE_AGENT);
@@ -247,10 +326,11 @@
         double sum = 0;
         for (int ww = 0; ww < kTailThreads / 64; ++ww) sum += scratch[threadIdx.x * (kTailThreads / 64) + ww];
         q.P[((size_t)(par ^ 1) * q.nwg + blockIdx.x) * 8 + threadIdx.x] = sum;
-    }
-}
-
-enum { TAIL_GEMV = 0, TAIL_SYMV = 1, TAIL_PEER = 2, TAIL_PEER1 = 3 };
+        if (threadIdx.x < kGateCols) q.P[tall_norm_compact(q.nwg, par ^ 1) + (size_t)threadIdx.x * q.nwg + blockIdx.x] = sum;
+    }
+}
+
+enum { TAIL_GEMV = 0, TAIL_SYMV = 1, TAIL_PEER = 2, TAIL_PEER1 = 3, TAIL_SYMV1 = 4 };
 
 __device__ __forceinline__ void tall_lane_sum(float& a, float& b) {
 #pragma unroll
@@ -261,6 +341,10 @@
 __device__ __forceinline__ void tall_gather_ab(const TallParams& q, int i, int sub, bool valid, float& a, float& b) {
     if (MODE == TAIL_SYMV) {
         symv_sum_partials<kTailLanes>(q.dot0, q.dot1, q.axp0, q.axp1, q.ldo, q.nrb, q.sched, q.p32, i, sub, valid, a, b);
+        return;
+    }
+    if (MODE == TAIL_SYMV1) {
+        a = b = symv_sum_partials1<kTailLanes>(q.dot0, q.axp0, q.ldo, q.nrb, q.sched, q.p32, i, sub, valid);
         return;
     }
     a = 0.f; b = 0.f;
@@ -337,7 +421,7 @@
 __global__ void __launch_bounds__(kTailThreads)
 tall_group_tail_kernel(TallParams q, int par, GroupTailParams gp) {
 #pragma clang fp contract(off)
-    static_assert(MODE == TAIL_GEMV || MODE == TAIL_SYMV, "single device");
+    static_assert(MODE == TAIL_GEMV || MODE == TAIL_SYMV || MODE == TAIL_SYMV1, "single device");
     __shared__ double scratch[6 * (kTailThreads / 64)];
     __shared__ double snrm[kTailElems];
     __shared__ float sx[kGroupMax], sadjz[kGroupMax], sadjy[kGroupMax], sv[kGroupMax], szc[kGroupMax], syc[kGroupMax], sxy[kGroupMax];
@@ -437,7 +521,7 @@
 __global__ void __launch_bounds__(kTailThreads)
 tall_box_tail_kernel(TallParams q, int par, BoxTailParams bp) {
 #pragma clang fp contract(off)
-    static_assert(MODE == TAIL_GEMV || MODE == TAIL_SYMV, "single device");
+    static_assert(MODE == TAIL_GEMV || MODE == TAIL_SYMV || MODE == TAIL_SYMV1, "single device");
     __shared__ double scratch[6 * (kTailThreads / 64)];
     const TallCtl c = q.ctl[par ^ 1];
     const int sub = threadIdx.x & (kTailLanes - 1);
@@ -650,7 +734,7 @@
         q.x[i] = 0.f; q.z0[i] = 0.f; q.z1[i] = 0.f; q.y0[i] = 0.f; q.y1[i] = 0.f;
         q.adj_z[i] = 0.f; q.adj_y[i] = 0.f; q.u[i] = q.XY[i]; q.w[i] = 0.f;
     }
-    if (i < 2 * q.nwg * 8) q.P[i] = 0.0;
+    if (i < 2 * q.nwg * (8 + kGateCols)) q.P[i] = 0.0;
     if (i == 0) {
         TallCtl c;
         c.rho = rho; c.lam = lam0; c.eps_primal = 0.0; c.eps_dual = 0.0;
@@ -658,7 +742,8 @@
         c.a_next = 0.5 + 0.5 * sqrt(5.0); c.tau_next = 0.0;
         c.mode = 1; c.restart = 0; c.iter = 0; c.lam_idx = 0; c.done = 0; c.first = 1; c.total = 0; c.fin_idx = -1; c.fin_niter = 0; c.pad = 0;
         q.ctl[0] = c; q.ctl[1] = c;
-        if (q.verdict != nullptr) q.verdict[kVerdictWords] = 0;
+        if (q.early != nullptr)
+            for (int k = 0; k < kSyEarlySlots; ++k) q.early[(size_t)k * kSyVerdictStride] = 0;
     }
 }
 
@@ -691,6 +776,7 @@
     DevBuf<TallCtl> ctl;
     DevBuf<unsigned long long> verdict;
     bool verdict_on = false, verdict_mid = false;
+    bool decide_first = false;
     unsigned long long run_no = 0;
     TallParams q{};
     bool refine = false;
@@ -906,7 +992,7 @@
         x.alloc(npl * ldv); z0.alloc(npl * ldv); z1.alloc(npl * ldv); y0.alloc(npl * ldv); y1.alloc(npl * ldv);
         adj_z.alloc(npl * ldv); adj_y.alloc(npl * ldv); u.alloc(ldv); w.alloc(ldv);
         beta.alloc((size_t)nlam * p * npl); niter.alloc(nlam);
-        P.alloc((size_t)2 * nwg * 8); dlam.alloc(nlam); ctl.alloc(2);
+        P.alloc((size_t)2 * nwg * (8 + kGateCols)); dlam.alloc(nlam); ctl.alloc(2);
         u.zero(st); w.zero(st);
         ADMM_HIP_CHECK(hipMemcpyAsync(dlam.get(), lam_int.data(), nlam * sizeof(double), hipMemcpyHostToDevice, st));
 
@@ -922,11 +1008,14 @@
         q.adj_z = adj_z.get(); q.adj_y = adj_y.get(); q.u = u.get(); q.w = w.get();
         q.ctl = ctl.get(); q.P = P.get(); q.beta = beta.get(); q.niter = niter.get();
         q.done_host = hflag.p;
-        verdict_on = use_sym && !shard && !refine && !mt && !opt_off(Opt::SYMV_VERDICT);
-        verdict_mid = opt_int(Opt::SYMV_VERDICT, 2) == 2;
+        const int level = (int)opt_int(Opt::SYMV_VERDICT, 3);
+        verdict_on = use_sym && !shard && !refine && !mt && level != 0;
+        decide_first = verdict_on && level == 3;
+        verdict_mid = level == 2;
         if (verdict_on) {
-            verdict.alloc(kVerdictWords + kSyVerdictStride); verdict.zero(st);
-            q.verdict = verdict.get();
+            verdict.alloc(kVerdictWords + kSyEarlySlots * kSyVerdictStride); verdict.zero(st);
+            q.verdict = decide_first ? nullptr : verdict.get();
+            q.early = verdict.get() + kVerdictWords;
         }
 #ifdef ADMM_HIP_PROBE
         probe.alloc((size_t)4096 * 4 * 8); probe.zero(st);
@@ -1054,7 +1143,7 @@
         res.lambda = lam_user;
         beta.zero(st); niter.zero(st);
         q.run_tag = ++run_no << kVerdictShift;
-        const int init_n = std::max(p, 2 * nwg * 8);
+        const int init_n = std::max(p, 2 * nwg * (8 + kGateCols));
         for (int k = 0; k < std::max(mt, 1); ++k) {
             TallParams qk = q;
             if (mt) {
@@ -1092,15 +1181,20 @@
             }
             const TallDecideExtra dec{q, par};
             SymvVerdict vd;
-            if (verdict_on) { vd.words = verdict.get(); vd.discard = tall_verdict_word(q.run_tag, (int)(g + 1), true); vd.early = verdict.get() + kVerdictWords; vd.mid = verdict_mid; }
+            if (verdict_on && !decide_first) { vd.words = verdict.get(); vd.discard = tall_verdict_word(q.run_tag, (int)(g + 1), true); vd.early = verdict.get() + kVerdictWords; vd.mid = verdict_mid; }
             const int* skip = &ctl.get()[par].done;
             const auto xupdate = [&] {
-                if (use_sym) sy.launch(M.get(), ldp, u.get(), w.get(), skip, st, dec, e0, e1, vd);
+                if (decide_first) {
+                    const TallGate gate{ctl.get() + par, P.get() + tall_norm_compact(nwg, par), nwg, q.maxit, q.nlam};
+                    sy.launch_one(M.get(), ldp, u.get(), w.get(), skip, st, gate, q.early, dec, e0, e1);
+                }
+                else if (use_sym) sy.launch(M.get(), ldp, u.get(), w.get(), skip, st, dec, e0, e1, vd);
                 else launch_gemv_t<float, 2, 4, TallDecideExtra>(pl, M.get(), ldp, p, p, u.get(), w.get(), a_part.get(), b_part.get(), ldp, skip, st, dec, e0, e1);
             };
             const auto group_tail = [&] {
                 void (*tail)(TallParams, int, GroupTailParams) =
-                    use_sym ? (sgl ? tall_group_tail_kernel<TAIL_SYMV, true> : tall_group_tail_kernel<TAIL_SYMV>)
+                    decide_first ? (sgl ? tall_group_tail_kernel<TAIL_SYMV1, true> : tall_group_tail_kernel<TAIL_SYMV1>)
+                    : use_sym ? (sgl ? tall_group_tail_kernel<TAIL_SYMV, true> : tall_group_tail_kernel<TAIL_SYMV>)
                             : (sgl ? tall_group_tail_kernel<TAIL_GEMV, true> : tall_group_tail_kernel<TAIL_GEMV>);
                 hipLaunchKernelGGL(tail, dim3(nwg), dim3(kTailThreads), 0, st, q, par, gq);
             };
@@ -1148,18 +1242,24 @@
                 hipLaunchKernelGGL(tall_tail_kernel<TAIL_SYMV>, dim3(nwg), dim3(kTailThreads), 0, st, q, par, PeerExchange{});
             } else if (box) {
                 xupdate();
-                if (use_sym) hipLaunchKernelGGL(tall_box_tail_kernel<TAIL_SYMV>, dim3(nwg), dim3(kTailThreads), 0, st, q, par, bq);
+                if (decide_first) hipLaunchKernelGGL(tall_box_tail_kernel<TAIL_SYMV1>, dim3(nwg), dim3(kTailThreads), 0, st, q, par, bq);
+                else if (use_sym) hipLaunchKernelGGL(tall_box_tail_kernel<TAIL_SYMV>, dim3(nwg), dim3(kTailThreads), 0, st, q, par, bq);
                 else hipLaunchKernelGGL(tall_box_tail_kernel<TAIL_GEMV>, dim3(nwg), dim3(kTailThreads), 0, st, q, par, bq);
             } else {
                 xupdate();
-                if (use_sym) hipLaunchKernelGGL(tall_tail_kernel<TAIL_SYMV>, dim3(nwg), dim3(kTailThreads), 0, st, q, par, PeerExchange{});
+                if (decide_first) hipLaunchKernelGGL(tall_tail_kernel<TAIL_SYMV1>, dim3(nwg), dim3(kTailThreads), 0, st, q, par, PeerExchange{});
+                else if (use_sym) hipLaunchKernelGGL(tall_tail_kernel<TAIL_SYMV>, dim3(nwg), dim3(kTailThreads), 0, st, q, par, PeerExchange{});
                 else hipLaunchKernelGGL(tall_tail_kernel<TAIL_GEMV>, dim3(nwg), dim3(kTailThreads), 0, st, q, par, PeerExchange{});
             }
         }, LoopOpts{shard ? nullptr : hflag.p, 0, false});
         S.t_loop = lt.wall_s; S.loop_ms_events = lt.events_ms; S.xupdate_launches = lt.launched;
         const CtlPair<TallCtl> hctl = read_ctl(ctl.get());
         unsigned long long early = 0;
-        if (verdict_on) ADMM_HIP_CHECK(hipMemcpy(&early, verdict.get() + kVerdictWords, sizeof early, hipMemcpyDeviceToHost));
+        if (verdict_on) {
+            std::vector<unsigned long long> slots((size_t)kSyEarlySlots * kSyVerdictStride);
+            ADMM_HIP_CHECK(hipMemcpy(slots.data(), verdict.get() + kVerdictWords, slots.size() * sizeof(unsigned long long), hipMemcpyDeviceToHost));
+            for (int k = 0; k < kSyEarlySlots; ++k) early += slots[(size_t)k * kSyVerdictStride];
+        }
         t_early_exits = (long long)early;
         WIDE_PROBE_DUMP(probe);
         if (nev > 0) {
diff --git a/admm_amd/csrc/options.h b/admm_amd/csrc/options.h
--- a/admm_amd/csrc/options.h
+++ b/admm_amd/csrc/options.h
@@ -30,7 +30,7 @@
     X(INVERSE, Choice("f32|f64"), "precision the cached inverse is built in")                                                           \
     X(XUPDATE, Choice("sym|gemv|full"), "tall x-update: symmetric lower-triangle kernel / full-matrix mat-vec (gemv and full alike)")   \
     X(SYMV_SCHED, Sched(), "tall x-update: column-segment widths of the long / short row strips and the split between them")           \
-    X(SYMV_VERDICT, Choice("0|1|2"), "tall x-update: tiles of a discarded launch leave never / when they start / also mid-tile (default)") \
+    X(SYMV_VERDICT, Choice("0|1|2|3"), "tall x-update: discarded launches stream on / leave on block 0's word at start / also mid-tile / every tile decides first, one vector (default)") \
     X(REFINE, Flag(), "tall path: refine every x-update with a double-precision residual")                                               \
     X(DIST_FACTOR, Flag(), "row-sharded tall solver: 0 = every rank factorises the whole all-reduced Gram")                            \
     X(CV_DOWNDATE, Flag(), "cross-validation folds' Grams as down-dates of the full-data Gram: 1 always, 0 never")                      \
diff --git a/admm_amd/csrc/symv_kernels.h b/admm_amd/csrc/symv_kernels.h
--- a/admm_amd/csrc/symv_kernels.h
+++ b/admm_amd/csrc/symv_kernels.h
@@ -3,6 +3,7 @@
 #include "device_utils.h"
 #include <hip/hip_ext.h>
 #include <climits>
+#include <type_traits>
 
 namespace admm {
 
@@ -219,6 +220,132 @@
     if (a.probe != nullptr && threadIdx.x == 0) {
         const int nt = (int)gridDim.x - 1, t = (int)blockIdx.x - 1;
         const int which = t == 0 ? 0 : (t == nt / 2 ? 1 : (t == nt - 1 ? 2 : (t == (3 * nt) / 4 ? 3 : -1)));
+        if (which >= 0) {
+            long long* d = a.probe + ((size_t)(a.probe_idx & 4095) * 4 + 3) * 8 + which * 2;
+            d[0] = pt0; d[1] = wall_clock64();
+        }
+    }
+#endif
+}
+
+constexpr int kSyGateLeave = -1;
+constexpr int kSyEarlySlots = kSyVerdictReplicas;
+constexpr int kSyGateScratch = 6 * (kSyThreads / 64);
+struct SymvForcedGate {
+    struct Req {};
+    int answer;
+    __device__ __forceinline__ Req request() const { return Req(); }
+    __device__ __forceinline__ int decide(const Req&, double*) const { return answer; }
+};
+#ifndef ADMM_HIP_SYMV1_WGS
+#define ADMM_HIP_SYMV1_WGS 4
+#endif
+#ifndef ADMM_HIP_SYMV1_PRE
+#define ADMM_HIP_SYMV1_PRE 8
+#endif
+
+template <typename Gate, typename Extra, bool NT = false, int PRE = ADMM_HIP_SYMV1_PRE>
+__global__ void __launch_bounds__(kSyThreads, ADMM_HIP_SYMV1_WGS)
+symv1_lower_kernel(SymvArgs a, Gate gate, Extra extra) {
+    if (blockIdx.x == 0) { extra(); return; }
+    __shared__ float4 red[kSyThreads];
+    __shared__ __attribute__((aligned(16))) float sdot[kSyCBMax];
+    __shared__ double gate_lds[kSyGateScratch];
+    const int4 t = a.tiles[blockIdx.x - 1];
+    const int done = *a.skip;
+    const typename Gate::Req greq = gate.request();
+    if (done != 0) return;
+    const int rb = t.x, seg = t.w;
+    const int cw = t.z >> 2;
+    const int lane = threadIdx.x & 63, wid = threadIdx.x >> 6;
+    const int row = rb * kSyRB + lane * 4;
+    const int col0 = t.y + wid * cw;
+    const int p4 = (a.p + 3) & ~3;
+    const bool active = row < p4;
+    const bool has = col0 < a.p;
+    const float* base = a.A + (size_t)col0 * a.lda + row;
+    const bool diag = col0 + (cw - 1) >= rb * kSyRB;
+    const int nq = has ? cw >> 3 : 0;
+    const int last = active ? min(a.p - 1, diag ? row + 3 : INT_MAX) : -1;
+    float4 av[8];
+    const auto request = [&](int q, auto k0, auto k1) {
+#pragma unroll
+        for (int k = decltype(k0)::value; k < decltype(k1)::value; ++k) {
+            const int col = col0 + q * 8 + k;
+            av[k] = make_float4(0.f, 0.f, 0.f, 0.f);
+            if constexpr (NT) { if (col <= last) av[k] = load16_nt<float4>(base + (size_t)(q * 8 + k) * a.lda); }
+            else { if (col <= last) av[k] = *reinterpret_cast<const float4*>(base + (size_t)(q * 8 + k) * a.lda); }
+        }
+    };
+    using K0 = std::integral_constant<int, 0>; using KP = std::integral_constant<int, PRE>; using K8 = std::integral_constant<int, 8>;
+    static_assert(PRE >= 0 && PRE <= 8, "columns of the first chunk requested ahead of the gate");
+    if constexpr (PRE > 0) { if (nq > 0) request(0, K0(), KP()); }
+    const int g = gate.decide(greq, gate_lds);
+    if (g == kSyGateLeave) {
+        if (threadIdx.x == 0) atomicAdd(a.early + (size_t)(blockIdx.x & (kSyEarlySlots - 1)) * kSyVerdictStride, 1ull);
+        return;
+    }
+#ifdef ADMM_HIP_PROBE
+    const long long pt0 = wall_clock64();
+#endif
+    const float* v = g != 0 ? a.v1 : a.v0;
+    float4 aU = make_float4(0.f, 0.f, 0.f, 0.f);
+    if (has) {
+        const float4 uI = active ? *reinterpret_cast<const float4*>(v + row) : make_float4(0.f, 0.f, 0.f, 0.f);
+        const int cj = col0 + lane;
+        const float uj = (lane < cw && cj < a.p) ? v[cj] : 0.f;
+        const auto consume = [&](int q) {
+            float dU[8];
+#pragma unroll
+            for (int k = 0; k < 8; ++k) {
+                const int col = col0 + q * 8 + k;
+                float4 m = av[k];
+                float4 ax = m;
+                if (diag) {
+                    if (row + 0 < col) m.x = 0.f;
+                    if (row + 1 < col) m.y = 0.f;
+                    if (row + 2 < col) m.z = 0.f;
+                    if (row + 3 < col) m.w = 0.f;
+                    ax = m;
+                    if (row + 0 == col) ax.x = 0.f;
+                    if (row + 1 == col) ax.y = 0.f;
+                    if (row + 2 == col) ax.z = 0.f;
+                    if (row + 3 == col) ax.w = 0.f;
+                }
+                dU[k] = fmaf(m.x, uI.x, fmaf(m.y, uI.y, fmaf(m.z, uI.z, m.w * uI.w)));
+                const float ujc = __int_as_float(__builtin_amdgcn_readlane(__float_as_int(uj), (q * 8 + k) & 63));
+                aU.x = fmaf(ax.x, ujc, aU.x); aU.y = fmaf(ax.y, ujc, aU.y); aU.z = fmaf(ax.z, ujc, aU.z); aU.w = fmaf(ax.w, ujc, aU.w);
+            }
+            const float du = butterfly8(dU, lane);
+            if ((lane & 7) == 0) sdot[wid * cw + q * 8 + (lane >> 3)] = du;
+        };
+        if constexpr (PRE > 0) { request(0, KP(), K8()); consume(0); }
+#pragma unroll 1
+        for (int q = PRE > 0 ? 1 : 0; q < nq; ++q) {
+            request(q, K0(), K8());
+            consume(q);
+        }
+    } else {
+        for (int c = lane; c < cw; c += 64) sdot[wid * cw + c] = 0.f;
+    }
+    red[threadIdx.x] = aU;
+    __syncthreads();
+    if (wid == 0) {
+        float4 s = red[lane];
+#pragma unroll
+        for (int ww = 1; ww < 4; ++ww) {
+            const float4 o = red[ww * 64 + lane];
+            s.x += o.x; s.y += o.y; s.z += o.z; s.w += o.w;
+        }
+        *reinterpret_cast<float4*>(a.axp0 + (size_t)seg * a.ldo + row) = s;
+    } else if (wid == 1) {
+        float* dst = a.dot0 + (size_t)rb * a.ldo + t.y;
+        for (int c = lane * 4; c < t.z; c += 256) *reinterpret_cast<float4*>(dst + c) = *reinterpret_cast<const float4*>(&sdot[c]);
+    }
+#ifdef ADMM_HIP_PROBE
+    if (a.probe != nullptr && threadIdx.x == 0) {
+        const int nt = (int)gridDim.x - 1, ti = (int)blockIdx.x - 1;
+        const int which = ti == 0 ? 0 : (ti == nt / 2 ? 1 : (ti == nt - 1 ? 2 : (ti == (3 * nt) / 4 ? 3 : -1)));
         if (which >= 0) {
             long long* d = a.probe + ((size_t)(a.probe_idx & 4095) * 4 + 3) * 8 + which * 2;
             d[0] = pt0; d[1] = wall_clock64();
@@ -550,6 +677,21 @@
         if (ev_start == nullptr && ev_stop == nullptr) hipLaunchKernelGGL((symv2_lower_kernel<Extra>), dim3(ntiles + 1), dim3(kSyThreads), 0, st, a, extra);
         else hipExtLaunchKernelGGL((symv2_lower_kernel<Extra>), dim3(ntiles + 1), dim3(kSyThreads), 0, st, ev_start, ev_stop, 0, a, extra);
     }
+    template <typename Gate, typename Extra = SymvNoExtra>
+    void launch_one(const float* A, long long lda, const float* v0, const float* v1, const int* skip, hipStream_t st, Gate gate, unsigned long long* early,
+                    Extra extra = Extra(), hipEvent_t ev_start = nullptr, hipEvent_t ev_stop = nullptr) {
+        SymvVerdict vd;
+        vd.early = early;
+        const SymvArgs a = args(A, lda, v0, v1, skip, vd);
+        const bool timed = ev_start != nullptr || ev_stop != nullptr;
+        if (nt) {
+            if (!timed) hipLaunchKernelGGL((symv1_lower_kernel<Gate, Extra, true>), dim3(ntiles + 1), dim3(kSyThreads), 0, st, a, gate, extra);
+            else hipExtLaunchKernelGGL((symv1_lower_kernel<Gate, Extra, true>), dim3(ntiles + 1), dim3(kSyThreads), 0, st, ev_start, ev_stop, 0, a, gate, extra);
+            return;
+        }
+        if (!timed) hipLaunchKernelGGL((symv1_lower_kernel<Gate, Extra>), dim3(ntiles + 1), dim3(kSyThreads), 0, st, a, gate, extra);
+        else hipExtLaunchKernelGGL((symv1_lower_kernel<Gate, Extra>), dim3(ntiles + 1), dim3(kSyThreads), 0, st, ev_start, ev_stop, 0, a, gate, extra);
+    }
 };
 
 template <int NL, typename T = float>
@@ -586,6 +728,39 @@
     for (int m = 1; m < NL; m <<= 1) { a += __shfl_xor(a, m, 64); b += __shfl_xor(b, m, 64); }
 }
 
+template <int NL, typename T = float>
+__device__ __forceinline__ T symv_sum_partials1(const T* __restrict__ dot0, const T* __restrict__ axp0,
+                                                long long ldo, int nrb, const SymvSched sched, int p32, int i, int sub, bool valid) {
+    const int ic = valid ? i : 0;
+    const int rbi = ic / kSyRB;
+    const int rb0 = rbi;
+    const int ndot = nrb - rb0;
+    const int nax = sched.nseg(rbi, p32);
+    const int ntot = valid ? ndot + nax : 0;
+    const unsigned ld = (unsigned)ldo;
+    T a = T(0);
+    for (int k0 = 0; k0 < ntot; k0 += 16 * NL) {
+        T va[16];
+#pragma unroll
+        for (int j = 0; j < 16; ++j) {
+            const int k = k0 + j * NL + sub;
+            const bool isdot = k < ndot;
+            const int row = isdot ? rb0 + k : min(k, ntot - 1) - ndot;
+            const unsigned o = (unsigned)row * ld + (unsigned)ic;
+            va[j] = (isdot ? dot0 : axp0)[o];
+        }
+        __builtin_amdgcn_sched_barrier(0);
+#pragma unroll
+        for (int j = 0; j < 16; ++j) {
+            const bool in = k0 + j * NL + sub < ntot;
+            a += in ? va[j] : T(0);
+        }
+    }
+#pragma unroll
+    for (int m = 1; m < NL; m <<= 1) a += __shfl_xor(a, m, 64);
+    return a;
+}
+
 template <typename Extra>
 void symvn_launch(const SymvPlan& sy, int nr, const SymvNArgs& a, hipStream_t st, Extra extra, hipEvent_t ev_start = nullptr, hipEvent_t ev_stop = nullptr) {
     const dim3 grid(sy.ntiles + 1), block(kSyThreads);
diff --git a/include/admm_hip.h b/include/admm_hip.h
--- a/include/admm_hip.h
+++ b/include/admm_hip.h
@@ -291,6 +291,9 @@
                                          int tile_capacity);
 ADMM_HIP_API int admm_hip_test_symv_ex(const float* A, int p, const float* v0, const float* v1, int variant, int part, int nparts,
                                        float* y0, float* y1, int* sched_out);
+ADMM_HIP_API int admm_hip_test_symv_one(const float* A, int p, const float* v0, const float* v1, int gate, int nt, unsigned int fill,
+                                        float* y, float* dot_out, float* axp_out, long long plane_capacity, long long* info_out,
+                                        int* sched_out);
 ADMM_HIP_API int admm_hip_test_symv_multi_ex(const float* A, int p, const float* V, int nr, int rhs_per_pass, int nt, int finish,
                                              float* Yout, int* sched_out);
 ADMM_HIP_API int admm_hip_test_symv_f64acc(const float* A, int p, const float* v0, const float* v1, double* y0, double* y1, int* sched_out);
```

Result: no change. 26360 iterations/s (median of 6 runs) (+2.6%).
